# Christina-hshi/SH-assembly

Hardware: AMD Instinct MI355X
Metric: k-mers counted/sec (whole node), CQF build, C.elegans-like k=47 (higher is better)
Workload: dtype u64

## Files before the change

sh-assembly_amd/csrc/partition_kernels.hip:

```cpp
#include "shk_device.h"
#include <type_traits>

#define SHK_RP_TILE 4096
#define SHK_RP_MAXP 1024
#define SHK_SCAN_TILE 2048

struct ShkRpLevel {
  uint32_t shift;
  uint32_t bits;
  uint32_t nbuckets;
  uint32_t hb;
  uint64_t q_lo;
  uint64_t nslots;
  uint32_t cb;
  uint32_t out32;
  uint32_t ablate;
  uint32_t slot_cap;
  uint32_t ng_log2;
};

__device__ __forceinline__ uint32_t shk_word_region(uint64_t w, uint32_t hb, uint64_t q_lo) {
  uint64_t key = hb >= 64 ? w : (w & ((1ULL << hb) - 1));
  return (uint32_t)(((key >> 8) - q_lo) >> SHK_REGION_LOG2);
}

enum { RP_WORDS = 0, RP_NARROW_OUT = 1, RP_NARROW_IN = 2 };
__device__ __forceinline__ uint32_t shk_narrow_rec(uint64_t w, uint32_t hb, uint64_t q_lo, uint32_t cb) {
  const uint64_t key = hb >= 64 ? w : (w & ((1ULL << hb) - 1));
  const uint32_t up = (uint32_t)(key - (q_lo << 8)) & ((1u << (32 - cb)) - 1);
  return (up << cb) | ((uint32_t)(w >> hb) & ((1u << cb) - 1));
}

template <typename T>
__global__ void k_scan_reduce(const T *in, uint64_t n_host, const uint64_t *n_dev, uint64_t *block_sums) {
  __shared__ uint64_t scratch[SHK_MAX_WAVES + 1];
  const uint64_t n = n_dev ? *n_dev : n_host;
  const uint64_t base = (uint64_t)blockIdx.x * SHK_SCAN_TILE;
  uint64_t s = 0;
  for (uint64_t i = base + threadIdx.x; i < base + SHK_SCAN_TILE && i < n; i += blockDim.x) s += in[i];
  uint64_t tot = shk_block_sum64(s, scratch);
  if (threadIdx.x == 0) block_sums[blockIdx.x] = tot;
}
__global__ void k_scan_top(uint64_t *block_sums, uint64_t nblocks, uint64_t *total) {
  __shared__ uint64_t scratch[SHK_MAX_WAVES + 1];
  __shared__ uint64_t carry_s;
  if (threadIdx.x == 0) carry_s = 0;
  __syncthreads();
  for (uint64_t b = 0; b < nblocks; b += blockDim.x) {
    uint64_t i = b + threadIdx.x;
    uint64_t v = i < nblocks ? block_sums[i] : 0, tot;
    uint64_t ex = shk_block_exscan64(v, &tot, scratch);
    uint64_t carry = carry_s;
    if (i < nblocks) block_sums[i] = carry + ex;
    __syncthreads();
    if (threadIdx.x == 0) carry_s = carry + tot;
    __syncthreads();
  }
  if (threadIdx.x == 0) *total = carry_s;
}
template <typename T>
__global__ void k_scan_apply(const T *in, uint64_t n_host, const uint64_t *n_dev, const uint64_t *block_sums,
                             const uint64_t *total, uint64_t *out) {
  __shared__ uint64_t scratch[SHK_MAX_WAVES + 1];
  const uint64_t n = n_dev ? *n_dev : n_host;
  const uint64_t base = (uint64_t)blockIdx.x * SHK_SCAN_TILE;
  if (base > n) return;
  const unsigned per = SHK_SCAN_TILE / blockDim.x;
  const uint64_t my = base + (uint64_t)threadIdx.x * per;
  uint64_t s = 0;
  for (unsigned j = 0; j < per; j++)
    if (my + j < n) s += in[my + j];
  uint64_t tot;
  uint64_t ex = shk_block_exscan64(s, &tot, scratch) + block_sums[blockIdx.x];
  for (unsigned j = 0; j < per; j++) {
    if (my + j < n) { out[my + j] = ex; ex += in[my + j]; }
  }
  if (threadIdx.x == 0 && n >= base && n < base + SHK_SCAN_TILE) out[n] = *total;
}

__global__ void k_rp_base1(const uint64_t *n_p, uint64_t *bucket_base) {
  if (threadIdx.x == 0 && blockIdx.x == 0) { bucket_base[0] = 0; bucket_base[1] = *n_p; }
}

__global__ void k_rp_tile_first(const uint64_t *bucket_base, uint32_t nbuckets, const uint64_t *n_p, uint32_t *tfb) {
  const uint64_t n = *n_p;
  const uint64_t w = (uint64_t)blockIdx.x * blockDim.x + threadIdx.x;
  const uint64_t pos = w * SHK_RP_TILE;
  if (pos >= n) return;
  uint32_t lo = 0, hi = nbuckets;
  while (hi - lo > 1) {
    uint32_t mid = (lo + hi) / 2;
    if (bucket_base[mid] <= pos) lo = mid; else hi = mid;
  }
  tfb[w] = lo;
}

template <bool NARROW>
__global__ void k_rp_hist(const uint64_t *words_, const uint64_t *n_p, const uint64_t *bucket_base,
                          const uint32_t *tfb, ShkRpLevel lv, uint64_t *hist, uint32_t wtiles) {
  __shared__ uint32_t lh[SHK_RP_MAXP];
  using W = typename std::conditional<NARROW, uint32_t, uint64_t>::type;
  const W *words = reinterpret_cast<const W *>(words_);
  const uint64_t n = *n_p;
  const uint64_t wstart = (uint64_t)blockIdx.x * wtiles * SHK_RP_TILE;
  if (wstart >= n) return;
  const uint64_t wend = wstart + (uint64_t)wtiles * SHK_RP_TILE < n ? wstart + (uint64_t)wtiles * SHK_RP_TILE : n;
  const uint32_t P = 1u << lv.bits;
  for (uint32_t b = tfb[(uint64_t)blockIdx.x * wtiles]; b < lv.nbuckets && bucket_base[b] < wend; b++) {
    const uint64_t lo = bucket_base[b] > wstart ? bucket_base[b] : wstart;
    const uint64_t hi = bucket_base[b + 1] < wend ? bucket_base[b + 1] : wend;
    if (hi <= lo) continue;
    for (uint32_t d = threadIdx.x; d < (P << lv.ng_log2); d += blockDim.x) lh[d] = 0;
    __syncthreads();
    for (uint64_t i0 = lo; i0 < hi; i0 += 4ull * blockDim.x) {
      W w[4];
#pragma unroll
      for (int u = 0; u < 4; u++) {
        const uint64_t i = i0 + (uint64_t)u * blockDim.x + threadIdx.x;
        w[u] = i < hi ? words[i] : 0;
      }
#pragma unroll
      for (int u = 0; u < 4; u++) {
        const uint64_t i = i0 + (uint64_t)u * blockDim.x + threadIdx.x;
        if (i < hi) {
          const uint32_t dg = NARROW ? (uint32_t)(w[u] >> (16 + lv.cb)) : (shk_word_region(w[u], lv.hb, lv.q_lo) >> lv.shift) & (P - 1);
          const uint32_t grp = (uint32_t)(i >> SHK_RP_TILE0_LOG2) & ((1u << lv.ng_log2) - 1);
          atomicAdd(&lh[(dg << lv.ng_log2) | grp], 1u);
        }
      }
    }
    __syncthreads();
    for (uint32_t d = threadIdx.x; d < (P << lv.ng_log2); d += blockDim.x)
      if (lh[d]) atomicAdd((unsigned long long *)&hist[(((uint64_t)b * P) << lv.ng_log2) + d], (unsigned long long)lh[d]);
    __syncthreads();
  }
}

__global__ void k_rp_group_bases(const uint64_t *sub, uint32_t nd, uint32_t ng_log2, uint64_t *base) {
  const uint32_t d = blockIdx.x * blockDim.x + threadIdx.x;
  if (d <= nd) base[d] = sub[(uint64_t)d << ng_log2];
}

#define SHK_RP_THREADS 512
#define SHK_RP_KPT (SHK_RP_TILE / SHK_RP_THREADS)
template <int LB2>
__global__ void k_rp_hist2(const uint64_t *words, const uint64_t *n_p, ShkRpLevel lv0, ShkRpLevel lv1, uint64_t *hist0, uint64_t *hist1,
                           uint32_t wtiles) {
  __shared__ uint32_t lh0[SHK_RP_MAXP];
  __shared__ uint32_t lh1[1u << LB2];
  const uint64_t n = *n_p;
  const uint64_t wstart = (uint64_t)blockIdx.x * wtiles * SHK_RP_TILE;
  if (wstart >= n) return;
  const uint64_t wend = wstart + (uint64_t)wtiles * SHK_RP_TILE < n ? wstart + (uint64_t)wtiles * SHK_RP_TILE : n;
  const uint32_t P0 = 1u << lv0.bits, C = 1u << (lv0.bits + lv1.bits);
  for (uint32_t d = threadIdx.x; d < (P0 << lv0.ng_log2); d += blockDim.x) lh0[d] = 0;
  for (uint32_t d = threadIdx.x; d < C; d += blockDim.x) lh1[d] = 0;
  __syncthreads();
  for (uint64_t i0 = wstart; i0 < wend; i0 += 4ull * blockDim.x) {
    uint64_t w[4];
#pragma unroll
    for (int u = 0; u < 4; u++) {
      const uint64_t i = i0 + (uint64_t)u * blockDim.x + threadIdx.x;
      w[u] = i < wend ? words[i] : 0;
    }
#pragma unroll
    for (int u = 0; u < 4; u++) {
      const uint64_t i = i0 + (uint64_t)u * blockDim.x + threadIdx.x;
      if (i < wend) {
        const uint32_t region = shk_word_region(w[u], lv0.hb, lv0.q_lo);
        const uint32_t d0 = (region >> lv0.shift) & (P0 - 1);
        const uint32_t grp = (uint32_t)(i >> SHK_RP_TILE0_LOG2) & ((1u << lv0.ng_log2) - 1);
        atomicAdd(&lh0[(d0 << lv0.ng_log2) | grp], 1u);
        atomicAdd(&lh1[(region >> lv1.shift) & (C - 1)], 1u);
      }
    }
  }
  __syncthreads();
  for (uint32_t d = threadIdx.x; d < (P0 << lv0.ng_log2); d += blockDim.x)
    if (lh0[d]) atomicAdd((unsigned long long *)&hist0[d], (unsigned long long)lh0[d]);
  for (uint32_t d = threadIdx.x; d < C; d += blockDim.x)
    if (lh1[d]) atomicAdd((unsigned long long *)&hist1[d], (unsigned long long)lh1[d]);
}

__global__ void k_rp_slot_cursors(uint64_t *cursor, uint64_t n, uint32_t cap) {
  const uint64_t stride = (uint64_t)gridDim.x * blockDim.x;
  for (uint64_t i = (uint64_t)blockIdx.x * blockDim.x + threadIdx.x; i < n; i += stride) cursor[i] = i * cap;
}

template <int TILE_LOG2, int THREADS, int PMAX = SHK_RP_MAXP, int FORM = RP_WORDS>
__global__ void __launch_bounds__(THREADS) k_rp_scatter(const uint64_t *in_, uint64_t *out, const uint64_t *n_p,
                                                        const uint64_t *bucket_base, const uint32_t *tfb, ShkRpLevel lv,
                                                        uint64_t *cursor, uint32_t *err) {
  constexpr uint32_t SHK_RP_TILE_ = 1u << TILE_LOG2;
  constexpr int KPT_ = (int)(SHK_RP_TILE_ / THREADS);
  static_assert(SHK_RP_TILE_ <= 65536, "a rank inside a digit takes 16 bits");
  using WIN = typename std::conditional<FORM == RP_NARROW_IN, uint32_t, uint64_t>::type;
  using WST = typename std::conditional<FORM == RP_WORDS, uint64_t, uint32_t>::type;
  const WIN *in = reinterpret_cast<const WIN *>(in_);
  __shared__ uint32_t lh[PMAX];
  __shared__ uint32_t lbase[PMAX];
  __shared__ uint64_t gbase[PMAX];
  __shared__ WST stage[SHK_RP_TILE_];
  __shared__ uint32_t scratch[SHK_MAX_WAVES + 1];
  const uint64_t n = *n_p;
  const uint64_t wstart = (uint64_t)blockIdx.x * SHK_RP_TILE_;
  if (wstart >= n) return;
  const uint64_t wend = wstart + SHK_RP_TILE_ < n ? wstart + SHK_RP_TILE_ : n;
  const uint32_t P = 1u << lv.bits;
  for (uint32_t b = (lv.nbuckets > 1 ? tfb[(uint64_t)blockIdx.x << (TILE_LOG2 - 12)] : 0u); b < lv.nbuckets && bucket_base[b] < wend; b++) {
    const uint64_t lo = bucket_base[b] > wstart ? bucket_base[b] : wstart;
    const uint64_t hi = bucket_base[b + 1] < wend ? bucket_base[b + 1] : wend;
    if (hi <= lo) continue;
    const uint32_t cnt = (uint32_t)(hi - lo);
    for (uint32_t d = threadIdx.x; d < P; d += THREADS) lh[d] = 0;
    WIN w[KPT_];
#pragma unroll
    for (int u = 0; u < KPT_; u++) {
      const uint32_t i = threadIdx.x + (uint32_t)u * THREADS;
      w[u] = i < cnt ? in[lo + i] : 0;
    }
    __syncthreads();
    uint32_t dr[KPT_];
    WST x[KPT_];
#pragma unroll
    for (int u = 0; u < KPT_; u++) {
      const uint32_t i = threadIdx.x + (uint32_t)u * THREADS;
      dr[u] = 0;
      x[u] = (WST)w[u];
      if (i < cnt) {
        uint32_t d;
        if (FORM == RP_NARROW_IN) d = (uint32_t)(w[u] >> (16 + lv.cb));
        else d = (shk_word_region(w[u], lv.hb, lv.q_lo) >> lv.shift) & (P - 1);
        if (FORM == RP_NARROW_OUT) {
          const uint64_t key = lv.hb >= 64 ? w[u] : (w[u] & ((1ULL << lv.hb) - 1));
          if ((key >> 8) - lv.q_lo >= lv.nslots) atomicOr(err, SHK_E_CORRUPT);
          x[u] = (WST)shk_narrow_rec(w[u], lv.hb, lv.q_lo, lv.cb);
        }
        dr[u] = (d << 16) | atomicAdd(&lh[d], 1u);
      }
    }
    __syncthreads();
    uint32_t carry = 0;
    for (uint32_t d0 = 0; d0 < P; d0 += THREADS) {
      uint32_t d = d0 + threadIdx.x;
      uint32_t v = d < P ? lh[d] : 0, tot;
      uint32_t ex = shk_block_exscan(v, &tot, scratch);
      if (d < P) {
        lbase[d] = carry + ex;
        if (lv.ablate & 1) gbase[d] = cursor[((uint64_t)b * P + d) << lv.ng_log2] + (uint64_t)(blockIdx.x % 1024) * 24;
        else gbase[d] = v ? atomicAdd((unsigned long long *)&cursor[((((uint64_t)b * P) + d) << lv.ng_log2) | (blockIdx.x & ((1u << lv.ng_log2) - 1))], (unsigned long long)v) : 0;
        if (lv.slot_cap && v && gbase[d] + v > ((uint64_t)b * P + d + 1) * lv.slot_cap) {
          atomicOr(err, SHK_E_SLOT_FULL);
          gbase[d] = ~0ULL;
        }
      }
      carry += tot;
    }
    __syncthreads();
#pragma unroll
    for (int u = 0; u < KPT_; u++) {
      const uint32_t i = threadIdx.x + (uint32_t)u * THREADS;
      if (i < cnt) stage[lbase[dr[u] >> 16] + (dr[u] & 0xFFFFu)] = x[u];
    }
    __syncthreads();
    if (FORM == RP_NARROW_OUT) {
      uint32_t *out32 = reinterpret_cast<uint32_t *>(out);
      for (uint32_t d = threadIdx.x / SHK_WAVE; d < P; d += THREADS / SHK_WAVE) {
        const uint32_t l0 = lbase[d], len = lh[d];
        const uint64_t g0 = gbase[d];
        for (uint32_t j = threadIdx.x % SHK_WAVE; j < len; j += SHK_WAVE) out32[g0 + j] = stage[l0 + j];
      }
    } else {
      for (uint32_t i = threadIdx.x; i < cnt; i += THREADS) {
        const WST xs = stage[i];
        if (FORM == RP_NARROW_IN) {
          const uint32_t d = xs >> (16 + lv.cb);
          const uint32_t rec = (((uint32_t)(xs >> lv.cb) & 0xFFFFu) << SHK_CHUNK_BITS) | ((uint32_t)xs & ((1u << lv.cb) - 1));
          if (gbase[d] != ~0ULL) reinterpret_cast<uint32_t *>(out)[gbase[d] + (i - lbase[d])] = rec;
          continue;
        }
        const uint64_t x64 = xs;
        uint32_t d = (shk_word_region(x64, lv.hb, lv.q_lo) >> lv.shift) & (P - 1);
        if (lv.out32) {
          const uint64_t key = lv.hb >= 64 ? x64 : (x64 & ((1ULL << lv.hb) - 1));
          const uint64_t q = (key >> 8) - lv.q_lo;
          if (q >= lv.nslots) atomicOr(err, SHK_E_CORRUPT);
          const uint32_t rec = ((((uint32_t)q & (SHK_REGION - 1)) << 8 | (uint32_t)(key & 0xff)) << SHK_CHUNK_BITS) |
                               ((uint32_t)(x64 >> lv.hb) & (SHK_MAX_CHUNKS - 1));
          if (gbase[d] != ~0ULL) reinterpret_cast<uint32_t *>(out)[gbase[d] + (i - lbase[d])] = rec;
        } else {
          out[gbase[d] + (i - lbase[d])] = x64;
        }
      }
    }
    shk_lds_barrier();
  }
}
```

sh-assembly_amd/csrc/roll_kernels.hip:

```cpp
#include "shk_device.h"

#define SHK_ROLL_STEPS 16

struct ShkRollArgs {
  const uint8_t *text;
  uint64_t safe_end;
  const uint64_t *rd_start, *rd_end, *nreads_p;
  const uint16_t *rd_chunk;
  uint32_t chunk_first, chunk_mul, k, hb;
  uint64_t q_lo;
  uint32_t dig_shift, dig_bits;
  uint32_t hist_shift, hist_bits;
  uint64_t *hist;
  uint64_t *cursor;
  uint64_t *out;
  uint64_t cap;
  uint32_t *err;
  const struct ShkQuad *pk;
  const uint64_t *pk_base;
  const uint32_t *pk_flag;
};

struct ShkRollRow { uint64_t f, r; };
struct ShkRollTabs {
// ... 9 lines not shown
    const uint64_t f = b >= 0 ? sf[b] : 0, c = bc >= 0 ? sf[bc] : 0;
    t->in[i].f = f; t->in[i].r = shk_rol64(c, k - 1);
    t->out[i].f = shk_rol64(f, k); t->out[i].r = shk_ror64(c, 1);
    if (i < 4) {
      t->in4[i].f = sf[i]; t->in4[i].r = shk_rol64(sf[3 - i], k - 1);
      t->out4[i].f = shk_rol64(sf[i], k); t->out4[i].r = shk_ror64(sf[3 - i], 1);
    }
  }
}
__device__ __forceinline__ uint64_t shk_rol1(uint64_t x) {
  const uint32_t lo = (uint32_t)x, hi = (uint32_t)(x >> 32);
  return ((uint64_t)((hi << 1) | (lo >> 31)) << 32) | ((lo << 1) | (hi >> 31));
}
__device__ __forceinline__ uint64_t shk_ror1(uint64_t x) {
  const uint32_t lo = (uint32_t)x, hi = (uint32_t)(x >> 32);
  return ((uint64_t)((hi >> 1) | (lo << 31)) << 32) | ((lo >> 1) | (hi << 31));
}

struct ShkQuad { uint32_t x, y, z, w; };
__device__ __forceinline__ ShkQuad shk_quad(uint32_t x, uint32_t y, uint32_t z, uint32_t w) { ShkQuad q = {x, y, z, w}; return q; }
__device__ __forceinline__ ShkQuad shk_load16(const uint8_t *text, uint64_t at, uint64_t safe_end) {
  ShkQuad v;
  if (at + 16 <= safe_end) { __builtin_memcpy(&v, text + at, 16); return v; }
  uint32_t w[4] = {0, 0, 0, 0};
#pragma unroll
  for (int j = 0; j < 16; j++)
    if (at + j < safe_end) w[j >> 2] |= (uint32_t)text[at + j] << (8 * (j & 3));
  return shk_quad(w[0], w[1], w[2], w[3]);
}

#define SHK_ROLL_QUADS 4
struct ShkRollState {
  uint64_t st;
  uint32_t len;
  uint32_t i;
  uint32_t fill;
  uint64_t fh, rh;
  ShkQuad i0_, i1_, i2_, i3_, o0_, o1_, o2_, o3_;
};
__device__ __forceinline__ ShkQuad shk_pick_quad(const ShkQuad &a, const ShkQuad &b, const ShkQuad &c, const ShkQuad &d, uint32_t p) {
  const uint32_t m0 = 0u - (uint32_t)(p == 0), m1 = 0u - (uint32_t)(p == 1), m2 = 0u - (uint32_t)(p == 2), m3 = 0u - (uint32_t)(p == 3);
  ShkQuad v;
  v.x = (a.x & m0) | (b.x & m1) | (c.x & m2) | (d.x & m3);
  v.y = (a.y & m0) | (b.y & m1) | (c.y & m2) | (d.y & m3);
  v.z = (a.z & m0) | (b.z & m1) | (c.z & m2) | (d.z & m3);
  v.w = (a.w & m0) | (b.w & m1) | (c.w & m2) | (d.w & m3);
  return v;
}

template <int NQ, typename Emit>
__device__ __forceinline__ bool shk_roll_round(const ShkRollTabs *T, const uint8_t *text, uint64_t safe_end, ShkRollState &s,
                                               uint32_t k, uint64_t mask, Emit emit) {
  if (s.i >= s.len) return false;
  const uint32_t ph = (s.i / SHK_ROLL_STEPS) % NQ;
  if (ph == 0) {
#define SHK_ROLL_LOAD(Q, IN, OUT) { const uint32_t at = s.i + SHK_ROLL_STEPS * Q; \
      IN = at < s.len ? shk_load16(text, s.st + at, safe_end) : shk_quad(0, 0, 0, 0); \
      OUT = (at >= k && at < s.len) ? shk_load16(text, s.st + at - k, safe_end) : shk_quad(0, 0, 0, 0); }
    SHK_ROLL_LOAD(0, s.i0_, s.o0_)
    if (NQ > 1) SHK_ROLL_LOAD(1, s.i1_, s.o1_)
    if (NQ > 2) { SHK_ROLL_LOAD(2, s.i2_, s.o2_) SHK_ROLL_LOAD(3, s.i3_, s.o3_) }
#undef SHK_ROLL_LOAD
  }
  ShkQuad vin, vout;
  if (NQ == 1) { vin = s.i0_; vout = s.o0_; }
  else if (NQ == 2) { vin = shk_pick_quad(s.i0_, s.i1_, s.i0_, s.i1_, ph); vout = shk_pick_quad(s.o0_, s.o1_, s.o0_, s.o1_, ph); }
  else { vin = shk_pick_quad(s.i0_, s.i1_, s.i2_, s.i3_, ph); vout = shk_pick_quad(s.o0_, s.o1_, s.o2_, s.o3_, ph); }
  const uint32_t win[4] = {vin.x, vin.y, vin.z, vin.w}, wout[4] = {vout.x, vout.y, vout.z, vout.w};
  const uint32_t i0 = s.i;
  uint32_t anyN = 0;
#pragma unroll
  for (int q = 0; q < 4; q++) {
    const uint32_t x = win[q] ^ 0x4E4E4E4Eu;
    anyN |= (x - 0x01010101u) & ~x & 0x80808080u;
  }
  if (s.fill >= k && i0 >= k && !anyN) {
    uint64_t fh = s.fh, rh = s.rh;
    const auto step = [&](int j, bool whole) {
      const int sh = 8 * (j & 3) - 4;
      const uint32_t oi = (sh < 0 ? win[j >> 2] << 4 : win[j >> 2] >> sh) & 0xFF0u;
      const uint32_t oo = (sh < 0 ? wout[j >> 2] << 4 : wout[j >> 2] >> sh) & 0xFF0u;
      const ShkRollRow ri = *reinterpret_cast<const ShkRollRow *>(reinterpret_cast<const uint8_t *>(T->in) + oi);
      const ShkRollRow ro = *reinterpret_cast<const ShkRollRow *>(reinterpret_cast<const uint8_t *>(T->out) + oo);
      fh = shk_rol1(fh) ^ ri.f ^ ro.f;
      rh = shk_ror1(rh) ^ ri.r ^ ro.r;
      if (whole || i0 + j < s.len) emit(j, (fh < rh ? fh : rh) & mask);
    };
    if (i0 + SHK_ROLL_STEPS <= s.len) {
#pragma unroll
      for (int j = 0; j < SHK_ROLL_STEPS; j++) step(j, true);
    } else {
#pragma unroll
      for (int j = 0; j < SHK_ROLL_STEPS; j++) step(j, false);
    }
    s.fh = fh; s.rh = rh;
  } else if (s.fill + SHK_ROLL_STEPS < k && i0 + SHK_ROLL_STEPS <= s.len) {
    uint64_t fh = s.fh, rh = s.rh;
#pragma unroll
    for (int j = 0; j < SHK_ROLL_STEPS; j++) {
      const int sh = 8 * (j & 3) - 4;
      const uint32_t oi = (sh < 0 ? win[j >> 2] << 4 : win[j >> 2] >> sh) & 0xFF0u;
      const ShkRollRow ri = *reinterpret_cast<const ShkRollRow *>(reinterpret_cast<const uint8_t *>(T->in) + oi);
      fh = shk_rol1(fh) ^ ri.f;
      rh = shk_ror1(rh) ^ ri.r;
    }
    s.fh = fh; s.rh = rh; s.fill += SHK_ROLL_STEPS;
  } else {
#pragma unroll
    for (int j = 0; j < SHK_ROLL_STEPS; j++) {
      if (i0 + j < s.len) {
        const uint32_t cin = (win[j >> 2] >> (8 * (j & 3))) & 0xFFu;
        if (s.fill >= k && cin == 'N') {
          s.fill = 0; s.fh = 0; s.rh = 0;
        } else {
          uint64_t f = shk_rol1(s.fh) ^ T->in[cin].f, r = shk_ror1(s.rh) ^ T->in[cin].r;
          if (s.fill >= k) {
            const uint32_t cout = i0 >= k ? (wout[j >> 2] >> (8 * (j & 3))) & 0xFFu : text[s.st + i0 + j - k];
            f ^= T->out[cout].f; r ^= T->out[cout].r;
          } else s.fill++;
          s.fh = f; s.rh = r;
          if (s.fill >= k) emit(j, (f < r ? f : r) & mask);
        }
      }
    }
  }
  s.i = i0 + SHK_ROLL_STEPS < s.len ? i0 + SHK_ROLL_STEPS : s.len;
  return true;
}

__global__ void k_pack_count(const uint64_t *rd_start, const uint64_t *rd_end, const uint64_t *nreads_p, uint32_t k, uint32_t *units) {
  const uint64_t nreads = *nreads_p;
  const uint64_t stride = (uint64_t)gridDim.x * blockDim.x;
  for (uint64_t r = (uint64_t)blockIdx.x * blockDim.x + threadIdx.x; r < nreads; r += stride) {
    const uint64_t len = rd_end[r] - rd_start[r];
    units[r] = (len >= k && len <= 65535) ? (uint32_t)((len + 63) >> 6) : 0;
  }
}
__device__ __forceinline__ uint32_t shk_zero_bytes(uint32_t v) { return ~(((v & 0x7F7F7F7Fu) + 0x7F7F7F7Fu) | v | 0x7F7F7F7Fu); }
__global__ void k_pack_reads(const uint8_t *text, uint64_t safe_end, const uint64_t *rd_start, const uint64_t *rd_end, const uint64_t *nreads_p,
                             const uint64_t *pk_base, uint32_t *flag, ShkQuad *pk, uint64_t cap_units) {
  const uint64_t nreads = *nreads_p;
  const uint64_t stride = ((uint64_t)gridDim.x * blockDim.x) >> 2;
  for (uint64_t r = ((uint64_t)blockIdx.x * blockDim.x + threadIdx.x) >> 2; r < nreads; r += stride) {
    const uint32_t units = flag[r] & 0x7FFFFFFFu;
    if (!units) continue;
    const uint64_t base = pk_base[r];
    if (base + units > cap_units) { if ((threadIdx.x & 3) == 0) atomicOr(&flag[r], 0x80000000u); continue; }
    const uint64_t st = rd_start[r];
    const uint32_t len = (uint32_t)(rd_end[r] - st);
    uint32_t bad = 0;
    for (uint32_t u = threadIdx.x & 3; u < units; u += 4) {
      uint32_t o[4] = {0, 0, 0, 0};
#pragma unroll
      for (int q = 0; q < 4; q++) {
        const uint32_t pos = 64 * u + 16 * q;
        if (pos < len) {
          const ShkQuad v = shk_load16(text, st + pos, safe_end);
          const uint32_t w[4] = {v.x, v.y, v.z, v.w};
#pragma unroll
          for (int b = 0; b < 4; b++) {
            const uint32_t y = w[b] & 0xDFDFDFDFu;
            const uint32_t ok = shk_zero_bytes(y ^ 0x41414141u) | shk_zero_bytes(y ^ 0x43434343u) | shk_zero_bytes(y ^ 0x47474747u) |
                                shk_zero_bytes(y ^ 0x54545454u);
            const uint32_t left = len - pos > 4u * b ? len - pos - 4u * b : 0;
            const uint32_t need = left >= 4 ? 0x80808080u : (0x80808080u & ((1u << (8 * left)) - 1));
            bad |= need & ~ok;
            const uint32_t x = ((w[b] >> 1) ^ (w[b] >> 2)) & 0x03030303u;
            o[q] |= ((x * 0x01041040u) >> 24) << (8 * b);
          }
        }
      }
      pk[base + u] = shk_quad(o[0], o[1], o[2], o[3]);
    }
    if (bad) atomicOr(&flag[r], 0x80000000u);
  }
}

__device__ __forceinline__ uint32_t shk_pick_word(uint32_t a, uint32_t b, uint32_t c, uint32_t d, uint32_t p) {
  return (a & (0u - (uint32_t)(p == 0))) | (b & (0u - (uint32_t)(p == 1))) | (c & (0u - (uint32_t)(p == 2))) | (d & (0u - (uint32_t)(p == 3)));
}
template <typename Emit>
__device__ __forceinline__ bool shk_roll_round_pk(const ShkRollTabs *T, const ShkQuad *pk, ShkRollState &s, uint32_t k, uint64_t mask, Emit emit) {
  if (s.i >= s.len) return false;
  const uint32_t i0 = s.i, ph = (i0 >> 4) & 3;
  if (ph == 0) s.i0_ = pk[i0 >> 6];
  const uint32_t zin = shk_pick_word(s.i0_.x, s.i0_.y, s.i0_.z, s.i0_.w, ph);
  uint64_t fh = s.fh, rh = s.rh;
  if (i0 >= k) {
    const uint32_t n = (i0 >> 4) - ((k + 15) >> 4);
    const uint32_t n3 = n - 3 * ((n * 0xAAABu) >> 17);
    const uint32_t ob = 2 * (i0 - k);
    if (n3 == 0) __builtin_memcpy(&s.o0_, reinterpret_cast<const uint8_t *>(pk) + 4 * (uint64_t)(ob >> 5), 16);
    const uint32_t a = shk_pick_word(s.o0_.x, s.o0_.y, s.o0_.z, 0, n3), b = shk_pick_word(s.o0_.y, s.o0_.z, s.o0_.w, 0, n3);
    const uint32_t zout = (uint32_t)((((uint64_t)b << 32) | a) >> (ob & 31));
    const auto step = [&](int j, bool whole) {
      const uint32_t oi = (j < 2 ? zin << (4 - 2 * j) : zin >> (2 * j - 4)) & 0x30u;
      const uint32_t oo = (j < 2 ? zout << (4 - 2 * j) : zout >> (2 * j - 4)) & 0x30u;
      const ShkRollRow ri = *reinterpret_cast<const ShkRollRow *>(reinterpret_cast<const uint8_t *>(T->in4) + oi);
      const ShkRollRow ro = *reinterpret_cast<const ShkRollRow *>(reinterpret_cast<const uint8_t *>(T->out4) + oo);
      fh = shk_rol1(fh) ^ ri.f ^ ro.f;
      rh = shk_ror1(rh) ^ ri.r ^ ro.r;
      if (whole || i0 + j < s.len) emit(j, (fh < rh ? fh : rh) & mask);
    };
    if (i0 + SHK_ROLL_STEPS <= s.len) {
#pragma unroll
      for (int j = 0; j < SHK_ROLL_STEPS; j++) step(j, true);
    } else {
#pragma unroll
      for (int j = 0; j < SHK_ROLL_STEPS; j++) step(j, false);
    }
  } else if (i0 + SHK_ROLL_STEPS < k) {
#pragma unroll
    for (int j = 0; j < SHK_ROLL_STEPS; j++) {
      const uint32_t oi = (j < 2 ? zin << (4 - 2 * j) : zin >> (2 * j - 4)) & 0x30u;
      const ShkRollRow ri = *reinterpret_cast<const ShkRollRow *>(reinterpret_cast<const uint8_t *>(T->in4) + oi);
      fh = shk_rol1(fh) ^ ri.f;
      rh = shk_ror1(rh) ^ ri.r;
    }
  } else {
    const uint32_t z0 = (i0 >> 6) == 0 ? s.i0_.x : pk[0].x;
#pragma unroll
    for (int j = 0; j < SHK_ROLL_STEPS; j++) {
      const uint32_t idx = i0 + j;
      const ShkRollRow ri = T->in4[(zin >> (2 * j)) & 3u];
      uint64_t f = shk_rol1(fh) ^ ri.f, r = shk_ror1(rh) ^ ri.r;
      if (idx >= k) {
        const ShkRollRow ro = T->out4[(z0 >> (2 * (idx - k))) & 3u];
        f ^= ro.f; r ^= ro.r;
      }
      fh = f; rh = r;
      if (idx + 1 >= k && idx < s.len) emit(j, (f < r ? f : r) & mask);
    }
  }
  s.fh = fh; s.rh = rh;
  s.i = i0 + SHK_ROLL_STEPS < s.len ? i0 + SHK_ROLL_STEPS : s.len;
  return true;
}

__device__ __forceinline__ uint32_t shk_roll_digit(uint64_t key, const ShkRollArgs &A) {
  const uint32_t region = (uint32_t)(key >> 16) - (uint32_t)(A.q_lo >> 8);
  return (region >> A.dig_shift) & ((1u << A.dig_bits) - 1);
}

template <int LB, int THREADS>
__global__ void __launch_bounds__(THREADS) k_roll_hist(ShkRollArgs A) {
  __shared__ ShkRollTabs T;
  __shared__ uint32_t lh[1u << LB];
  shk_roll_tabs_init(&T, A.k);
  const uint32_t P = 1u << A.hist_bits;
  for (uint32_t d = threadIdx.x; d < P; d += blockDim.x) lh[d] = 0;
  __syncthreads();
  const uint64_t nreads = *A.nreads_p;
  const uint64_t mask = A.hb >= 64 ? ~0ULL : ((1ULL << A.hb) - 1);
  const uint64_t stride = (uint64_t)gridDim.x * blockDim.x;
  const uint32_t qlo16 = (uint32_t)(A.q_lo >> 8);
  for (uint64_t r = (uint64_t)blockIdx.x * blockDim.x + threadIdx.x; r < nreads; r += stride) {
    const uint64_t st = A.rd_start[r], en = A.rd_end[r];
    if (en - st > 65535) { atomicOr(A.err, SHK_E_BAD_FASTQ); continue; }
    if (en - st < A.k) continue;
    ShkRollState s;
    s.st = st; s.len = (uint32_t)(en - st); s.i = 0; s.fill = 0; s.fh = 0; s.rh = 0;
    const auto count = [&](int, uint64_t key) { atomicAdd(&lh[(((uint32_t)(key >> 16) - qlo16) >> A.hist_shift) & (P - 1)], 1u); };
    if (A.pk && !(A.pk_flag[r] >> 31)) {
      const ShkQuad *up = A.pk + A.pk_base[r];
      while (shk_roll_round_pk(&T, up, s, A.k, mask, count)) {}
    } else {
      while (shk_roll_round<4>(&T, A.text, A.safe_end, s, A.k, mask, count)) {}
    }
  }
  __syncthreads();
  for (uint32_t d = threadIdx.x; d < P; d += blockDim.x)
    if (lh[d]) atomicAdd((unsigned long long *)&A.hist[d], (unsigned long long)lh[d]);
}
__global__ void k_roll_fold(const uint64_t *hist2, uint32_t p0, uint32_t p1, uint64_t *hist0) {
  const uint32_t d = blockIdx.x * blockDim.x + threadIdx.x;
  if (d >= p0) return;
  uint64_t t = 0;
  for (uint32_t j = 0; j < p1; j++) t += hist2[(uint64_t)d * p1 + j];
  hist0[d] = t;
}

template <int THREADS, int NQ>
__global__ void __launch_bounds__(THREADS) k_roll_scatter(ShkRollArgs A) {
  constexpr uint32_t TILE = THREADS * SHK_ROLL_STEPS;
  __shared__ ShkRollTabs T;
  __shared__ uint32_t lh[1024], lbase[1024];
  __shared__ uint64_t gbase[1024];
  __shared__ uint64_t stage[TILE];
  __shared__ uint32_t scratch[SHK_MAX_WAVES + 1];
  __shared__ uint32_t any_left;
  shk_roll_tabs_init(&T, A.k);
  const uint32_t P = 1u << A.dig_bits;
  const uint64_t nreads = *A.nreads_p;
  const uint64_t mask = A.hb >= 64 ? ~0ULL : ((1ULL << A.hb) - 1);
  const uint64_t stride = (uint64_t)gridDim.x * THREADS;
  uint64_t r = (uint64_t)blockIdx.x * THREADS + threadIdx.x;
  ShkRollState s;
  s.st = 0; s.len = 0; s.i = 0; s.fill = 0; s.fh = 0; s.rh = 0;
  uint64_t tag = 0;
  bool have = false;
  for (;;) {
    while (!have && r < nreads) {
      const uint64_t st = A.rd_start[r], en = A.rd_end[r];
      if (en - st <= 65535 && en - st >= A.k) {
        s.st = st; s.len = (uint32_t)(en - st); s.i = 0; s.fill = 0; s.fh = 0; s.rh = 0;
        tag = (uint64_t)(A.chunk_first + A.rd_chunk[r] * A.chunk_mul) << A.hb;
        if (A.pk && !(A.pk_flag[r] >> 31)) s.st = A.pk_base[r] | (1ULL << 63);
        have = true;
      }
      r += stride;
    }
    for (uint32_t d = threadIdx.x; d < P; d += THREADS) lh[d] = 0;
    if (threadIdx.x == 0) any_left = 0;
    shk_lds_barrier();
    uint64_t w[SHK_ROLL_STEPS];
    uint32_t vm = 0;
    if (have) {
      const auto keep = [&](int j, uint64_t key) {
        w[j] = key | tag;
        atomicAdd(&lh[shk_roll_digit(key, A)], 1u);
        vm |= 1u << j;
      };
      have = (s.st >> 63) ? shk_roll_round_pk(&T, A.pk + (s.st & ~(1ULL << 63)), s, A.k, mask, keep)
                          : shk_roll_round<NQ>(&T, A.text, A.safe_end, s, A.k, mask, keep);
      if (have && s.i >= s.len) have = false;
    }
    if (have || r < nreads) any_left = 1;
    __syncthreads();
    const bool more = any_left != 0;
    uint32_t carry = 0;
    for (uint32_t d0 = 0; d0 < P; d0 += THREADS) {
      const uint32_t d = d0 + threadIdx.x;
      uint32_t v = d < P ? lh[d] : 0, tot;
      const uint32_t ex = shk_block_exscan(v, &tot, scratch);
      if (d < P) {
        lbase[d] = carry + ex;
        gbase[d] = (v ? atomicAdd((unsigned long long *)&A.cursor[d], (unsigned long long)v) : 0) - (carry + ex);
      }
      carry += tot;
    }
    __syncthreads();
    const uint32_t cnt = carry;
#pragma unroll
    for (int u = 0; u < SHK_ROLL_STEPS; u++)
      if ((vm >> u) & 1u) stage[atomicAdd(&lbase[shk_roll_digit(A.hb >= 64 ? w[u] : (w[u] & mask), A)], 1u)] = w[u];
    __syncthreads();
    for (uint32_t i = threadIdx.x; i < cnt; i += THREADS) {
      const uint64_t x = stage[i];
      const uint32_t d = shk_roll_digit(A.hb >= 64 ? x : (x & mask), A);
      const uint64_t at = gbase[d] + i;
      if (at < A.cap) A.out[at] = x; else atomicOr(A.err, SHK_E_KEYS_FULL);
    }
    shk_lds_barrier();
    if (!more) break;
  }
}
```

sh-assembly_amd/csrc/shk_api.hip:

```cpp
#include "../../include/shk.h"
#include <thread>

#include <hip/hip_runtime.h>
#include <math.h>
#include <stdio.h>
#include <stdlib.h>
#include <string.h>
#include <vector>
#include <string>
#include <algorithm>
#include <unordered_set>
#include <unordered_map>

#include "kmer_kernels.hip"
#include "roll_kernels.hip"
#include "partition_kernels.hip"
#include "cqf_kernels.hip"
#include "merge2_kernels.hip"
#include "walk_kernels.hip"
#include "unitig_kernels.hip"

#define SHK_SLACK 256

enum {
  KP_COUNT_LINES, KP_SCAN_CHUNKS, KP_EMIT_READS, KP_COUNT_KEYS, KP_HASH, KP_SCAN, KP_RP_PREP, KP_RP_HIST,
  KP_RP_SCATTER, KP_MERGE_SUM, KP_REGION_SCAN, KP_MERGE_WRITE, KP_MERGE_SPILL, KP_PLACE, KP_MARKS, KP_LOOKUP, KP_WALK, KP_UG_WALK, KP_UG_FINISH, KP_MERGE_FUSED, KP_MERGE_SAMPLE, KP_MISC, KP_ROLL_HIST, KP_ROLL_SCATTER, KP_PACK, KP_RP_SLOTS, KP_RP_SCATTER_NARROW, KP_SPECTRUM, KP_JOIN, KP_N
};
static const char *kp_names[KP_N] = {
  "k_count_lines", "k_scan_chunks", "k_emit_reads", "k_count_keys", "k_hash_reads", "k_scan_*", "k_rp_prep",
  "k_rp_hist", "k_rp_scatter", "k_region_merge<summary>", "k_region_scan", "k_region_merge<write>",
  "k_region_merge<spill>", "k_region_place", "k_denoise_marks", "k_lookup", "k_extend_forward+k_select_seeds", "k_ug_walk", "k_ug_check/emit/median/links", "k_region_merge<fused>", "k_region_merge<sample>", "misc", "k_roll_hist", "k_roll_scatter", "k_pack_reads", "k_rp_slot_cursors", "k_rp_scatter<narrow>", "k_region_spectrum", "k_region_join"};

struct PendingEvent { int id; hipEvent_t a, b; };

#define SHK_SCALAR_WORDS 64
enum ShkDevSlot {
  DS_NREADS = 0,
  DS_NWORDS = 1,
  DS_SCAN_TOTAL = 2,
  DS_MARKS = 3,
  DS_MAX_COUNT = 4,
  DS_DUMP_STOP = 5,
  DS_JOIN_STOP = 6,
  DS_JOIN_ACC = 7,
  DS_WALK_IN = 8,
  DS_WALK_OUT = 10,
  DS_SPECTRUM = 12,
  DS_STAMPS = 16,
  DS_PAIR_LEN = 40,
  DS_PAIR_BASE = 42,
  DS_END = 46
};
enum ShkHostSlot {
  HP_COUNTERS = 0,
  HP_SPECTRUM = 8,
  HP_ERR = 40,
  HP_NREADS = 41,
  HP_NWORDS = 42,
  HP_NWORDS_IN = 43,
  HP_FREE_PTR = 44,
  HP_TOTAL = 45,
  HP_AUX = 46,
  HP_MARKS = 47,
  HP_IFIN = 48,
  HP_IFIRST = 49,
  HP_WALK_IN = 50,
  HP_WALK_OUT = 52,
  HP_PAIR = 56,
  HP_END = 62
};
enum { CNT_NEWD, CNT_ADDED, CNT_REMOVED, CNT_ADDED_BEFORE };
static_assert(HP_COUNTERS + SHK_NCOUNTERS <= HP_ERR, "the counters mirror ends before the error word");
static_assert(HP_COUNTERS + SHK_NCOUNTERS <= HP_SPECTRUM && DS_SPECTRUM + (int)SHK_SPEC_WORDS <= DS_STAMPS, "the spectrum's totals have four words of their own");
static_assert(DS_END <= SHK_SCALAR_WORDS && HP_END <= SHK_SCALAR_WORDS, "both blocks fit their 64 words");
static_assert(DS_PAIR_BASE + 4 == DS_END && HP_PAIR + (DS_END - DS_PAIR_LEN) == HP_END, "the pair block is uploaded in one copy");

enum { RP_SCATTER_GROUPED, RP_SCATTER_WIDE, RP_SCATTER_TILE };
struct ShkPartLevel {
  uint8_t scatter;
  bool pair_hist;
  bool may_slot;
  bool may_narrow;
};

struct ShkStageBufs {
  hipStream_t stream = hipStream_t();
  bool lent = false;
  uint8_t *d_text = nullptr;
  uint64_t *d_chunk_off = nullptr, *d_chunk_len = nullptr, *d_nlines = nullptr, *d_reads_base = nullptr;
  uint64_t *d_rd_start = nullptr, *d_rd_end = nullptr;
  uint16_t *d_rd_chunk = nullptr;
  uint32_t *d_nkeys = nullptr;
  uint64_t *d_key_base = nullptr;
  uint64_t *d_words[2] = {};
  uint64_t *d_scalars = nullptr;
  uint64_t *d_block_sums = nullptr;
  uint64_t *d_hist[4] = {};
  uint64_t *d_base_sub = nullptr;
  uint64_t *d_base[5] = {};
  uint64_t *d_cursor = nullptr;
  uint32_t *d_tfb = nullptr;
  uint32_t *d_err = nullptr;
  uint64_t *h_pinned = nullptr;
  uint32_t last_err_bits = 0;
  uint32_t region_cap = 0;
  uint32_t slot_overflows = 0;
  int slots_off = 0;
  double prof_ms[KP_N] = {};
  uint64_t prof_n[KP_N] = {};
  std::vector<PendingEvent> pending;
  std::vector<hipEvent_t> evpool;
};

struct shk_ctx : ShkStageBufs {
  shk_config cfg;
  int dev;
  uint64_t g_nslots;
  uint64_t q_lo, nslots, xnslots, nblocks, table_bytes;
  uint32_t nregions, rbits;
  uint32_t nlevels;
  ShkRpLevel lv[4];
  ShkPartLevel part[4];
  bool roll_two;
  uint32_t threads, hash_groups;
  uint64_t nelts, ndistinct;
  uint32_t rounds_left, rounds_done;
  uint8_t *tab[2];
  uint64_t *fin[2];
  int cur;
  uint8_t *d_up[2];
  hipStream_t copy_stream;
  hipEvent_t up_done[2];
  int up_next, up_pending[2];
  uint32_t *d_summary;
  long long *d_tile_a, *d_tile_b, *d_tile_f;
  uint64_t *d_dump_offs;
  int big_image;
  uint8_t *spill[2];
  int live;
  int rec_live;
  int table_stale;
  int lazy_ok;
  uint32_t *d_over_list;
  int spill_valid; const uint64_t *spill_words; uint32_t spill_lo, spill_hi; int spill_denoise, spill_big;
  uint64_t spill_nover;
  uint16_t *d_newchunks;
  unsigned long long *d_chist;
  uint64_t *h_chist;
  uint32_t chist_n;
  uint32_t sample_stride;
  uint32_t pt_lo, pt_split, pt_hi; int pt_valid; uint64_t pt_nprot;
  const uint64_t *pt_words;
  unsigned long long *d_counters;
  uint64_t max_reads;
  int prof_on;
  double new_frac;
  int staged;
  uint32_t *d_isum; uint8_t *d_ilens; uint64_t *d_fin_i; uint64_t *d_prot;
  int counted;
  uint64_t *d_send[2];
  int send_next;
  struct ShkFront *front;
};

#define HIPCHK(x) do { hipError_t e_ = (x); if (e_ != hipSuccess) { fprintf(stderr, "libshk: %s failed: %s (%s:%d)\n", #x, hipGetErrorString(e_), __FILE__, __LINE__); return SHK_ERR_HIP; } } while (0)

static hipEvent_t ev_get(ShkStageBufs *c) {
  if (!c->evpool.empty()) { hipEvent_t e = c->evpool.back(); c->evpool.pop_back(); return e; }
  hipEvent_t e; hipEventCreate(&e); return e;
}
struct ProfScope {
  ShkStageBufs *c; int id; bool on; hipEvent_t a, b;
  ProfScope(const shk_ctx *ctx, ShkStageBufs *c_, int id_) : c(c_), id(id_), on(ctx->prof_on != 0) {
    if (on) { a = ev_get(c); b = ev_get(c); hipEventRecord(a, c->stream); }
  }
  ProfScope(shk_ctx *ctx, int id_) : ProfScope(ctx, ctx, id_) {}
  ~ProfScope() {
    if (on) { hipEventRecord(b, c->stream); PendingEvent p = {id, a, b}; c->pending.push_back(p); }
  }
};
static void prof_collect(ShkStageBufs *c) {
  for (size_t i = 0; i < c->pending.size(); i++) {
    float ms = 0;
    hipEventSynchronize(c->pending[i].b);
    hipEventElapsedTime(&ms, c->pending[i].a, c->pending[i].b);
    c->prof_ms[c->pending[i].id] += ms;
    c->prof_n[c->pending[i].id]++;
    c->evpool.push_back(c->pending[i].a);
    c->evpool.push_back(c->pending[i].b);
  }
  c->pending.clear();
}

static int map_err_bits(uint32_t bits) {
  if (!bits) return SHK_OK;
  if (bits & SHK_E_TABLE_FULL) return SHK_ERR_TABLE_FULL;
  if (bits & (SHK_E_OLD_EXTENT | SHK_E_NEW_EXTENT | SHK_E_HASH_FULL | SHK_E_RUN_TOO_LONG)) return SHK_ERR_REGION;
  if (bits & SHK_E_CORRUPT) return SHK_ERR_CORRUPT;
  if (bits & SHK_E_BAD_FASTQ) return SHK_ERR_FASTQ;
  if (bits & SHK_E_KEYS_FULL) return SHK_ERR_BATCH;
  return SHK_ERR_CORRUPT;
}

extern "C" const char *shk_strerror(int code) {
  switch (code) {
    case SHK_OK: return "ok";
    case SHK_ERR_ARG: return "bad argument or unsupported geometry";
    case SHK_ERR_HIP: return "HIP runtime error (is a GPU present?)";
    case SHK_ERR_TABLE_FULL: return "counting quotient filter is full";
    case SHK_ERR_REGION: return "a 256-quotient region exceeds the kernel's on-chip image or hash";
    case SHK_ERR_CORRUPT: return "table metadata inconsistent or key outside this context's range";
    case SHK_ERR_FASTQ: return "malformed FASTQ input";
    case SHK_ERR_BATCH: return "batch exceeds the capacities given to shk_create";
    case SHK_ERR_IO: return "file I/O error";
  }
  return "unknown error";
}
extern "C" uint32_t shk_last_error_bits(shk_ctx *c) { return c ? c->last_err_bits : 0; }

template <typename T> static int dmalloc(T **p, uint64_t n) {
  void *v = nullptr;
  HIPCHK(hipMalloc(&v, n * sizeof(T) + SHK_SLACK));
  *p = (T *)v;
  return 0;
}

static int ensure_chist(shk_ctx *c);
static int point_alloc(shk_ctx *c);
static uint64_t level_out(const shk_ctx *c, uint32_t l) { return (uint64_t)c->lv[l].nbuckets << c->lv[l].bits; }

static int bufs_alloc(const shk_ctx *c, ShkStageBufs *b, bool lent) {
  const uint64_t capk = c->cfg.max_batch_keys;
  const uint32_t maxch = SHK_MAX_CHUNKS;
  b->lent = lent;
  if (lent) HIPCHK(hipStreamCreateWithFlags(&b->stream, hipStreamNonBlocking));
  else HIPCHK(hipStreamCreate(&b->stream));
  if (dmalloc(&b->d_text, c->cfg.max_batch_bytes + 64)) return SHK_ERR_HIP;
  if (dmalloc(&b->d_chunk_off, maxch) || dmalloc(&b->d_chunk_len, maxch) || dmalloc(&b->d_nlines, (uint64_t)maxch * SHK_PARSE_SEGS) ||
      dmalloc(&b->d_reads_base, maxch + 1)) return SHK_ERR_HIP;
  if (dmalloc(&b->d_rd_start, c->max_reads + 1) || dmalloc(&b->d_rd_end, c->max_reads + 1) ||
      dmalloc(&b->d_nkeys, c->max_reads + 1) || dmalloc(&b->d_rd_chunk, c->max_reads + 1) || dmalloc(&b->d_key_base, c->max_reads + 2)) return SHK_ERR_HIP;
  if (!lent && (dmalloc(&b->d_words[0], capk + 1) || dmalloc(&b->d_words[1], capk + 1))) return SHK_ERR_HIP;
  if (dmalloc(&b->d_scalars, SHK_SCALAR_WORDS)) return SHK_ERR_HIP;
  HIPCHK(hipMemsetAsync(b->d_scalars, 0, SHK_SCALAR_WORDS * 8, b->stream));
  {
    uint64_t mx = capk > c->max_reads ? capk : c->max_reads;
    uint64_t pw = 1ULL << c->rbits;
    if (pw > mx) mx = pw;
    if (dmalloc(&b->d_block_sums, mx / SHK_SCAN_TILE + 4 + 8192)) return SHK_ERR_HIP;
  }
  if (dmalloc(&b->d_base[0], 2)) return SHK_ERR_HIP;
  for (uint32_t l = 0; l < c->nlevels; l++) {
    const uint64_t n = level_out(c, l);
    if (dmalloc(&b->d_hist[l], (n << c->lv[l].ng_log2) + 1)) return SHK_ERR_HIP;
    if (!(lent && l + 1 == c->nlevels) && dmalloc(&b->d_base[l + 1], n + 2)) return SHK_ERR_HIP;
    if (l == 0 && dmalloc(&b->d_base_sub, (n << c->lv[0].ng_log2) + 2)) return SHK_ERR_HIP;
  }
  { const uint64_t nb = level_out(c, c->nlevels - 1), first = 1ULL << (c->lv[0].bits + c->lv[0].ng_log2);
    if (dmalloc(&b->d_cursor, (nb > first ? nb : first) + 2)) return SHK_ERR_HIP; }
  if (dmalloc(&b->d_tfb, capk / SHK_RP_TILE + 2)) return SHK_ERR_HIP;
  if (dmalloc(&b->d_err, 4)) return SHK_ERR_HIP;
  HIPCHK(hipMemsetAsync(b->d_err, 0, 16, b->stream));
  HIPCHK(hipHostMalloc((void **)&b->h_pinned, SHK_SCALAR_WORDS * sizeof(uint64_t), hipHostMallocDefault));
  HIPCHK(hipStreamSynchronize(b->stream));
  return SHK_OK;
}

static void bufs_free(const shk_ctx *c, ShkStageBufs *b) {
  if (b->stream) hipStreamSynchronize(b->stream);
  prof_collect(b);
  for (size_t i = 0; i < b->evpool.size(); i++) hipEventDestroy(b->evpool[i]);
  b->evpool.clear();
  hipFree(b->d_text); hipFree(b->d_chunk_off); hipFree(b->d_chunk_len); hipFree(b->d_nlines); hipFree(b->d_reads_base);
  hipFree(b->d_rd_start); hipFree(b->d_rd_end); hipFree(b->d_rd_chunk); hipFree(b->d_nkeys); hipFree(b->d_key_base); hipFree(b->d_scalars);
  hipFree(b->d_block_sums); hipFree(b->d_base_sub); hipFree(b->d_cursor); hipFree(b->d_tfb); hipFree(b->d_err);
  if (!b->lent) { hipFree(b->d_words[0]); hipFree(b->d_words[1]); }
  for (uint32_t l = 0; l < 4; l++) hipFree(b->d_hist[l]);
  for (uint32_t l = 0; l < 5; l++) if (!(b->lent && l == c->nlevels)) hipFree(b->d_base[l]);
  hipHostFree(b->h_pinned);
  if (b->stream) hipStreamDestroy(b->stream);
  *b = ShkStageBufs();
}

static int create_init(shk_ctx *c, const shk_config *cfg) {
  const uint32_t ns = cfg->num_shards ? cfg->num_shards : 1;
  c->cfg = *cfg;
  c->dev = cfg->device;
  HIPCHK(hipSetDevice(c->dev));
  c->g_nslots = 1ULL << cfg->qb;
  if (c->g_nslots / ns < 64) return SHK_ERR_ARG;
  c->nslots = c->g_nslots / ns;
  c->q_lo = c->nslots * cfg->shard_index;
  c->xnslots = c->nslots + (uint64_t)(10 * sqrt((double)c->g_nslots));
  c->nblocks = (c->xnslots + 63) / 64;
  c->table_bytes = c->nblocks * SHK_BLOCK_BYTES;
  c->nregions = (uint32_t)((c->nslots + SHK_REGION - 1) / SHK_REGION);
  c->rbits = 0;
  while ((1u << c->rbits) < c->nregions) c->rbits++;
  const uint32_t mlb = cfg->max_level_bits ? cfg->max_level_bits : 10;
  if (mlb > 10) return SHK_ERR_ARG;
  const uint32_t nlevels = (c->rbits + mlb - 1) / mlb;
  if (nlevels > 4) return SHK_ERR_ARG;
  c->nlevels = nlevels ? nlevels : 1;
  {
    uint32_t left = c->rbits, nb = 1;
    for (uint32_t l = 0; l < c->nlevels; l++) {
      uint32_t bits = (left + (c->nlevels - l) - 1) / (c->nlevels - l);
      left -= bits;
      c->lv[l].shift = left; c->lv[l].bits = bits; c->lv[l].nbuckets = nb; c->lv[l].hb = cfg->hb; c->lv[l].q_lo = c->q_lo;
      c->lv[l].nslots = c->nslots; c->lv[l].cb = 0; c->lv[l].out32 = 0; c->lv[l].ablate = 0; c->lv[l].ng_log2 = 0; c->lv[l].slot_cap = 0;
      nb <<= bits;
    }
    c->lv[c->nlevels - 1].out32 = 1;
    if (c->lv[0].bits >= 2 && c->lv[0].bits <= 7 && !getenv("SHK_RP_NO_GROUPS")) c->lv[0].ng_log2 = 3;
  }
  c->threads = cfg->threads_per_group ? cfg->threads_per_group : 512;
  if (c->threads < 64 || c->threads > 1024 || (c->threads & (c->threads - 1))) return SHK_ERR_ARG;
  c->hash_groups = cfg->hash_groups ? cfg->hash_groups : 2048;
  const bool words8 = getenv("SHK_RP_WORDS8") && atoi(getenv("SHK_RP_WORDS8")) != 0;
  c->roll_two = c->nlevels >= 2 && c->lv[0].bits + c->lv[1].bits <= 14;
  for (uint32_t l = 0; l < c->nlevels; l++) {
    const bool last = l + 1 == c->nlevels;
    c->part[l].scatter = l == 0 && c->lv[0].ng_log2 ? RP_SCATTER_GROUPED : c->threads >= 512 && !last && c->lv[l].bits <= 8 ? RP_SCATTER_WIDE : RP_SCATTER_TILE;
    c->part[l].pair_hist = l == 0 && c->roll_two && c->lv[1].ng_log2 == 0;
    c->part[l].may_slot = last && l >= 1 && c->lv[l].out32;
    c->part[l].may_narrow = l >= 1 && l + 2 == c->nlevels && !words8;
    c->lv[l].cb = 32 - 16 - c->lv[c->nlevels - 1].bits;
  }
  c->rounds_left = cfg->num_denoise;
  c->max_reads = cfg->max_batch_reads ? cfg->max_batch_reads : cfg->max_batch_bytes / 16 + 1024;
  { int rc = bufs_alloc(c, c, false); if (rc) return rc; }
  for (int i = 0; i < 2; i++) {
    if (dmalloc(&c->tab[i], c->table_bytes)) return SHK_ERR_HIP;
    if (dmalloc(&c->fin[i], (uint64_t)c->nregions + 2)) return SHK_ERR_HIP;
  }
  if (dmalloc(&c->d_summary, SHK_SUM_STRIDE * (uint64_t)c->nregions + 8)) return SHK_ERR_HIP;
  if (dmalloc(&c->d_dump_offs, (uint64_t)c->nregions + 2)) return SHK_ERR_HIP;
  c->sample_stride = c->nregions >= (1u << 20) ? 16 : 8;
  if (const char *e = getenv("SHK_SAMPLE_STRIDE")) c->sample_stride = (uint32_t)atoi(e);
  else if (c->nregions < (1u << 14)) c->sample_stride = 0;
  c->lazy_ok = 1;
  if (const char *e = getenv("SHK_LAZY_PLACE")) c->lazy_ok = atoi(e) != 0;
  if (dmalloc(&c->spill[0], (uint64_t)c->nregions * SHK_SPILL_STRIDE) || dmalloc(&c->d_over_list, (uint64_t)c->nregions + 1)) return SHK_ERR_HIP;
  { uint64_t nt = c->nregions / SHK_RSCAN_TILE + 2;
    if (dmalloc(&c->d_tile_a, nt) || dmalloc(&c->d_tile_b, nt) || dmalloc(&c->d_tile_f, nt)) return SHK_ERR_HIP; }
  if (dmalloc(&c->d_counters, SHK_NCOUNTERS)) return SHK_ERR_HIP;
  HIPCHK(hipMemsetAsync(c->tab[0], 0, c->table_bytes + SHK_SLACK, c->stream));
  HIPCHK(hipMemsetAsync(c->tab[1], 0, c->table_bytes + SHK_SLACK, c->stream));
  HIPCHK(hipMemsetAsync(c->fin[0], 0, ((uint64_t)c->nregions + 2) * 8, c->stream));
  HIPCHK(hipMemsetAsync(c->fin[1], 0, ((uint64_t)c->nregions + 2) * 8, c->stream));
  HIPCHK(hipStreamSynchronize(c->stream));
  if (cfg->num_denoise > 0 || cfg->num_shards > 1) {
    if (ensure_chist(c) || point_alloc(c)) return SHK_ERR_HIP;
  }
  if (cfg->num_shards > 1) {
    for (int b = 0; b < 2; b++)
      if (dmalloc(&c->d_send[b], c->cfg.max_batch_keys + 1)) return SHK_ERR_HIP;
  }
  return SHK_OK;
}

extern "C" int shk_create(const shk_config *cfg, shk_ctx **out) {
  if (!cfg || !out) return SHK_ERR_ARG;
  if (cfg->qb < 6 || cfg->qb > 40 || cfg->hb != cfg->qb + 8 || cfg->k < 1 || cfg->k > SHK_MAX_K) return SHK_ERR_ARG;
  uint32_t ns = cfg->num_shards ? cfg->num_shards : 1;
  if (ns & (ns - 1)) return SHK_ERR_ARG;
  if (cfg->shard_index >= ns) return SHK_ERR_ARG;
  if (cfg->hb + SHK_CHUNK_BITS > 64) return SHK_ERR_ARG;
  shk_ctx *c = new shk_ctx();
  const int rc = create_init(c, cfg);
  if (rc) { shk_destroy(c); return rc; }
  *out = c;
  return SHK_OK;
}

static void front_destroy(shk_ctx *c);
extern "C" void shk_destroy(shk_ctx *c) {
  if (!c) return;
  hipSetDevice(c->dev);
  front_destroy(c);
  if (c->stream) hipStreamSynchronize(c->stream);
  if (c->copy_stream) {
    hipStreamSynchronize(c->copy_stream);
    for (int b = 0; b < 2; b++) { if (c->d_up[b]) hipFree(c->d_up[b]); if (c->up_done[b]) hipEventDestroy(c->up_done[b]); }
    hipStreamDestroy(c->copy_stream);
  }
  if (getenv("SHK_STAMPS") && c->d_scalars) {
    unsigned long long st[16];
    hipMemcpy(st, c->d_scalars + DS_STAMPS, sizeof(st), hipMemcpyDeviceToHost);
    static const char *nm[9] = {"stage+init", "fold keys", "old rank/select", "count sort", "merge pass", "scan+stats", "(unused)", "placement", "stores"};
    unsigned long long tot = 0; for (int i = 0; i < 9; i++) tot += st[i];
    for (int i = 0; i < 9; i++) fprintf(stderr, "SHK_STAMPS %-16s %6.2f %%\n", nm[i], tot ? 100.0 * st[i] / tot : 0.0);
  }
  for (int i = 0; i < 2; i++) { hipFree(c->tab[i]); hipFree(c->fin[i]); hipFree(c->d_send[i]); }
  hipFree(c->d_isum); hipFree(c->d_ilens); hipFree(c->d_fin_i); hipFree(c->d_prot);
  hipFree(c->d_newchunks); hipFree(c->d_chist); hipHostFree(c->h_chist);
  hipFree(c->spill[0]); hipFree(c->spill[1]); hipFree(c->d_over_list); hipFree(c->d_summary); hipFree(c->d_dump_offs); hipFree(c->d_tile_a); hipFree(c->d_tile_b); hipFree(c->d_tile_f); hipFree(c->d_counters);
  bufs_free(c, c);
  delete c;
}

template <typename T>
static int run_scan(const shk_ctx *c, ShkStageBufs *b, const T *in, uint64_t n_max, const uint64_t *n_dev, uint64_t *out, uint64_t *sums = nullptr) {
  ProfScope ps(c, b, KP_SCAN);
  if (!sums) sums = b->d_block_sums;
  const uint32_t nb = (uint32_t)(n_max / SHK_SCAN_TILE + 1);
  hipLaunchKernelGGL((k_scan_reduce<T>), dim3(nb), dim3(c->threads), 0, b->stream, in, n_max, n_dev, sums);
  hipLaunchKernelGGL(k_scan_top, dim3(1), dim3(c->threads), 0, b->stream, sums, (uint64_t)nb, b->d_scalars + DS_SCAN_TOTAL);
  hipLaunchKernelGGL((k_scan_apply<T>), dim3(nb), dim3(c->threads), 0, b->stream, in, n_max, n_dev, sums,
                     b->d_scalars + DS_SCAN_TOTAL, out);
  HIPCHK(hipGetLastError());
  return 0;
}

static int err_enqueue(ShkStageBufs *b) { HIPCHK(hipMemcpyAsync(b->h_pinned + HP_ERR, b->d_err, 4, hipMemcpyDeviceToHost, b->stream)); return 0; }
static int err_take(ShkStageBufs *b, bool record, uint32_t *bits) {
  *bits = *(uint32_t *)(b->h_pinned + HP_ERR);
  if (*bits && record) b->last_err_bits = *bits;
  if (*bits) HIPCHK(hipMemsetAsync(b->d_err, 0, 16, b->stream));
  return 0;
}
static int fetch_err(ShkStageBufs *b, uint32_t *bits) {
  if (err_enqueue(b)) return SHK_ERR_HIP;
  HIPCHK(hipStreamSynchronize(b->stream));
  return err_take(b, true, bits);
}
static int set_nwords(ShkStageBufs *b, uint64_t n) {
  b->h_pinned[HP_NWORDS_IN] = n;
  HIPCHK(hipMemcpyAsync(b->d_scalars + DS_NWORDS, b->h_pinned + HP_NWORDS_IN, 8, hipMemcpyHostToDevice, b->stream));
  return 0;
}

static int upload_wait(shk_ctx *c, const void *text, int on_device, hipStream_t stream) {
  for (int u = 0; on_device && u < 2; u++)
    if (c->d_up[u] && text == (const void *)c->d_up[u] && c->up_pending[u]) { HIPCHK(hipStreamWaitEvent(stream, c->up_done[u], 0)); c->up_pending[u] = 0; }
  return SHK_OK;
}

static bool chunk_labels_ok(uint32_t nchunks, uint32_t chunk_first, uint32_t chunk_mul) {
  return nchunks != 0 && nchunks <= SHK_MAX_CHUNKS && chunk_first + (uint64_t)(nchunks - 1) * chunk_mul < SHK_MAX_CHUNKS;
}

static bool text_aligned(const void *text, int on_device) { return !on_device || ((uintptr_t)text & 15) == 0; }
static int parse_stage(const shk_ctx *c, ShkStageBufs *b, const void *text, int on_device, uint64_t text_bytes, const uint64_t *chunk_off,
                       const uint64_t *chunk_len, uint32_t nchunks, const uint8_t **dtext_out, uint64_t *nreads_out) {
  if (!text_aligned(text, on_device)) return SHK_ERR_ARG;
  for (uint32_t i = 0; i < nchunks; i++)
    if (chunk_off[i] + chunk_len[i] > text_bytes) return SHK_ERR_ARG;
  const uint8_t *dtext;
  if (on_device) {
    dtext = (const uint8_t *)text;
  } else {
    if (text_bytes > c->cfg.max_batch_bytes) return SHK_ERR_BATCH;
    HIPCHK(hipMemcpyAsync(b->d_text, text, text_bytes, hipMemcpyHostToDevice, b->stream));
    dtext = b->d_text;
  }
  HIPCHK(hipMemcpyAsync(b->d_chunk_off, chunk_off, nchunks * 8, hipMemcpyHostToDevice, b->stream));
  HIPCHK(hipMemcpyAsync(b->d_chunk_len, chunk_len, nchunks * 8, hipMemcpyHostToDevice, b->stream));
  { ProfScope ps(c, b, KP_COUNT_LINES);
    hipLaunchKernelGGL(k_count_lines, dim3(nchunks * SHK_PARSE_SEGS), dim3(c->threads), 0, b->stream, dtext, b->d_chunk_off, b->d_chunk_len, b->d_nlines); }
  { ProfScope ps(c, b, KP_SCAN_CHUNKS);
    hipLaunchKernelGGL(k_scan_chunks, dim3(1), dim3(c->threads), 0, b->stream, b->d_nlines, nchunks, b->d_reads_base, b->d_scalars + DS_NREADS); }
  HIPCHK(hipMemcpyAsync(b->h_pinned + HP_NREADS, b->d_scalars + DS_NREADS, 8, hipMemcpyDeviceToHost, b->stream));
  HIPCHK(hipStreamSynchronize(b->stream));
  const uint64_t nreads = b->h_pinned[HP_NREADS];
  if (nreads > c->max_reads) return SHK_ERR_BATCH;
  { ProfScope ps(c, b, KP_EMIT_READS);
    hipLaunchKernelGGL(k_emit_reads, dim3(nchunks * SHK_PARSE_SEGS), dim3(c->threads), 0, b->stream, dtext, b->d_chunk_off, b->d_chunk_len,
                       b->d_reads_base, b->d_nlines, b->d_rd_start, b->d_rd_end, b->d_rd_chunk); }
  *dtext_out = dtext;
  *nreads_out = nreads;
  return SHK_OK;
}

static int hash_stage(const shk_ctx *c, ShkStageBufs *b, const void *text, int on_device, uint64_t text_bytes, const uint64_t *chunk_off,
                      const uint64_t *chunk_len, uint32_t nchunks, uint32_t chunk_first, uint32_t chunk_mul, bool hist0 = false) {
  if (!chunk_labels_ok(nchunks, chunk_first, chunk_mul)) return SHK_ERR_BATCH;
  if (!text_aligned(text, on_device)) return SHK_ERR_ARG;
  if (hist0) HIPCHK(hipMemsetAsync(b->d_hist[0], 0, (1ULL << (c->lv[0].bits + c->lv[0].ng_log2)) * 8, b->stream));
  const uint8_t *dtext;
  uint64_t nreads;
  { int rc = parse_stage(c, b, text, on_device, text_bytes, chunk_off, chunk_len, nchunks, &dtext, &nreads); if (rc) return rc; }
  uint32_t groups = c->hash_groups;
  { uint64_t need = nreads / (c->threads / SHK_WAVE) + 1; if (need < groups) groups = (uint32_t)need; }
  { ProfScope ps(c, b, KP_COUNT_KEYS);
    const uint64_t blocks = nreads / 256 + 1;
    hipLaunchKernelGGL(k_count_keys, dim3((uint32_t)(blocks < (1u << 20) ? blocks : (1u << 20))), dim3(256), 0, b->stream, dtext, b->d_rd_start, b->d_rd_end,
                       b->d_scalars + DS_NREADS, c->cfg.k, b->d_nkeys, b->d_err); }
  if (run_scan<uint32_t>(c, b, b->d_nkeys, nreads, nullptr, b->d_key_base)) return SHK_ERR_HIP;
  HIPCHK(hipMemcpyAsync(b->d_scalars + DS_NWORDS, b->d_key_base + nreads, 8, hipMemcpyDeviceToDevice, b->stream));
  { ProfScope ps(c, b, KP_HASH);
    const uint32_t ht = c->threads < SHK_HASH_WAVES * SHK_WAVE ? c->threads : SHK_HASH_WAVES * SHK_WAVE;
    hipLaunchKernelGGL(k_hash_reads, dim3(groups * (c->threads / ht)), dim3(ht), 0, b->stream, dtext, b->d_rd_start, b->d_rd_end,
                       b->d_scalars + DS_NREADS, b->d_rd_chunk, chunk_first, chunk_mul, b->d_key_base, c->cfg.k, c->cfg.hb,
                       b->d_words[0], c->cfg.max_batch_keys, b->d_err, hist0 ? b->d_hist[0] : nullptr, c->lv[0].shift, c->lv[0].bits, c->q_lo, c->lv[0].ng_log2); }
  HIPCHK(hipGetLastError());
  return SHK_OK;
}

static int pack_stage(const shk_ctx *c, ShkStageBufs *b, ShkRollArgs &A, uint64_t nreads, uint64_t text_bytes, uint64_t *buf) {
  A.pk = nullptr; A.pk_base = nullptr; A.pk_flag = nullptr;
  const uint64_t cap_units = c->cfg.max_batch_keys / 2 > 1 ? c->cfg.max_batch_keys / 2 - 1 : 0;
  if (getenv("SHK_NO_PACK") || text_bytes / 64 + nreads + 1 > cap_units) return SHK_OK;
  ProfScope ps(c, b, KP_PACK);
  const uint32_t t = c->threads < 256 ? c->threads : 256;
  { const uint64_t blocks = nreads / t + 1;
    hipLaunchKernelGGL(k_pack_count, dim3((uint32_t)(blocks < 4096 ? blocks : 4096)), dim3(t), 0, b->stream, (const uint64_t *)b->d_rd_start,
                       (const uint64_t *)b->d_rd_end, (const uint64_t *)(b->d_scalars + DS_NREADS), c->cfg.k, b->d_nkeys); }
  if (run_scan<uint32_t>(c, b, b->d_nkeys, nreads, nullptr, b->d_key_base)) return SHK_ERR_HIP;
  { const uint64_t blocks = nreads * 4 / t + 1;
    hipLaunchKernelGGL(k_pack_reads, dim3((uint32_t)(blocks < 16384 ? blocks : 16384)), dim3(t), 0, b->stream, A.text, A.safe_end,
                       (const uint64_t *)b->d_rd_start, (const uint64_t *)b->d_rd_end, (const uint64_t *)(b->d_scalars + DS_NREADS),
                       (const uint64_t *)b->d_key_base, b->d_nkeys, (ShkQuad *)buf, cap_units); }
  A.pk = (const ShkQuad *)buf; A.pk_base = b->d_key_base; A.pk_flag = b->d_nkeys;
  return SHK_OK;
}

static void roll_args(const shk_ctx *c, ShkStageBufs *b, ShkRollArgs &A, const uint8_t *dtext, uint64_t text_bytes,
                      uint32_t chunk_first, uint32_t chunk_mul) {
  A.text = dtext; A.safe_end = (text_bytes + 15) & ~15ULL;
  A.rd_start = b->d_rd_start; A.rd_end = b->d_rd_end; A.nreads_p = b->d_scalars + DS_NREADS; A.rd_chunk = b->d_rd_chunk;
  A.chunk_first = chunk_first; A.chunk_mul = chunk_mul; A.k = c->cfg.k; A.hb = c->cfg.hb;
  A.cap = c->cfg.max_batch_keys; A.err = b->d_err;
}
static void launch_roll_hist(const shk_ctx *c, ShkStageBufs *b, const ShkRollArgs &A, uint64_t nreads, bool wide) {
  const bool small = c->threads < 512;
  const uint32_t t = small ? 64 : wide ? 512 : 256, max_blocks = small ? 64 : wide ? 1024 : 4096;
  const uint64_t blocks = nreads / t + 1;
  const dim3 grid((uint32_t)(blocks < max_blocks ? blocks : max_blocks));
  if (small && wide) hipLaunchKernelGGL((k_roll_hist<14, 64>), grid, dim3(64), 0, b->stream, A);
  else if (small) hipLaunchKernelGGL((k_roll_hist<10, 64>), grid, dim3(64), 0, b->stream, A);
  else if (wide) hipLaunchKernelGGL((k_roll_hist<14, 512>), grid, dim3(512), 0, b->stream, A);
  else hipLaunchKernelGGL((k_roll_hist<10, 256>), grid, dim3(256), 0, b->stream, A);
}
static void launch_roll_scatter(const shk_ctx *c, ShkStageBufs *b, const ShkRollArgs &A, uint64_t nreads) {
  ProfScope ps(c, b, KP_ROLL_SCATTER);
  if (c->threads >= 512) {
    const uint64_t blocks = nreads / 1024 + 1;
    hipLaunchKernelGGL((k_roll_scatter<1024, 1>), dim3((uint32_t)(blocks < 512 ? blocks : 512)), dim3(1024), 0, b->stream, A);
  } else {
    const uint64_t blocks = nreads / 64 + 1;
    hipLaunchKernelGGL((k_roll_scatter<64, 4>), dim3((uint32_t)(blocks < 64 ? blocks : 64)), dim3(64), 0, b->stream, A);
  }
}

static bool roll_path(const shk_ctx *c) { return c->nlevels >= 2; }
static int roll_stage(const shk_ctx *c, ShkStageBufs *b, const void *text, int on_device, uint64_t text_bytes, const uint64_t *chunk_off,
                      const uint64_t *chunk_len, uint32_t nchunks, uint32_t chunk_first, uint32_t chunk_mul) {
  if (!chunk_labels_ok(nchunks, chunk_first, chunk_mul)) return SHK_ERR_BATCH;
  const uint8_t *dtext;
  uint64_t nreads;
  { int rc = parse_stage(c, b, text, on_device, text_bytes, chunk_off, chunk_len, nchunks, &dtext, &nreads); if (rc) return rc; }
  const uint64_t P = 1ULL << c->lv[0].bits;
  const uint32_t cb = c->lv[0].bits + c->lv[1].bits;
  const bool two = c->roll_two;
  if (two) HIPCHK(hipMemsetAsync(b->d_hist[1], 0, (1ULL << cb) * 8, b->stream));
  else HIPCHK(hipMemsetAsync(b->d_hist[0], 0, P * 8, b->stream));
  ShkRollArgs A;
  roll_args(c, b, A, dtext, text_bytes, chunk_first, chunk_mul);
  A.q_lo = c->q_lo;
  A.dig_shift = c->lv[0].shift; A.dig_bits = c->lv[0].bits;
  A.hist = two ? b->d_hist[1] : b->d_hist[0]; A.hist_shift = two ? c->lv[1].shift : c->lv[0].shift; A.hist_bits = two ? cb : c->lv[0].bits;
  A.cursor = b->d_cursor; A.out = b->d_words[0];
  { int rc = pack_stage(c, b, A, nreads, text_bytes, b->d_words[1]); if (rc) return rc; }
  { ProfScope ps(c, b, KP_ROLL_HIST);
    launch_roll_hist(c, b, A, nreads, two);
    if (two) hipLaunchKernelGGL(k_roll_fold, dim3((uint32_t)(P / 256 + 1)), dim3(256), 0, b->stream, (const uint64_t *)b->d_hist[1], (uint32_t)P,
                                1u << c->lv[1].bits, b->d_hist[0]); }
  if (run_scan<uint64_t>(c, b, b->d_hist[0], P, nullptr, b->d_base[1])) return SHK_ERR_HIP;
  HIPCHK(hipMemcpyAsync(b->d_scalars + DS_NWORDS, b->d_base[1] + P, 8, hipMemcpyDeviceToDevice, b->stream));
  HIPCHK(hipMemcpyAsync(b->d_cursor, b->d_base[1], P * 8, hipMemcpyDeviceToDevice, b->stream));
  launch_roll_scatter(c, b, A, nreads);
  HIPCHK(hipGetLastError());
  return SHK_OK;
}

struct ShkPartInput {
  const uint64_t *src[2]; uint64_t n[2]; int nsrc;
  int in_buf;
  uint32_t first_level;
  bool counted[2];
  uint32_t nchunks;
};
static ShkPartInput part_from_roll(const shk_ctx *c, const ShkStageBufs *b, uint64_t n, uint32_t nchunks) { return {{b->d_words[0], nullptr}, {n, 0}, 1, 0, 1, {false, c->roll_two}, nchunks}; }
static ShkPartInput part_from_hash(const ShkStageBufs *b, uint64_t n, uint32_t nchunks) { return {{b->d_words[0], nullptr}, {n, 0}, 1, 0, 0, {true, false}, nchunks}; }
static ShkPartInput part_from_words(const ShkStageBufs *b, const uint64_t *w, uint64_t n, const uint64_t *w2 = nullptr, uint64_t n2 = 0) {
  return {{w, w2}, {n, n2}, w2 ? 2 : 1, w == b->d_words[0] ? 0 : w == b->d_words[1] ? 1 : -1, 0, {false, false}, 0};
}

static uint32_t slot_capacity(const shk_ctx *c, uint64_t nregions, uint64_t nwords) {
  uint64_t cp = 2 * c->cfg.max_batch_keys / nregions;
  if (cp > (1u << 20)) cp = 1u << 20;
  const double mean = (double)nwords / (double)nregions;
  return cp >= 64 && (double)cp >= mean + 6.0 * sqrt(8.0 * mean + 1.0) + 16.0 ? (uint32_t)cp : 0;
}

static int partition_stage(const shk_ctx *c, ShkStageBufs *b, const ShkPartInput &in, int *dst) {
  const uint64_t *n_p = b->d_scalars + DS_NWORDS;
  const uint64_t nmax = in.n[0] + in.n[1];
  { ProfScope ps(c, b, KP_RP_PREP);
    hipLaunchKernelGGL(k_rp_base1, dim3(1), dim3(64), 0, b->stream, n_p, b->d_base[0]); }
  const uint32_t nwin = (uint32_t)(nmax / SHK_RP_TILE + 1);
  int cur = in.in_buf < 0 ? 1 : in.in_buf;
  bool counted[4] = {in.counted[0], in.counted[1], false, false};
  bool narrow = false;
  b->region_cap = 0;
  for (uint32_t l = in.first_level; l < c->nlevels; l++) {
    const ShkPartLevel &pl = c->part[l];
    const uint64_t nb = c->lv[l].nbuckets, P = 1ULL << c->lv[l].bits;
    const bool narrow_in = narrow;
    narrow = pl.may_narrow && in.nchunks && in.nchunks <= (1u << c->lv[l].cb);
    struct Src { const uint64_t *w, *n_p, *base; uint64_t n; } srcs[2] = {{l == in.first_level ? in.src[0] : b->d_words[cur], n_p, b->d_base[l], nmax}, {}};
    int nsrc = 1;
    if (l == 0 && in.nsrc == 2) {
      srcs[0] = {in.src[0], b->d_scalars + DS_PAIR_LEN, b->d_scalars + DS_PAIR_BASE, in.n[0]};
      srcs[1] = {in.src[1], b->d_scalars + DS_PAIR_LEN + 1, b->d_scalars + DS_PAIR_BASE + 2, in.n[1]};
      nsrc = 2;
    }
    uint32_t cap = pl.may_slot && !b->slots_off && !counted[l] ? slot_capacity(c, nb * P, nmax) : 0;
    { ProfScope ps(c, b, KP_RP_PREP);
      hipLaunchKernelGGL(k_rp_tile_first, dim3(nwin / 256 + 1), dim3(256), 0, b->stream, b->d_base[l], (uint32_t)nb, n_p, b->d_tfb); }
    for (;;) {
      ShkRpLevel lvl = c->lv[l];
#ifdef SHK_DIAGNOSTICS
      if (const char *e = getenv("SHK_RP_ABLATE")) lvl.ablate = (uint32_t)atoi(e);
#endif
      uint64_t *cursor = b->d_cursor;
      if (cap) {
        ProfScope ps(c, b, KP_RP_SLOTS);
        cursor = b->d_base[l + 1];
        lvl.slot_cap = cap;
        hipLaunchKernelGGL(k_rp_slot_cursors, dim3((uint32_t)((nb * P) / 256 + 1 < 4096 ? (nb * P) / 256 + 1 : 4096)), dim3(256), 0, b->stream, cursor, nb * P, cap);
      } else {
        if (!counted[l] && pl.pair_hist) {
          HIPCHK(hipMemsetAsync(b->d_hist[0], 0, (P << c->lv[0].ng_log2) * 8, b->stream));
          HIPCHK(hipMemsetAsync(b->d_hist[1], 0, (P << c->lv[1].bits) * 8, b->stream));
          ProfScope ps(c, b, KP_RP_HIST);
          const uint32_t wt = nwin / 1024 + 1;
          for (int si = 0; si < nsrc; si++)
            hipLaunchKernelGGL((k_rp_hist2<14>), dim3(nwin / wt + 1), dim3(c->threads < 512 ? c->threads : 512), 0, b->stream, srcs[si].w, srcs[si].n_p,
                               c->lv[0], c->lv[1], b->d_hist[0], b->d_hist[1], wt);
          counted[1] = true;
        } else if (!counted[l]) {
          HIPCHK(hipMemsetAsync(b->d_hist[l], 0, ((nb * P) << c->lv[l].ng_log2) * 8, b->stream));
          ProfScope ps(c, b, KP_RP_HIST);
          const uint32_t wt = nwin / 4096 + 1;
          for (int si = 0; si < nsrc; si++)
            if (narrow_in)
              hipLaunchKernelGGL(k_rp_hist<true>, dim3(nwin / wt + 1), dim3(c->threads), 0, b->stream, srcs[si].w, srcs[si].n_p, srcs[si].base, b->d_tfb,
                                 c->lv[l], b->d_hist[l], wt);
            else
              hipLaunchKernelGGL(k_rp_hist<false>, dim3(nwin / wt + 1), dim3(c->threads), 0, b->stream, srcs[si].w, srcs[si].n_p, srcs[si].base, b->d_tfb,
                                 c->lv[l], b->d_hist[l], wt);
        }
        if (c->lv[l].ng_log2) {
          const uint32_t ng = c->lv[l].ng_log2;
          if (run_scan<uint64_t>(c, b, b->d_hist[l], P << ng, nullptr, b->d_base_sub)) return SHK_ERR_HIP;
          HIPCHK(hipMemcpyAsync(b->d_cursor, b->d_base_sub, (P << ng) * 8, hipMemcpyDeviceToDevice, b->stream));
          ProfScope ps(c, b, KP_RP_PREP);
          hipLaunchKernelGGL(k_rp_group_bases, dim3((uint32_t)(P / 256 + 1)), dim3(256), 0, b->stream, b->d_base_sub, (uint32_t)P, ng, b->d_base[l + 1]);
        } else {
          if (run_scan<uint64_t>(c, b, b->d_hist[l], nb * P, nullptr, b->d_base[l + 1])) return SHK_ERR_HIP;
          HIPCHK(hipMemcpyAsync(b->d_cursor, b->d_base[l + 1], nb * P * 8, hipMemcpyDeviceToDevice, b->stream));
        }
      }
      { ProfScope ps(c, b, narrow || narrow_in ? KP_RP_SCATTER_NARROW : KP_RP_SCATTER);
        for (int si = 0; si < nsrc; si++) {
          const Src &S = srcs[si];
          const dim3 wide((uint32_t)(S.n >> SHK_RP_TILE0_LOG2) + 1);
          if (narrow && pl.scatter == RP_SCATTER_WIDE)
            hipLaunchKernelGGL((k_rp_scatter<SHK_RP_TILE0_LOG2, 1024, 256, RP_NARROW_OUT>), wide, dim3(1024), 0, b->stream, S.w, b->d_words[cur ^ 1], S.n_p,
                               S.base, b->d_tfb, lvl, cursor, b->d_err);
          else if (narrow)
            hipLaunchKernelGGL((k_rp_scatter<12, SHK_RP_THREADS, SHK_RP_MAXP, RP_NARROW_OUT>), dim3((uint32_t)(S.n / SHK_RP_TILE + 1)), dim3(SHK_RP_THREADS), 0,
                               b->stream, S.w, b->d_words[cur ^ 1], S.n_p, S.base, b->d_tfb, lvl, cursor, b->d_err);
          else if (narrow_in)
            hipLaunchKernelGGL((k_rp_scatter<12, SHK_RP_THREADS, SHK_RP_MAXP, RP_NARROW_IN>), dim3((uint32_t)(S.n / SHK_RP_TILE + 1)), dim3(SHK_RP_THREADS), 0,
                               b->stream, S.w, b->d_words[cur ^ 1], S.n_p, S.base, b->d_tfb, lvl, cursor, b->d_err);
          else if (pl.scatter == RP_SCATTER_GROUPED)
            hipLaunchKernelGGL((k_rp_scatter<SHK_RP_TILE0_LOG2, 1024>), wide, dim3(1024), 0, b->stream, S.w, b->d_words[cur ^ 1], S.n_p, S.base,
                               b->d_tfb, lvl, cursor, b->d_err);
          else if (pl.scatter == RP_SCATTER_WIDE)
            hipLaunchKernelGGL((k_rp_scatter<SHK_RP_TILE0_LOG2, 1024, 256>), wide, dim3(1024), 0, b->stream, S.w, b->d_words[cur ^ 1], S.n_p, S.base,
                               b->d_tfb, lvl, cursor, b->d_err);
          else
            hipLaunchKernelGGL((k_rp_scatter<12, SHK_RP_THREADS>), dim3((uint32_t)(S.n / SHK_RP_TILE + 1)), dim3(SHK_RP_THREADS), 0, b->stream, S.w,
                               b->d_words[cur ^ 1], S.n_p, S.base, b->d_tfb, lvl, cursor, b->d_err);
        } }
      if (!cap) break;
      uint32_t bits = 0;
      if (fetch_err(b, &bits)) return SHK_ERR_HIP;
      if (bits & ~SHK_E_SLOT_FULL) return map_err_bits(bits & ~SHK_E_SLOT_FULL);
      if (!bits) { b->region_cap = cap; b->slot_overflows = 0; break; }
      if (++b->slot_overflows >= 2) b->slots_off = 1;
      cap = 0;
    }
    cur ^= 1;
  }
  HIPCHK(hipGetLastError());
  *dst = cur;
  return SHK_OK;
}

#define SHK_REGION_SLICE (1u << 24)
#define SHK_FOR_REGION_SLICES(c, A, nblk) \
  for (uint32_t r0_ = 0, nblk = 0; r0_ < (c)->nregions && ((A).r0 = r0_, nblk = (c)->nregions - r0_ < SHK_REGION_SLICE ? (c)->nregions - r0_ : SHK_REGION_SLICE, true); r0_ += SHK_REGION_SLICE)

template <int MODE>
static void launch_merge(shk_ctx *c, const ShkMergeArgs &A0, bool rec = false) {
  ShkMergeArgs A = A0;
  SHK_FOR_REGION_SLICES(c, A, nblk) {
    if (MODE != 1 && rec)
      hipLaunchKernelGGL((k_region_merge<MODE == 1 ? 0 : MODE, SHK_IMG_BLOCKS, false, true>), dim3(nblk), dim3(SHK_MERGE_GROUP), 0, c->stream, A);
    else if (c->big_image)
      hipLaunchKernelGGL((k_region_merge<MODE, SHK_IMG_BLOCKS_BIG>), dim3(nblk), dim3(SHK_MERGE_GROUP), 0, c->stream, A);
    else
      hipLaunchKernelGGL((k_region_merge<MODE, SHK_IMG_BLOCKS>), dim3(nblk), dim3(SHK_MERGE_GROUP), 0, c->stream, A);
  }
}

struct MergeOut {
  uint64_t newd, added, removed;
  uint32_t err;
};

static uint8_t *spill_out(const shk_ctx *c) { return c->spill[c->rec_live ? c->live ^ 1 : c->live]; }

static bool lazy_reserve(shk_ctx *c) {
  if (!c->lazy_ok || c->spill[1]) return c->lazy_ok != 0;
  void *v = nullptr;
  if (hipMalloc(&v, (uint64_t)c->nregions * SHK_SPILL_STRIDE + SHK_SLACK) != hipSuccess) {
    (void)hipGetLastError();
    c->lazy_ok = 0;
    return false;
  }
  c->spill[1] = (uint8_t *)v;
  return true;
}

static void fill_args(shk_ctx *c, ShkMergeArgs *A, const uint64_t *words, uint32_t lo, uint32_t hi, int denoise);
static int table_sync(shk_ctx *c) {
  if (!c->table_stale) return SHK_OK;
  ShkMergeArgs A;
  fill_args(c, &A, nullptr, 0, 0, 0);
  A.tabB = c->tab[c->cur]; A.finB = c->fin[c->cur]; A.spill = c->spill[c->live]; A.summary = nullptr;
  HIPCHK(hipMemsetAsync(c->tab[c->cur], 0, c->table_bytes, c->stream));
  { ProfScope ps(c, KP_PLACE);
    SHK_FOR_REGION_SLICES(c, A, nblk)
      hipLaunchKernelGGL((k_region_place<SHK_IMG_BLOCKS>), dim3(nblk), dim3(SHK_WAVE), 0, c->stream, A); }
  HIPCHK(hipGetLastError());
  uint32_t bits = 0;
  if (fetch_err(c, &bits)) return SHK_ERR_HIP;
  if (bits) return map_err_bits(bits);
  c->table_stale = 0;
  return SHK_OK;
}

static void fill_args(shk_ctx *c, ShkMergeArgs *A, const uint64_t *words, uint32_t lo, uint32_t hi, int denoise) {
  A->want_hist = 0;
  A->tabA = c->tab[c->cur]; A->tabB = c->tab[c->cur ^ 1];
  A->finA = c->fin[c->cur]; A->finB = c->fin[c->cur ^ 1];
  A->words = reinterpret_cast<const uint32_t *>(words); A->region_base = c->d_base[c->nlevels]; A->region_cap = c->region_cap;
  A->nslots = c->nslots; A->xnslots = c->xnslots; A->nblocks = c->nblocks; A->q_lo = c->q_lo; A->hb = c->cfg.hb;
  A->chunk_lo = lo; A->chunk_hi = hi; A->denoise = denoise;
  A->ablate = 0;
#ifdef SHK_DIAGNOSTICS
  { const char *ab = getenv("SHK_ABLATE"); A->ablate = ab ? (uint32_t)atoi(ab) : 0; }
#endif
  { const char *sp = getenv("SHK_STAMPS");
    A->dbg = (sp && strcmp(sp, "fused") != 0) ? (unsigned long long *)(c->d_scalars + DS_STAMPS) : nullptr; }
  A->spill = spill_out(c); A->orec = c->spill[c->live]; A->over_list = c->d_over_list; A->n_over = c->d_counters + SHK_CNT_NOVER; A->list = nullptr;
  A->newchunks = nullptr; A->chist = nullptr;
  A->counted = c->counted;
  A->r0 = 0; A->rstride = 1;
  A->split = ~0u; A->isum = nullptr; A->ilens = nullptr; A->prot_list = nullptr; A->nprot = 0;
  A->summary = c->d_summary; A->counters = c->d_counters; A->err = c->d_err;
}

static int ensure_chist(shk_ctx *c) {
  if (c->d_newchunks) return SHK_OK;
  if (dmalloc(&c->d_newchunks, (uint64_t)c->nregions * SHK_NC_CAP) || dmalloc(&c->d_chist, (uint64_t)SHK_MAX_CHUNKS)) return SHK_ERR_HIP;
  HIPCHK(hipHostMalloc((void **)&c->h_chist, SHK_MAX_CHUNKS * sizeof(uint64_t), hipHostMallocDefault));
  return SHK_OK;
}

static int merge_summary(shk_ctx *c, const uint64_t *words, uint32_t lo, uint32_t hi, int denoise, MergeOut *o,
                         bool with_chist, bool spill) {
  const bool rec = c->rec_live && !denoise;
  if (!rec) { int rc = table_sync(c); if (rc) return rc; }
  ShkMergeArgs A;
  fill_args(c, &A, words, lo, hi, denoise);
  HIPCHK(hipMemsetAsync(c->d_counters, 0, (SHK_CNT_NOVER + 1) * 8, c->stream));
  c->spill_valid = 0;
  if (with_chist) {
    int rc = ensure_chist(c);
    if (rc) return rc;
    A.want_hist = 1; A.newchunks = c->d_newchunks; A.chist = c->d_chist;
    HIPCHK(hipMemsetAsync(c->d_chist, 0, SHK_MAX_CHUNKS * 8, c->stream));
  }
  if (spill) { ProfScope ps(c, KP_MERGE_SPILL);
    launch_merge<3>(c, A, rec); }
  else { ProfScope ps(c, KP_MERGE_SUM);
    launch_merge<0>(c, A, rec); }
  { ProfScope ps(c, KP_REGION_SCAN);
    const uint32_t ntiles = (c->nregions + SHK_RSCAN_TILE - 1) / SHK_RSCAN_TILE;
    hipLaunchKernelGGL(k_region_scan_a, dim3(ntiles), dim3(c->threads), 0, c->stream, c->d_summary, c->nregions, c->d_tile_a, c->d_tile_b);
    hipLaunchKernelGGL(k_region_scan_b, dim3(1), dim3(c->threads), 0, c->stream, c->d_tile_a, c->d_tile_b, ntiles, c->d_tile_f);
    hipLaunchKernelGGL(k_region_scan_c, dim3(ntiles), dim3(c->threads), 0, c->stream, c->d_summary, c->nregions, c->d_tile_f,
                       c->xnslots, (uint32_t)(c->big_image ? SHK_IMG_BLOCKS_BIG * 64 : SHK_IMG_SLOTS), c->fin[c->cur ^ 1], c->d_counters, c->d_err); }
  if (with_chist) {
    ProfScope ps(c, KP_MISC);
    hipLaunchKernelGGL(k_chunk_hist, dim3((c->nregions + SHK_CHIST_REGIONS - 1) / SHK_CHIST_REGIONS), dim3(256), 0, c->stream,
                       c->d_newchunks, c->d_summary, c->nregions, c->d_chist);
    HIPCHK(hipMemcpyAsync(c->h_chist, c->d_chist, ((uint64_t)hi + 1) * 8, hipMemcpyDeviceToHost, c->stream));
  }
  HIPCHK(hipGetLastError());
  const uint64_t *cnt = c->h_pinned + HP_COUNTERS;
  HIPCHK(hipMemcpyAsync(c->h_pinned + HP_COUNTERS, c->d_counters, (SHK_CNT_NOVER + 1) * 8, hipMemcpyDeviceToHost, c->stream));
  if (err_enqueue(c)) return SHK_ERR_HIP;
  HIPCHK(hipStreamSynchronize(c->stream));
  o->newd = cnt[CNT_NEWD]; o->added = cnt[CNT_ADDED]; o->removed = cnt[CNT_REMOVED];
  if (err_take(c, true, &o->err)) return SHK_ERR_HIP;
  c->chist_n = with_chist ? hi + 1 : 0;
  if (spill && !o->err) {
    c->spill_valid = 1; c->spill_words = words; c->spill_lo = lo; c->spill_hi = hi; c->spill_denoise = denoise;
    c->spill_big = c->big_image; c->spill_nover = cnt[SHK_CNT_NOVER];
  }
  return SHK_OK;
}

static int merge_write(shk_ctx *c, const uint64_t *words, uint32_t lo, uint32_t hi, int denoise) {
  const bool match = c->spill_valid && c->spill_words == words && c->spill_lo == lo && c->spill_hi == hi && c->spill_denoise == denoise &&
                     c->spill_big == c->big_image;
  if (match && c->spill_nover == 0 && !c->big_image && !c->counted && lazy_reserve(c)) {
    if (c->rec_live) c->live ^= 1;
    c->rec_live = 1; c->table_stale = 1;
    c->spill_valid = 0;
    c->cur ^= 1;
    return SHK_OK;
  }
  if (!match || c->spill_nover) { int rc = table_sync(c); if (rc) return rc; }
  ShkMergeArgs A;
  fill_args(c, &A, words, lo, hi, denoise);
  HIPCHK(hipMemsetAsync(c->tab[c->cur ^ 1], 0, c->table_bytes, c->stream));
  if (match) {
    { ProfScope ps(c, KP_PLACE);
      SHK_FOR_REGION_SLICES(c, A, nblk) {
        if (c->big_image) hipLaunchKernelGGL((k_region_place<SHK_IMG_BLOCKS_BIG>), dim3(nblk), dim3(SHK_WAVE), 0, c->stream, A);
        else hipLaunchKernelGGL((k_region_place<SHK_IMG_BLOCKS>), dim3(nblk), dim3(SHK_WAVE), 0, c->stream, A);
      }
      A.r0 = 0; }
    if (c->spill_nover) {
      A.list = c->d_over_list;
      ProfScope ps(c, KP_MERGE_WRITE);
      if (c->big_image)
        hipLaunchKernelGGL((k_region_merge<1, SHK_IMG_BLOCKS_BIG>), dim3((uint32_t)c->spill_nover), dim3(SHK_MERGE_GROUP), 0, c->stream, A);
      else
        hipLaunchKernelGGL((k_region_merge<1, SHK_IMG_BLOCKS>), dim3((uint32_t)c->spill_nover), dim3(SHK_MERGE_GROUP), 0, c->stream, A);
    }
  } else {
    ProfScope ps(c, KP_MERGE_WRITE);
    launch_merge<1>(c, A);
  }
  c->spill_valid = 0;
  HIPCHK(hipGetLastError());
  c->rec_live = 0; c->table_stale = 0;
  c->cur ^= 1;
  return SHK_OK;
}

static int denoise_round_once(shk_ctx *c, uint64_t *removed) {
  uint64_t ml = c->cfg.min_denoise_len ? c->cfg.min_denoise_len : (1ULL << 20);
  { int rc = table_sync(c); if (rc) return rc; }
  { ProfScope ps(c, KP_MARKS);
    hipLaunchKernelGGL(k_denoise_marks, dim3(1), dim3(64), 0, c->stream, c->tab[c->cur], c->nslots, c->xnslots, c->nblocks,
                       ml, (unsigned long long *)(c->d_scalars + DS_MARKS)); }
  MergeOut o;
  int rc = merge_summary(c, nullptr, 0, 0, 1, &o, false, true);
  if (rc) return rc;
  if (o.err) return map_err_bits(o.err);
  rc = merge_write(c, nullptr, 0, 0, 1);
  if (rc) return rc;
  c->nelts -= o.removed;
  c->ndistinct -= o.removed;
  *removed = o.removed;
  return SHK_OK;
}

static int denoise_with_rest(shk_ctx *c, const uint64_t *words, uint32_t lo, uint32_t hi, shk_batch_stats *st, bool *done) {
  *done = false;
  uint64_t ml = c->cfg.min_denoise_len ? c->cfg.min_denoise_len : (1ULL << 20);
  { int rc = table_sync(c); if (rc) return rc; }
  { ProfScope ps(c, KP_MARKS);
    hipLaunchKernelGGL(k_denoise_marks, dim3(1), dim3(64), 0, c->stream, c->tab[c->cur], c->nslots, c->xnslots, c->nblocks,
                       ml, (unsigned long long *)(c->d_scalars + DS_MARKS)); }
  MergeOut o;
  int rc = merge_summary(c, words, lo, hi, 1, &o, false, true);
  if (rc) return rc;
  if (o.err) return SHK_OK;
  if (c->rounds_left > 0 && c->ndistinct - o.removed + o.newd >= c->cfg.ndistinct_for_denoise) return SHK_OK;
  rc = merge_write(c, words, lo, hi, 1);
  if (rc) return rc;
  c->nelts = c->nelts - o.removed + o.added;
  c->ndistinct = c->ndistinct - o.removed + o.newd;
  st->removed += o.removed; st->denoise_rounds++;
  st->kmers += o.added; st->new_distinct += o.newd; st->chunks += hi - lo + 1;
  c->big_image = 0;
  *done = true;
  return SHK_OK;
}

#define SHK_PROT_CAP 65536u
struct PointOut {
  uint64_t newd_after, added_after, removed, added_before;
  uint32_t err;
  uint64_t islots, ifin;
  int first_used;
};

static int point_alloc(shk_ctx *c) {
  if (c->d_isum) return SHK_OK;
  if (dmalloc(&c->d_isum, 2 * (uint64_t)c->nregions + 2) || dmalloc(&c->d_ilens, (uint64_t)c->nregions * SHK_REGION) ||
      dmalloc(&c->d_fin_i, (uint64_t)c->nregions + 2) || dmalloc(&c->d_prot, (uint64_t)SHK_PROT_CAP)) return SHK_ERR_HIP;
  return SHK_OK;
}

static void point_scans(shk_ctx *c, bool final_table, bool inter_table, long long carry) {
  const uint32_t ntiles = (c->nregions + SHK_RSCAN_TILE - 1) / SHK_RSCAN_TILE;
  const uint32_t img_slots = (uint32_t)SHK_IMG_SLOTS;
  ProfScope ps(c, KP_REGION_SCAN);
  if (final_table) {
    hipLaunchKernelGGL(k_region_scan_a, dim3(ntiles), dim3(c->threads), 0, c->stream, c->d_summary, c->nregions, c->d_tile_a, c->d_tile_b, (uint32_t)SHK_SUM_STRIDE);
    hipLaunchKernelGGL(k_region_scan_b, dim3(1), dim3(c->threads), 0, c->stream, c->d_tile_a, c->d_tile_b, ntiles, c->d_tile_f, 0LL);
    hipLaunchKernelGGL(k_region_scan_c, dim3(ntiles), dim3(c->threads), 0, c->stream, c->d_summary, c->nregions, c->d_tile_f,
                       c->xnslots, img_slots, c->fin[c->cur ^ 1], c->d_counters, c->d_err, (uint32_t)SHK_SUM_STRIDE);
  }
  if (inter_table) {
    hipLaunchKernelGGL(k_region_scan_a, dim3(ntiles), dim3(c->threads), 0, c->stream, c->d_isum, c->nregions, c->d_tile_a, c->d_tile_b, 2u);
    hipLaunchKernelGGL(k_region_scan_b, dim3(1), dim3(c->threads), 0, c->stream, c->d_tile_a, c->d_tile_b, ntiles, c->d_tile_f, carry);
    hipLaunchKernelGGL(k_region_scan_c, dim3(ntiles), dim3(c->threads), 0, c->stream, c->d_isum, c->nregions, c->d_tile_f,
                       c->xnslots, img_slots, c->d_fin_i, c->d_counters, c->d_err, 2u);
  }
}

static int point_read(shk_ctx *c, PointOut *po) {
  HIPCHK(hipGetLastError());
  const uint64_t *cnt = c->h_pinned + HP_COUNTERS;
  HIPCHK(hipMemcpyAsync(c->h_pinned + HP_COUNTERS, c->d_counters, SHK_NCOUNTERS * 8, hipMemcpyDeviceToHost, c->stream));
  if (err_enqueue(c)) return SHK_ERR_HIP;
  HIPCHK(hipStreamSynchronize(c->stream));
  po->newd_after = cnt[CNT_NEWD]; po->added_after = cnt[CNT_ADDED]; po->removed = cnt[CNT_REMOVED]; po->added_before = cnt[CNT_ADDED_BEFORE];
  return err_take(c, false, &po->err);
}

static int point_try(shk_ctx *c, const uint64_t *words, uint32_t lo, uint32_t split, uint32_t hi, bool with_chist, PointOut *po) {
  int rc = point_alloc(c);
  if (rc) return rc;
  if (with_chist) { rc = ensure_chist(c); if (rc) return rc; }
  ShkMergeArgs A;
  fill_args(c, &A, words, lo, hi, 1);
  A.split = split; A.isum = c->d_isum; A.ilens = c->d_ilens;
  if (with_chist) {
    A.want_hist = 1; A.newchunks = c->d_newchunks; A.chist = c->d_chist;
    HIPCHK(hipMemsetAsync(c->d_chist, 0, SHK_MAX_CHUNKS * 8, c->stream));
  }
  { const char *sp = getenv("SHK_STAMPS");
    A.dbg = (sp && strcmp(sp, "plain") != 0) ? (unsigned long long *)(c->d_scalars + DS_STAMPS) : nullptr; }
  c->spill_valid = 0;
  c->chist_n = 0;
  HIPCHK(hipMemsetAsync(c->d_counters, 0, SHK_NCOUNTERS * 8, c->stream));
  { ProfScope ps(c, KP_MERGE_FUSED);
    SHK_FOR_REGION_SLICES(c, A, nblk) {
      if (c->rec_live) hipLaunchKernelGGL((k_region_merge<3, SHK_IMG_BLOCKS, true, true>), dim3(nblk), dim3(SHK_MERGE_GROUP), 0, c->stream, A);
      else hipLaunchKernelGGL((k_region_merge<3, SHK_IMG_BLOCKS, true>), dim3(nblk), dim3(SHK_MERGE_GROUP), 0, c->stream, A);
    } }
  point_scans(c, true, true, 0);
  if (with_chist) {
    ProfScope ps(c, KP_MISC);
    hipLaunchKernelGGL(k_chunk_hist, dim3((c->nregions + SHK_CHIST_REGIONS - 1) / SHK_CHIST_REGIONS), dim3(256), 0, c->stream,
                       c->d_newchunks, c->d_summary, c->nregions, c->d_chist, 1u);
    HIPCHK(hipMemcpyAsync(c->h_chist, c->d_chist, ((uint64_t)hi + 1) * 8, hipMemcpyDeviceToHost, c->stream));
  }
  HIPCHK(hipMemcpyAsync(c->h_pinned + HP_IFIN, c->d_fin_i + c->nregions, 8, hipMemcpyDeviceToHost, c->stream));
  HIPCHK(hipMemcpyAsync(c->h_pinned + HP_IFIRST, c->d_ilens, 1, hipMemcpyDeviceToHost, c->stream));
  rc = point_read(c, po);
  if (rc) return rc;
  po->islots = c->h_pinned[HP_COUNTERS + SHK_CNT_ISLOTS];
  po->ifin = c->h_pinned[HP_IFIN];
  po->first_used = (c->h_pinned[HP_IFIRST] & 0xff) != 0;
  if (with_chist && !po->err) c->chist_n = hi + 1;
  return SHK_OK;
}

static int point_walk(shk_ctx *c, long long carry, const ShkWalkShard &W, const uint64_t state_in[2], uint64_t state_out[2],
                      uint64_t *nprot, uint32_t *err) {
  const uint64_t ml = c->cfg.min_denoise_len ? c->cfg.min_denoise_len : (1ULL << 20);
  if (carry > 0) point_scans(c, false, true, carry);
  c->h_pinned[HP_WALK_IN] = state_in[0]; c->h_pinned[HP_WALK_IN + 1] = state_in[1];
  HIPCHK(hipMemcpyAsync(c->d_scalars + DS_WALK_IN, c->h_pinned + HP_WALK_IN, 16, hipMemcpyHostToDevice, c->stream));
  { ProfScope ps(c, KP_MARKS);
    hipLaunchKernelGGL(k_denoise_marks_virtual, dim3(1), dim3(64), 0, c->stream, (const uint64_t *)c->d_fin_i, (const uint8_t *)c->d_ilens,
                       (const uint32_t *)c->d_isum, c->nslots, c->xnslots, ml, c->d_prot, SHK_PROT_CAP, (unsigned long long *)(c->d_scalars + DS_MARKS),
                       W, (const uint64_t *)(c->d_scalars + DS_WALK_IN), c->d_scalars + DS_WALK_OUT); }
  HIPCHK(hipGetLastError());
  HIPCHK(hipMemcpyAsync(c->h_pinned + HP_MARKS, c->d_scalars + DS_MARKS, 8, hipMemcpyDeviceToHost, c->stream));
  HIPCHK(hipMemcpyAsync(c->h_pinned + HP_WALK_OUT, c->d_scalars + DS_WALK_OUT, 16, hipMemcpyDeviceToHost, c->stream));
  if (err_enqueue(c)) return SHK_ERR_HIP;
  HIPCHK(hipStreamSynchronize(c->stream));
  *nprot = c->h_pinned[HP_MARKS];
  state_out[0] = c->h_pinned[HP_WALK_OUT]; state_out[1] = c->h_pinned[HP_WALK_OUT + 1];
  return err_take(c, false, err);
}

static int point_finish(shk_ctx *c, const uint64_t *words, uint32_t lo, uint32_t split, uint32_t hi, uint64_t nprot, PointOut *po) {
  if (nprot > SHK_PROT_CAP) { po->err |= SHK_E_FUSED; return SHK_OK; }
  if (nprot) {
    std::vector<uint64_t> prot(nprot);
    HIPCHK(hipMemcpyAsync(prot.data(), c->d_prot, nprot * 8, hipMemcpyDeviceToHost, c->stream));
    HIPCHK(hipStreamSynchronize(c->stream));
    std::vector<uint32_t> regs;
    for (uint64_t q : prot) { const uint32_t r = (uint32_t)(q >> SHK_REGION_LOG2); if (regs.empty() || regs.back() != r) regs.push_back(r); }
    ShkMergeArgs A;
    fill_args(c, &A, words, lo, hi, 1);
    A.split = split; A.isum = c->d_isum; A.ilens = c->d_ilens;
    HIPCHK(hipMemsetAsync(c->d_counters, 0, SHK_NCOUNTERS * 8, c->stream));
    HIPCHK(hipMemcpyAsync(c->d_over_list, regs.data(), regs.size() * 4, hipMemcpyHostToDevice, c->stream));
    A.list = c->d_over_list; A.prot_list = c->d_prot; A.nprot = (uint32_t)nprot;
    { ProfScope ps(c, KP_MISC);
      if (c->rec_live) hipLaunchKernelGGL((k_region_merge<3, SHK_IMG_BLOCKS, true, true>), dim3((uint32_t)regs.size()), dim3(SHK_MERGE_GROUP), 0, c->stream, A);
      else hipLaunchKernelGGL((k_region_merge<3, SHK_IMG_BLOCKS, true>), dim3((uint32_t)regs.size()), dim3(SHK_MERGE_GROUP), 0, c->stream, A); }
    HIPCHK(hipStreamSynchronize(c->stream));
    point_scans(c, true, false, 0);
    int rc = point_read(c, po);
    if (rc) return rc;
  }
  if (!po->err) {
    c->spill_valid = 1; c->spill_words = words; c->spill_lo = lo; c->spill_hi = hi; c->spill_denoise = 1; c->spill_big = c->big_image;
    c->spill_nover = 0;
  }
  return SHK_OK;
}

static int denoise_fused(shk_ctx *c, const uint64_t *words, uint32_t lo, uint32_t cstar, uint32_t hi, uint64_t newd_before,
                         shk_batch_stats *st, bool *done, bool verify = false, uint32_t *exact_ch = nullptr, int *crossing = nullptr) {
  *done = false;
  if (crossing) *crossing = -1;
  if (c->big_image || getenv("SHK_NO_FUSED_POINT")) return SHK_OK;
  PointOut po;
  int rc = point_try(c, words, lo, cstar, hi, verify, &po);
  if (rc) return rc;
  if (po.err) {
    if (getenv("SHK_DEBUG_FUSED")) fprintf(stderr, "SHK_DEBUG_FUSED fallback: flags 0x%x\n", po.err);
    return SHK_OK;
  }
  if (verify) {
    uint64_t run = c->ndistinct;
    uint32_t ch = lo;
    for (; ch < hi; ch++) {
      run += c->h_chist[ch];
      if (run >= c->cfg.ndistinct_for_denoise) break;
    }
    if (ch == hi) run += c->h_chist[ch];
    const bool crosses = run >= c->cfg.ndistinct_for_denoise;
    if (exact_ch) *exact_ch = ch;
    if (crossing) *crossing = crosses ? 1 : 0;
    if (getenv("SHK_DEBUG_FUSED")) fprintf(stderr, "SHK_DEBUG_FUSED guess %u exact %u crossing %d\n", cstar, ch, (int)crosses);
    if (!crosses || ch != cstar) return SHK_OK;
    newd_before = run - c->ndistinct;
  }
  ShkWalkShard W;
  W.prev_fp = -1; W.cap_local = c->nslots; W.last = 1; W.next_first_used = 0;
  const uint64_t s_in[2] = {0, 0};
  uint64_t s_out[2], nprot = 0;
  uint32_t werr = 0;
  rc = point_walk(c, 0, W, s_in, s_out, &nprot, &werr);
  if (rc) return rc;
  if (werr) return SHK_OK;
  rc = point_finish(c, words, lo, cstar, hi, nprot, &po);
  if (rc) return rc;
  if (po.err) {
    c->spill_valid = 0;
    if (getenv("SHK_DEBUG_FUSED")) fprintf(stderr, "SHK_DEBUG_FUSED fallback: flags 0x%x (second go)\n", po.err);
    return SHK_OK;
  }
  if (c->rounds_left > 1 && c->ndistinct + newd_before - po.removed + po.newd_after >= c->cfg.ndistinct_for_denoise) { c->spill_valid = 0; return SHK_OK; }
  rc = merge_write(c, words, lo, hi, 1);
  if (rc) return rc;
  c->nelts = c->nelts + po.added_before - po.removed + po.added_after;
  c->ndistinct = c->ndistinct + newd_before - po.removed + po.newd_after;
  c->rounds_left--; c->rounds_done++;
  st->removed += po.removed; st->denoise_rounds++;
  st->kmers += po.added_before + po.added_after; st->new_distinct += newd_before + po.newd_after; st->chunks += hi - lo + 1;
  *done = true;
  if (getenv("SHK_DEBUG_FUSED")) fprintf(stderr, "SHK_DEBUG_FUSED one-pass point at chunk %u of [%u, %u]: removed %llu protected %llu\n", cstar, lo, hi,
                                         (unsigned long long)po.removed, (unsigned long long)nprot);
  return SHK_OK;
}

static int denoise_round(shk_ctx *c, uint64_t *removed) {
  int rc = denoise_round_once(c, removed);
  if (rc == SHK_ERR_REGION && !c->big_image && (c->last_err_bits & (SHK_E_OLD_EXTENT | SHK_E_NEW_EXTENT))) {
    c->big_image = 1;
    c->last_err_bits = 0;
    rc = denoise_round_once(c, removed);
  }
  if (!rc) c->big_image = 0;
  return rc;
}

static int sample_pass(shk_ctx *c, const uint64_t *words, uint32_t lo, uint32_t hi, uint32_t *ns_out, uint32_t *err_out) {
  int rc = ensure_chist(c);
  if (rc) return rc;
  const uint32_t stride = c->sample_stride > 1 ? c->sample_stride : 1;
  const uint32_t ns = (c->nregions + stride - 1) / stride;
  ShkMergeArgs A;
  fill_args(c, &A, words, lo, hi, 0);
  A.want_hist = 1; A.newchunks = c->d_newchunks; A.chist = c->d_chist; A.rstride = stride;
  c->spill_valid = 0;
  c->chist_n = 0;
  HIPCHK(hipMemsetAsync(c->d_chist, 0, SHK_MAX_CHUNKS * 8, c->stream));
  { ProfScope ps(c, KP_MERGE_SAMPLE);
    for (uint32_t r0 = 0; r0 < ns; r0 += SHK_REGION_SLICE) {
      A.r0 = r0;
      const uint32_t nblk = ns - r0 < SHK_REGION_SLICE ? ns - r0 : SHK_REGION_SLICE;
      if (c->rec_live) hipLaunchKernelGGL((k_region_merge<0, SHK_IMG_BLOCKS, false, true>), dim3(nblk), dim3(SHK_MERGE_GROUP), 0, c->stream, A);
      else hipLaunchKernelGGL((k_region_merge<0, SHK_IMG_BLOCKS>), dim3(nblk), dim3(SHK_MERGE_GROUP), 0, c->stream, A);
    }
    hipLaunchKernelGGL(k_chunk_hist, dim3((ns + SHK_CHIST_REGIONS - 1) / SHK_CHIST_REGIONS), dim3(256), 0, c->stream,
                       c->d_newchunks, c->d_summary, c->nregions, c->d_chist, stride); }
  HIPCHK(hipGetLastError());
  HIPCHK(hipMemcpyAsync(c->h_chist, c->d_chist, ((uint64_t)hi + 1) * 8, hipMemcpyDeviceToHost, c->stream));
  if (err_enqueue(c)) return SHK_ERR_HIP;
  HIPCHK(hipStreamSynchronize(c->stream));
  *ns_out = ns;
  return err_take(c, false, err_out);
}

static int sample_locate(shk_ctx *c, const uint64_t *words, uint32_t lo, uint32_t hi, int *verdict, uint32_t *guess) {
  *verdict = 2;
  if (c->ndistinct >= c->cfg.ndistinct_for_denoise) return SHK_OK;
  uint32_t ns = 0, err = 0;
  int rc = sample_pass(c, words, lo, hi, &ns, &err);
  if (rc) return rc;
  if (err) return SHK_OK;
  const double F = (double)c->nregions / (double)ns;
  const double need = (double)(c->cfg.ndistinct_for_denoise - c->ndistinct);
  double cum = 0;
  uint32_t at = hi + 1;
  for (uint32_t ch = lo; ch <= hi; ch++) {
    cum += F * (double)c->h_chist[ch];
    if (at > hi && cum >= need) at = ch;
  }
  const double margin = 6.0 * sqrt(F * cum + 1.0);
  if (cum + margin < need) *verdict = 0;
  else if (cum - margin >= need && at <= hi) { *verdict = 1; *guess = at; }
  if (getenv("SHK_DEBUG_FUSED")) fprintf(stderr, "SHK_DEBUG_FUSED sample: need %.0f predicted %.0f +- %.0f -> verdict %d at %u of [%u, %u]\n", need, cum, margin / 6.0, *verdict, at, lo, hi);
  return SHK_OK;
}

static int merge_stage_from(shk_ctx *c, const uint64_t *words, uint32_t nchunks, uint64_t nwords, shk_batch_stats *st,
                            uint32_t *lo_io) {
  const uint32_t soft = SHK_E_TABLE_FULL | SHK_E_NEW_EXTENT;
  uint32_t &lo = *lo_io;
  while (lo < nchunks) {
    uint32_t hi = nchunks - 1;
    const bool watch = c->rounds_left > 0;
    MergeOut o;
    int rc;
    const double reach = c->new_frac > 0 ? 2.0 * c->new_frac * (double)nwords * (double)(hi - lo + 1) / (double)nchunks : (double)nwords;
    const bool possible = watch && (double)c->ndistinct + reach >= (double)c->cfg.ndistinct_for_denoise;
    int sv = 2;
    if (possible && c->sample_stride > 1 && !c->big_image && !c->counted) {
      uint32_t guess = 0;
      rc = sample_locate(c, words, lo, hi, &sv, &guess);
      if (rc) return rc;
      if (sv == 1 && guess + 1 < nchunks) {
        bool fused = false;
        uint32_t ech = 0;
        int crossing = -1;
        rc = denoise_fused(c, words, lo, guess, nchunks - 1, 0, st, &fused, true, &ech, &crossing);
        if (rc) return rc;
        if (fused) { lo = nchunks; continue; }
        if (crossing == 1 && ech != guess && ech + 1 < nchunks) {
          uint64_t run = 0;
          for (uint32_t ch = lo; ch <= ech; ch++) run += c->h_chist[ch];
          rc = denoise_fused(c, words, lo, ech, nchunks - 1, run, st, &fused);
          if (rc) return rc;
          if (fused) { lo = nchunks; continue; }
        }
      }
    }
    const bool with_chist = possible && sv != 0;
    bool have_chist = false;
    for (;;) {
      rc = merge_summary(c, words, lo, hi, 0, &o, with_chist, true);
      if (rc) return rc;
      if (with_chist && !(o.err & ~soft)) have_chist = true;
      if (o.err & ~(soft | SHK_E_HASH_FULL)) return map_err_bits(o.err & ~(soft | SHK_E_HASH_FULL));
      if (o.err & SHK_E_HASH_FULL) {
        if (hi == lo) return SHK_ERR_REGION;
        hi = lo + (hi - lo) / 2;
        continue;
      }
      break;
    }
    bool fire = false;
    if (watch && c->ndistinct + o.newd >= c->cfg.ndistinct_for_denoise) {
      if (!have_chist) {
        rc = merge_summary(c, words, lo, hi, 0, &o, true, false);
        if (rc) return rc;
        if (o.err & ~soft) return map_err_bits(o.err & ~soft);
      }
      uint64_t run = c->ndistinct;
      uint32_t ch = lo;
      for (; ch < hi; ch++) {
        run += c->h_chist[ch];
        if (run >= c->cfg.ndistinct_for_denoise) break;
      }
      if (ch == hi) run += c->h_chist[ch];
      if (ch + 1 < nchunks) {
        bool fused = false;
        rc = denoise_fused(c, words, lo, ch, nchunks - 1, run - c->ndistinct, st, &fused);
        if (rc) return rc;
        if (fused) { lo = nchunks; continue; }
      }
      hi = ch;
      fire = true;
      rc = merge_summary(c, words, lo, hi, 0, &o, false, true);
      if (rc) return rc;
      if (o.err) return map_err_bits(o.err);
      rc = merge_write(c, words, lo, hi, 0);
      if (rc) return rc;
    } else {
      if (o.err) return map_err_bits(o.err);
      rc = merge_write(c, words, lo, hi, 0);
      if (rc) return rc;
    }
    if (o.added && !fire) c->new_frac = (double)o.newd / (double)o.added;
    c->ndistinct += o.newd;
    c->nelts += o.added;
    st->kmers += o.added;
    st->new_distinct += o.newd;
    st->chunks += hi - lo + 1;
    if (fire) {
      uint64_t removed = 0;
      c->rounds_left--;
      c->rounds_done++;
      if (hi + 1 < nchunks) {
        bool done = false;
        rc = denoise_with_rest(c, words, hi + 1, nchunks - 1, st, &done);
        if (rc) return rc;
        if (done) { lo = nchunks; continue; }
      }
      rc = denoise_round(c, &removed);
      if (rc) return rc;
      st->removed += removed;
      st->denoise_rounds++;
    }
    lo = hi + 1;
  }
  return SHK_OK;
}

static int merge_stage(shk_ctx *c, const uint64_t *words, uint32_t nchunks, uint64_t nwords, shk_batch_stats *st) {
  uint32_t lo = 0;
  int rc = merge_stage_from(c, words, nchunks, nwords, st, &lo);
  if (rc == SHK_ERR_REGION && !c->big_image && (c->last_err_bits & (SHK_E_OLD_EXTENT | SHK_E_NEW_EXTENT))) {
    c->big_image = 1;
    c->last_err_bits = 0;
    rc = merge_stage_from(c, words, nchunks, nwords, st, &lo);
  }
  return rc;
}

static int finish(shk_ctx *c, int rc) {
  uint32_t bits = 0;
  int rc2 = fetch_err(c, &bits);
  prof_collect(c);
  if (rc) return rc;
  if (rc2) return rc2;
  return map_err_bits(bits);
}

static int front_end(const shk_ctx *c, ShkStageBufs *b, const void *text, int on_device, uint64_t text_bytes, const uint64_t *chunk_off,
                     const uint64_t *chunk_len, uint32_t nchunks, uint64_t *nwords, int *dst, uint32_t *region_cap) {
  const bool roll = roll_path(c);
  int rc = roll ? roll_stage(c, b, text, on_device, text_bytes, chunk_off, chunk_len, nchunks, 0, 1)
                : hash_stage(c, b, text, on_device, text_bytes, chunk_off, chunk_len, nchunks, 0, 1, true);
  if (rc) return rc;
  uint32_t bits = 0;
  HIPCHK(hipMemcpyAsync(b->h_pinned + HP_NWORDS, b->d_scalars + DS_NWORDS, 8, hipMemcpyDeviceToHost, b->stream));
  if (fetch_err(b, &bits)) return SHK_ERR_HIP;
  if (bits) return map_err_bits(bits);
  *nwords = b->h_pinned[HP_NWORDS];
  if (*nwords > c->cfg.max_batch_keys) return SHK_ERR_BATCH;
  rc = partition_stage(c, b, roll ? part_from_roll(c, b, *nwords, nchunks) : part_from_hash(b, *nwords, nchunks), dst);
  *region_cap = b->region_cap;
  return rc;
}

extern "C" int shk_count_chunks(shk_ctx *c, const void *text, int text_on_device, uint64_t text_bytes,
                                const uint64_t *chunk_off, const uint64_t *chunk_len, uint32_t nchunks,
                                shk_batch_stats *stats) {
  if (!c || !text || !chunk_off || !chunk_len) return SHK_ERR_ARG;
  shk_batch_stats st;
  memset(&st, 0, sizeof(st));
  HIPCHK(hipSetDevice(c->dev));
  if (upload_wait(c, text, text_on_device, c->stream)) return SHK_ERR_HIP;
  uint64_t nwords = 0;
  int dst = 0;
  uint32_t cap = 0;
  int rc = front_end(c, c, text, text_on_device, text_bytes, chunk_off, chunk_len, nchunks, &nwords, &dst, &cap);
  if (rc) return finish(c, rc);
  rc = merge_stage(c, c->d_words[dst], nchunks, nwords, &st);
  if (stats) *stats = st;
  return finish(c, rc);
}

struct ShkFrontSlot {
  uint64_t *words = nullptr;
  uint64_t *base = nullptr;
  uint32_t cap = 0;
  std::thread th;
  bool busy = false;
  int rc = 0;
  uint64_t nwords = 0;
  uint32_t nchunks = 0;
};
struct ShkFront {
  ShkStageBufs b;
  ShkFrontSlot slot[2];
  int head = 0, count = 0;
  int par = 0;
  uint64_t *scratch = nullptr;
};

static int front_init(shk_ctx *c) {
  ShkFront *F = new ShkFront();
  c->front = F;
  { int rc = bufs_alloc(c, &F->b, true); if (rc) return rc; }
  F->par = roll_path(c) ? (int)((c->nlevels - 1) & 1) : (int)(c->nlevels & 1);
  const uint64_t capk = c->cfg.max_batch_keys;
  if (dmalloc(&F->scratch, capk + 1)) return SHK_ERR_HIP;
  for (int k2 = 0; k2 < 2; k2++)
    if (dmalloc(&F->slot[k2].words, capk + 1) || dmalloc(&F->slot[k2].base, level_out(c, c->nlevels - 1) + 2)) return SHK_ERR_HIP;
  return SHK_OK;
}
static void front_destroy(shk_ctx *c) {
  ShkFront *F = c->front;
  if (!F) return;
  for (int k2 = 0; k2 < 2; k2++) if (F->slot[k2].th.joinable()) F->slot[k2].th.join();
  bufs_free(c, &F->b);
  hipFree(F->scratch);
  for (int k2 = 0; k2 < 2; k2++) { hipFree(F->slot[k2].words); hipFree(F->slot[k2].base); }
  delete F;
  c->front = nullptr;
}

static void front_run(const shk_ctx *c, ShkFrontSlot *S, const void *text, int on_device, uint64_t text_bytes, std::vector<uint64_t> off,
                      std::vector<uint64_t> len) {
  ShkFront *F = c->front;
  ShkStageBufs *b = &F->b;
  hipSetDevice(c->dev);
  b->d_words[F->par] = S->words; b->d_words[F->par ^ 1] = F->scratch;
  b->d_base[c->nlevels] = S->base;
  S->nwords = 0; S->nchunks = (uint32_t)off.size();
  int dst = 0;
  int rc = front_end(c, b, text, on_device, text_bytes, off.data(), len.data(), S->nchunks, &S->nwords, &dst, &S->cap);
  if (!rc) {
    uint32_t bits = 0;
    if (fetch_err(b, &bits)) rc = SHK_ERR_HIP;
    else if (bits) rc = map_err_bits(bits);
    else if (dst != F->par) rc = SHK_ERR_CORRUPT;
  }
  if (rc) hipStreamSynchronize(b->stream);
  S->rc = rc;
}

extern "C" int shk_prepare_chunks(shk_ctx *c, const void *text, int text_on_device, uint64_t text_bytes, const uint64_t *chunk_off,
                                  const uint64_t *chunk_len, uint32_t nchunks) {
  if (!c || !text || !chunk_off || !chunk_len || !text_aligned(text, text_on_device)) return SHK_ERR_ARG;
  if (!chunk_labels_ok(nchunks, 0, 1)) return SHK_ERR_BATCH;
  if (c->cfg.num_shards > 1) return SHK_ERR_ARG;
  HIPCHK(hipSetDevice(c->dev));
  if (!c->front) { int rc = front_init(c); if (rc) { front_destroy(c); return rc; } }
  ShkFront *F = c->front;
  if (F->count == 2) return SHK_ERR_BATCH;
  ShkFrontSlot *S = &F->slot[(F->head + F->count) & 1];
  ShkFrontSlot *O = &F->slot[(F->head + F->count + 1) & 1];
  if (O->th.joinable()) O->th.join();
  if (upload_wait(c, text, text_on_device, F->b.stream)) return SHK_ERR_HIP;
  std::vector<uint64_t> off(chunk_off, chunk_off + nchunks), len(chunk_len, chunk_len + nchunks);
  S->busy = true;
  F->count++;
#if defined(__HIPCC__)
  S->th = std::thread(front_run, c, S, text, text_on_device, text_bytes, std::move(off), std::move(len));
#else
  front_run(c, S, text, text_on_device, text_bytes, std::move(off), std::move(len));
#endif
  return SHK_OK;
}

extern "C" int shk_prepare_reserve(shk_ctx *c) {
  if (!c || c->cfg.num_shards > 1) return SHK_ERR_ARG;
  HIPCHK(hipSetDevice(c->dev));
  if (!c->front) { int rc = front_init(c); if (rc) { front_destroy(c); return rc; } }
  lazy_reserve(c);
  if (c->cfg.num_denoise) {
    int rc = ensure_chist(c);
    if (!rc) rc = point_alloc(c);
    if (rc) return rc;
  }
  return SHK_OK;
}

extern "C" int shk_count_prepared(shk_ctx *c, shk_batch_stats *stats) {
  if (!c || !c->front || c->front->count == 0) return SHK_ERR_ARG;
  HIPCHK(hipSetDevice(c->dev));
  ShkFront *F = c->front;
  ShkFrontSlot *S = &F->slot[F->head];
  if (S->th.joinable()) S->th.join();
  F->head ^= 1; F->count--;
  S->busy = false;
  ShkStageBufs *f = &F->b;
  shk_batch_stats st;
  memset(&st, 0, sizeof(st));
  if (stats) *stats = st;
  {
    ShkFrontSlot *O = &F->slot[F->head];
    if (!(O->busy && O->th.joinable())) {
      prof_collect(f);
      for (int i = 0; i < KP_N; i++) { c->prof_ms[i] += f->prof_ms[i]; c->prof_n[i] += f->prof_n[i]; f->prof_ms[i] = 0; f->prof_n[i] = 0; }
    } }
  if (S->rc) return S->rc;
  uint64_t *saved = c->d_base[c->nlevels];
  const uint32_t saved_cap = c->region_cap;
  c->d_base[c->nlevels] = S->base; c->region_cap = S->cap;
  int rc = merge_stage(c, S->words, S->nchunks, S->nwords, &st);
  c->d_base[c->nlevels] = saved; c->region_cap = saved_cap;
  if (stats) *stats = st;
  return finish(c, rc);
}

extern "C" int shk_upload_text(shk_ctx *c, const void *host_text, uint64_t nbytes, void **d_text) {
  if (!c || !host_text || !d_text || nbytes > c->cfg.max_batch_bytes) return c && host_text && d_text ? SHK_ERR_BATCH : SHK_ERR_ARG;
  HIPCHK(hipSetDevice(c->dev));
  if (!c->copy_stream) {
    HIPCHK(hipStreamCreateWithFlags(&c->copy_stream, hipStreamNonBlocking));
    for (int b = 0; b < 2; b++) HIPCHK(hipEventCreateWithFlags(&c->up_done[b], hipEventDisableTiming));
  }
  const int b = c->up_next;
  if (!c->d_up[b] && dmalloc(&c->d_up[b], c->cfg.max_batch_bytes + 64)) return SHK_ERR_HIP;
  HIPCHK(hipMemcpyAsync(c->d_up[b], host_text, nbytes, hipMemcpyHostToDevice, c->copy_stream));
  HIPCHK(hipEventRecord(c->up_done[b], c->copy_stream));
  c->up_pending[b] = 1;
  c->up_next ^= 1;
  *d_text = c->d_up[b];
  return SHK_OK;
}

extern "C" int shk_host_alloc(uint64_t nbytes, void **p) {
  if (!p) return SHK_ERR_ARG;
  HIPCHK(hipHostMalloc(p, nbytes, hipHostMallocDefault));
  return SHK_OK;
}
extern "C" void shk_host_free(void *p) { if (p) hipHostFree(p); }

extern "C" int shk_hash_chunks(shk_ctx *c, const void *text, int text_on_device, uint64_t text_bytes,
                               const uint64_t *chunk_off, const uint64_t *chunk_len, uint32_t nchunks,
                               uint64_t **d_words, uint64_t *nwords) {
  if (!c || !text || !d_words || !nwords) return SHK_ERR_ARG;
  HIPCHK(hipSetDevice(c->dev));
  if (upload_wait(c, text, text_on_device, c->stream)) return SHK_ERR_HIP;
  int rc = hash_stage(c, c, text, text_on_device, text_bytes, chunk_off, chunk_len, nchunks, c->cfg.shard_index, c->cfg.num_shards ? c->cfg.num_shards : 1);
  if (rc) return finish(c, rc);
  HIPCHK(hipMemcpyAsync(c->h_pinned + HP_NWORDS, c->d_scalars + DS_NWORDS, 8, hipMemcpyDeviceToHost, c->stream));
  rc = finish(c, 0);
  *d_words = c->d_words[0];
  *nwords = c->h_pinned[HP_NWORDS];
  return rc;
}

static int partition_words(shk_ctx *c, const uint64_t *d_words, uint64_t nwords, int *dst) {
  if (set_nwords(c, nwords)) return SHK_ERR_HIP;
  return partition_stage(c, c, part_from_words(c, d_words, nwords), dst);
}

extern "C" int shk_count_words(shk_ctx *c, const uint64_t *d_words, uint64_t nwords, uint32_t nchunks,
                               shk_batch_stats *stats) {
  if (!c || (!d_words && nwords) || nchunks == 0 || nchunks > SHK_MAX_CHUNKS) return SHK_ERR_ARG;
  if (nwords > c->cfg.max_batch_keys) return SHK_ERR_BATCH;
  shk_batch_stats st;
  memset(&st, 0, sizeof(st));
  HIPCHK(hipSetDevice(c->dev));
  int dst = 0;
  int rc = partition_words(c, d_words, nwords, &dst);
  if (rc) return finish(c, rc);
  rc = merge_stage(c, c->d_words[dst], nchunks, nwords, &st);
  if (stats) *stats = st;
  return finish(c, rc);
}

static int send_buffer(shk_ctx *c, uint64_t **send) {
  const int b = c->send_next;
  if (!c->d_send[b] && dmalloc(&c->d_send[b], c->cfg.max_batch_keys + 1)) return SHK_ERR_HIP;
  *send = c->d_send[b];
  c->send_next ^= 1;
  return SHK_OK;
}

enum { ROUTE_HIST = 0, ROUTE_CURSOR = 4096 };
template <typename F>
static int owner_bins(shk_ctx *c, uint32_t nbins, uint32_t per_owner, F count, uint64_t *counts, std::vector<uint64_t> &base) {
  uint64_t *hist = c->d_block_sums + ROUTE_HIST;
  HIPCHK(hipMemsetAsync(hist, 0, nbins * 8, c->stream));
  count();
  std::vector<uint64_t> hh(nbins);
  HIPCHK(hipMemcpyAsync(hh.data(), hist, nbins * 8, hipMemcpyDeviceToHost, c->stream));
  uint32_t bits = 0;
  if (fetch_err(c, &bits)) return SHK_ERR_HIP;
  if (bits) return map_err_bits(bits);
  base.assign(nbins + 1, 0);
  std::fill(counts, counts + nbins / per_owner, 0);
  for (uint32_t i = 0; i < nbins; i++) { counts[i / per_owner] += hh[i]; base[i + 1] = base[i] + hh[i]; }
  HIPCHK(hipMemcpyAsync(c->d_block_sums + ROUTE_CURSOR, base.data(), nbins * 8, hipMemcpyHostToDevice, c->stream));
  return SHK_OK;
}

extern "C" int shk_route_words(shk_ctx *c, uint64_t nwords, uint32_t nshards, uint64_t **d_out, uint64_t *counts) {
  if (!c || !d_out || !counts || nshards == 0 || (nshards & (nshards - 1)) || nshards > SHK_RP_MAXP) return SHK_ERR_ARG;
  if (nwords > c->cfg.max_batch_keys) return SHK_ERR_BATCH;
  HIPCHK(hipSetDevice(c->dev));
  uint32_t lg = 0;
  while ((1u << lg) < nshards) lg++;
  uint64_t *send;
  if (send_buffer(c, &send)) return SHK_ERR_HIP;
  if (lg == 0) {
    HIPCHK(hipMemcpyAsync(send, c->d_words[0], nwords * 8, hipMemcpyDeviceToDevice, c->stream));
    *d_out = send; counts[0] = nwords;
    return finish(c, 0);
  }
  if (c->cfg.qb < SHK_REGION_LOG2 + lg) return SHK_ERR_ARG;
  ShkRpLevel lv;
  lv.shift = (c->cfg.qb - SHK_REGION_LOG2) - lg; lv.bits = lg; lv.nbuckets = 1; lv.hb = c->cfg.hb; lv.q_lo = 0;
  lv.nslots = ~0ULL; lv.cb = 0; lv.out32 = 0; lv.ablate = 0; lv.ng_log2 = 0; lv.slot_cap = 0;
  if (set_nwords(c, nwords)) return SHK_ERR_HIP;
  const uint64_t *n_p = c->d_scalars + DS_NWORDS;
  const uint32_t nwin = (uint32_t)(nwords / SHK_RP_TILE + 1);
  { ProfScope ps(c, KP_RP_PREP);
    hipLaunchKernelGGL(k_rp_base1, dim3(1), dim3(64), 0, c->stream, n_p, c->d_base[0]);
    hipLaunchKernelGGL(k_rp_tile_first, dim3(nwin / 256 + 1), dim3(256), 0, c->stream, c->d_base[0], 1u, n_p, c->d_tfb); }
  std::vector<uint64_t> base;
  int rc = owner_bins(c, nshards, 1, [&] {
    ProfScope ps(c, KP_RP_HIST);
    const uint32_t wt = nwin / 4096 + 1;
    hipLaunchKernelGGL(k_rp_hist<false>, dim3(nwin / wt + 1), dim3(c->threads), 0, c->stream, c->d_words[0], n_p, c->d_base[0], c->d_tfb, lv, c->d_block_sums + ROUTE_HIST, wt);
  }, counts, base);
  if (rc) return finish(c, rc);
  { ProfScope ps(c, KP_RP_SCATTER);
    hipLaunchKernelGGL((k_rp_scatter<12, SHK_RP_THREADS>), dim3(nwin), dim3(SHK_RP_THREADS), 0, c->stream, c->d_words[0], send, n_p,
                       c->d_base[0], c->d_tfb, lv, c->d_block_sums + ROUTE_CURSOR, c->d_err); }
  HIPCHK(hipGetLastError());
  *d_out = send;
  return finish(c, 0);
}

extern "C" int shk_hash_route_chunks(shk_ctx *c, const void *text, int text_on_device, uint64_t text_bytes, const uint64_t *chunk_off,
                                     const uint64_t *chunk_len, uint32_t nchunks, uint32_t nshards, uint64_t **d_out, uint64_t *counts,
                                     uint64_t *nwords) {
  if (!c || !text || !chunk_off || !chunk_len || !d_out || !counts || !nwords) return SHK_ERR_ARG;
  if (nshards == 0 || (nshards & (nshards - 1)) || nshards > SHK_RP_MAXP) return SHK_ERR_ARG;
  HIPCHK(hipSetDevice(c->dev));
  uint32_t lg = 0;
  while ((1u << lg) < nshards) lg++;
  if (c->cfg.qb < SHK_REGION_LOG2 + lg) return SHK_ERR_ARG;
  const uint32_t chunk_first = c->cfg.shard_index, chunk_mul = c->cfg.num_shards ? c->cfg.num_shards : 1;
  if (!chunk_labels_ok(nchunks, chunk_first, chunk_mul)) return SHK_ERR_BATCH;
  uint64_t *send;
  if (send_buffer(c, &send)) return SHK_ERR_HIP;
  const uint8_t *dtext;
  uint64_t nreads;
  if (upload_wait(c, text, text_on_device, c->stream)) return SHK_ERR_HIP;
  int rc = parse_stage(c, c, text, text_on_device, text_bytes, chunk_off, chunk_len, nchunks, &dtext, &nreads);
  if (rc) return finish(c, rc);
  const uint32_t rb = c->cfg.qb - SHK_REGION_LOG2;
  const uint32_t db = lg > 7 ? lg : (rb < 7 ? (rb > lg ? rb : lg) : 7);
  const uint32_t nbins = 1u << db, per_owner = nbins / nshards;
  ShkRollArgs A;
  roll_args(c, c, A, dtext, text_bytes, chunk_first, chunk_mul);
  A.q_lo = 0;
  A.dig_shift = rb - db; A.dig_bits = db;
  A.hist_shift = A.dig_shift; A.hist_bits = db;
  A.hist = c->d_block_sums + ROUTE_HIST; A.cursor = c->d_block_sums + ROUTE_CURSOR; A.out = send;
  rc = pack_stage(c, c, A, nreads, text_bytes, c->d_words[0]);
  if (rc) return finish(c, rc);
  std::vector<uint64_t> base;
  rc = owner_bins(c, nbins, per_owner, [&] {
    ProfScope ps(c, KP_ROLL_HIST);
    launch_roll_hist(c, c, A, nreads, false);
  }, counts, base);
  if (rc) return finish(c, rc);
  *nwords = base[nbins];
  if (base[nbins] > c->cfg.max_batch_keys) return finish(c, SHK_ERR_BATCH);
  launch_roll_scatter(c, c, A, nreads);
  HIPCHK(hipGetLastError());
  *d_out = send;
  return finish(c, 0);
}

extern "C" int shk_route_reserve(shk_ctx *c) {
  if (!c) return SHK_ERR_ARG;
  HIPCHK(hipSetDevice(c->dev));
  for (int b = 0; b < 2; b++)
    if (!c->d_send[b] && dmalloc(&c->d_send[b], c->cfg.max_batch_keys + 1)) return SHK_ERR_HIP;
  { int rc = ensure_chist(c); if (!rc) rc = point_alloc(c); if (rc) return rc; }
  lazy_reserve(c);
  return SHK_OK;
}

extern "C" int shk_stage_words_pair(shk_ctx *c, const uint64_t *d_a, uint64_t na, const uint64_t *d_b, uint64_t nb) {
  if (!c || (!d_a && na) || (!d_b && nb)) return SHK_ERR_ARG;
  if (na == 0) return shk_stage_words(c, d_b, nb);
  if (nb == 0) return shk_stage_words(c, d_a, na);
  if (na + nb > c->cfg.max_batch_keys) return SHK_ERR_BATCH;
  { const uint64_t *o0 = c->d_words[0], *o1 = c->d_words[0] + c->cfg.max_batch_keys + 1;
    if ((d_a + na > o0 && d_a < o1) || (d_b + nb > o0 && d_b < o1)) return SHK_ERR_ARG; }
  if (c->nlevels == 0) return SHK_ERR_ARG;
  HIPCHK(hipSetDevice(c->dev));
  if (set_nwords(c, na + nb)) return SHK_ERR_HIP;
  const uint64_t pair[DS_END - DS_PAIR_LEN] = {na, nb, 0, na, 0, nb};
  memcpy(c->h_pinned + HP_PAIR, pair, sizeof(pair));
  HIPCHK(hipMemcpyAsync(c->d_scalars + DS_PAIR_LEN, c->h_pinned + HP_PAIR, sizeof(pair), hipMemcpyHostToDevice, c->stream));
  int dst = 0;
  int rc = partition_stage(c, c, part_from_words(c, d_a, na, d_b, nb), &dst);
  c->staged = dst;
  return finish(c, rc);
}

extern "C" int shk_stage_words(shk_ctx *c, const uint64_t *d_words, uint64_t nwords) {
  if (!c || (!d_words && nwords)) return SHK_ERR_ARG;
  if (nwords > c->cfg.max_batch_keys) return SHK_ERR_BATCH;
  HIPCHK(hipSetDevice(c->dev));
  int dst = 0;
  int rc = partition_words(c, d_words, nwords, &dst);
  c->staged = dst;
  return finish(c, rc);
}

static void summary_out(const MergeOut &o, shk_summary *out) {
  out->new_distinct = o.newd; out->added = o.added; out->removed = o.removed;
  out->err_bits = o.err; out->reserved = 0;
}

extern "C" int shk_stage_summary(shk_ctx *c, uint32_t lo, uint32_t hi, int want_chunks, shk_summary *out) {
  if (!c || !out || hi < lo || hi >= SHK_MAX_CHUNKS) return SHK_ERR_ARG;
  HIPCHK(hipSetDevice(c->dev));
  MergeOut o;
  int rc = merge_summary(c, c->d_words[c->staged], lo, hi, 0, &o, want_chunks != 0, true);
  if (!rc && !c->big_image && (o.err & (SHK_E_OLD_EXTENT | SHK_E_NEW_EXTENT)) && !(o.err & SHK_E_TABLE_FULL)) {
    c->big_image = 1;
    rc = merge_summary(c, c->d_words[c->staged], lo, hi, 0, &o, want_chunks != 0, true);
  }
  prof_collect(c);
  if (rc) return rc;
  summary_out(o, out);
  return SHK_OK;
}

extern "C" int shk_stage_commit(shk_ctx *c, uint32_t lo, uint32_t hi, const shk_summary *s) {
  if (!c || !s || hi < lo) return SHK_ERR_ARG;
  if (s->err_bits) return map_err_bits(s->err_bits);
  HIPCHK(hipSetDevice(c->dev));
  int rc = merge_write(c, c->d_words[c->staged], lo, hi, 0);
  if (!rc) { c->ndistinct += s->new_distinct; c->nelts += s->added; }
  return finish(c, rc);
}

extern "C" int shk_stage_try(shk_ctx *c, uint32_t lo, uint32_t hi, int want_chunks, shk_summary *out) {
  if (!c || !out || hi < lo || hi >= SHK_MAX_CHUNKS) return SHK_ERR_ARG;
  HIPCHK(hipSetDevice(c->dev));
  MergeOut o;
  int rc;
  for (int attempt = 0; attempt < 2; attempt++) {
    rc = merge_summary(c, c->d_words[c->staged], lo, hi, 0, &o, want_chunks != 0, true);
    if (rc || c->big_image || !(o.err & (SHK_E_OLD_EXTENT | SHK_E_NEW_EXTENT)) || (o.err & SHK_E_TABLE_FULL)) break;
    c->big_image = 1;
  }
  prof_collect(c);
  if (rc) return rc;
  summary_out(o, out);
  return SHK_OK;
}

extern "C" int shk_stage_accept(shk_ctx *c, const shk_summary *s) {
  if (!c || !s) return SHK_ERR_ARG;
  if (s->err_bits) return map_err_bits(s->err_bits);
  HIPCHK(hipSetDevice(c->dev));
  if (!c->spill_valid) return SHK_ERR_ARG;
  const int dn = c->spill_denoise;
  int rc = merge_write(c, c->spill_words, c->spill_lo, c->spill_hi, dn);
  if (rc) return finish(c, rc);
  if (dn) { c->big_image = 0; c->rounds_done++; }
  c->ndistinct += s->new_distinct; c->nelts += s->added;
  c->ndistinct -= s->removed; c->nelts -= s->removed;
  return finish(c, SHK_OK);
}

extern "C" int shk_stage_try_denoise(shk_ctx *c, uint32_t lo, uint32_t hi, shk_summary *out) {
  if (!c || !out || hi < lo || hi >= SHK_MAX_CHUNKS) return SHK_ERR_ARG;
  HIPCHK(hipSetDevice(c->dev));
  uint64_t ml = c->cfg.min_denoise_len ? c->cfg.min_denoise_len : (1ULL << 20);
  { int rc = table_sync(c); if (rc) return rc; }
  { ProfScope ps(c, KP_MARKS);
    hipLaunchKernelGGL(k_denoise_marks, dim3(1), dim3(64), 0, c->stream, c->tab[c->cur], c->nslots, c->xnslots, c->nblocks,
                       ml, (unsigned long long *)(c->d_scalars + DS_MARKS)); }
  MergeOut o;
  int rc = merge_summary(c, c->d_words[c->staged], lo, hi, 1, &o, false, true);
  prof_collect(c);
  if (rc) return rc;
  summary_out(o, out);
  return SHK_OK;
}

extern "C" int shk_stage_chunk_hist(shk_ctx *c, uint64_t *out, uint32_t n) {
  if (!c || !out || !c->chist_n || n > c->chist_n) return SHK_ERR_ARG;
  memcpy(out, c->h_chist, (size_t)n * sizeof(uint64_t));
  return SHK_OK;
}

extern "C" int shk_stage_sample(shk_ctx *c, uint32_t lo, uint32_t hi, uint64_t *hist, uint32_t *regions, uint32_t *sampled,
                                uint32_t *err_bits) {
  if (!c || !hist || !regions || !sampled || !err_bits || hi < lo || hi >= SHK_MAX_CHUNKS) return SHK_ERR_ARG;
  HIPCHK(hipSetDevice(c->dev));
  uint32_t ns = 0, err = 0;
  int rc = sample_pass(c, c->d_words[c->staged], lo, hi, &ns, &err);
  prof_collect(c);
  if (rc) return rc;
  memcpy(hist, c->h_chist, ((size_t)hi + 1) * sizeof(uint64_t));
  *regions = c->nregions; *sampled = ns; *err_bits = err;
  return SHK_OK;
}

extern "C" int shk_stage_point_try(shk_ctx *c, uint32_t lo, uint32_t split, uint32_t hi, shk_point *out) {
  if (!c || !out || hi < lo || split + 1 < lo || split > hi || hi >= SHK_MAX_CHUNKS) return SHK_ERR_ARG;
  HIPCHK(hipSetDevice(c->dev));
  c->pt_valid = 0;
  memset(out, 0, sizeof(*out));
  if (c->big_image) { out->err_bits = SHK_E_FUSED; return SHK_OK; }
  PointOut po;
  int rc = point_try(c, c->d_words[c->staged], lo, split, hi, true, &po);
  prof_collect(c);
  if (rc) return rc;
  out->new_after = po.newd_after; out->added_after = po.added_after; out->removed = po.removed; out->added_before = po.added_before;
  out->err_bits = po.err; out->first_used = (uint32_t)po.first_used; out->islots = po.islots; out->ifin = po.ifin;
  if (!po.err) { c->pt_lo = lo; c->pt_split = split; c->pt_hi = hi; c->pt_valid = 1; c->pt_nprot = 0; c->pt_words = c->d_words[c->staged]; }
  return SHK_OK;
}

extern "C" int shk_stage_round_try(shk_ctx *c, shk_point *out) {
  if (!c || !out) return SHK_ERR_ARG;
  HIPCHK(hipSetDevice(c->dev));
  c->pt_valid = 0;
  memset(out, 0, sizeof(*out));
  if (c->big_image) { out->err_bits = SHK_E_FUSED; return SHK_OK; }
  PointOut po;
  int rc = point_try(c, nullptr, 0, 0, 0, false, &po);
  prof_collect(c);
  if (rc) return rc;
  out->new_after = po.newd_after; out->added_after = po.added_after; out->removed = po.removed; out->added_before = po.added_before;
  out->err_bits = po.err; out->first_used = (uint32_t)po.first_used; out->islots = po.islots; out->ifin = po.ifin;
  if (!po.err) { c->pt_lo = 1; c->pt_split = 0; c->pt_hi = 0; c->pt_valid = 1; c->pt_nprot = 0; c->pt_words = nullptr; }
  return SHK_OK;
}

extern "C" int shk_stage_point_walk(shk_ctx *c, int64_t carry, int64_t prev_fp, int last, int next_first_used,
                                    const uint64_t state_in[2], uint64_t state_out[2], uint64_t *nprot, uint32_t *err_bits) {
  if (!c || !state_in || !state_out || !nprot || !err_bits || carry < 0 || !c->pt_valid) return SHK_ERR_ARG;
  HIPCHK(hipSetDevice(c->dev));
  ShkWalkShard W;
  W.prev_fp = prev_fp; W.cap_local = c->g_nslots - c->q_lo; W.last = last; W.next_first_used = next_first_used;
  int rc = point_walk(c, carry, W, state_in, state_out, nprot, err_bits);
  prof_collect(c);
  if (rc) return rc;
  c->pt_nprot = *nprot;
  return SHK_OK;
}

extern "C" int shk_stage_point_finish(shk_ctx *c, shk_point *out, shk_summary *accept) {
  if (!c || !out || !accept || !c->pt_valid || (c->pt_words && !c->chist_n)) return SHK_ERR_ARG;
  HIPCHK(hipSetDevice(c->dev));
  PointOut po;
  po.newd_after = out->new_after; po.added_after = out->added_after; po.removed = out->removed; po.added_before = out->added_before;
  po.err = 0;
  const bool round_only = c->pt_words == nullptr;
  int rc = point_finish(c, c->pt_words, round_only ? 0 : c->pt_lo, c->pt_split, c->pt_hi, c->pt_nprot, &po);
  prof_collect(c);
  c->pt_valid = 0;
  if (rc) return rc;
  out->new_after = po.newd_after; out->added_after = po.added_after; out->removed = po.removed; out->added_before = po.added_before;
  out->err_bits = po.err;
  uint64_t newd_before = 0;
  if (!round_only) for (uint32_t ch = c->pt_lo; ch <= c->pt_split; ch++) newd_before += c->h_chist[ch];
  memset(accept, 0, sizeof(*accept));
  accept->new_distinct = newd_before + po.newd_after; accept->added = po.added_before + po.added_after; accept->removed = po.removed;
  accept->err_bits = po.err;
  return SHK_OK;
}

extern "C" int shk_denoise(shk_ctx *c, uint64_t *removed) {
  if (!c) return SHK_ERR_ARG;
  HIPCHK(hipSetDevice(c->dev));
  uint64_t r = 0;
  int rc = table_sync(c);
  if (!rc) rc = denoise_round(c, &r);
  if (!rc) c->rounds_done++;
  if (removed) *removed = r;
  return finish(c, rc);
}

extern "C" int shk_stats(shk_ctx *c, shk_totals *o) {
  if (!c || !o) return SHK_ERR_ARG;
  HIPCHK(hipSetDevice(c->dev));
  o->nelts = c->nelts; o->ndistinct = c->ndistinct; o->rounds_left = c->rounds_left; o->rounds_done = c->rounds_done;
  o->nslots = c->nslots; o->xnslots = c->xnslots; o->nblocks = c->nblocks; o->table_bytes = c->table_bytes;
  HIPCHK(hipMemcpyAsync(c->h_pinned + HP_FREE_PTR, c->fin[c->cur] + c->nregions, 8, hipMemcpyDeviceToHost, c->stream));
  HIPCHK(hipStreamSynchronize(c->stream));
  o->free_pointer = c->h_pinned[HP_FREE_PTR];
  return SHK_OK;
}

extern "C" int shk_header(shk_ctx *c, uint8_t out[128]) {
  if (!c || !out) return SHK_ERR_ARG;
  memset(out, 0, 128);
  uint64_t v;
#define PUT(off, val) do { v = (val); memcpy(out + (off), &v, 8); } while (0)
  PUT(0, c->table_bytes);
  memcpy(out + 8, &c->cfg.seed, 4);
  PUT(16, c->nslots); PUT(24, c->xnslots); PUT(32, (uint64_t)c->cfg.hb); PUT(40, 0);
  PUT(48, 8); PUT(56, 8);
  { unsigned __int128 range = (unsigned __int128)c->nslots << 8; memcpy(out + 64, &range, 16); }
  PUT(80, c->nblocks); PUT(88, c->nelts); PUT(96, c->ndistinct); PUT(104, 0);
  PUT(112, c->xnslots / (1ULL << 16) + 2);
#undef PUT
  return SHK_OK;
}

extern "C" int shk_export_blocks(shk_ctx *c, void *dst, uint64_t cap) {
  if (!c || !dst || cap < c->table_bytes) return SHK_ERR_ARG;
  HIPCHK(hipSetDevice(c->dev));
  { int rc = table_sync(c); if (rc) return rc; }
  HIPCHK(hipMemcpyAsync(dst, c->tab[c->cur], c->table_bytes, hipMemcpyDeviceToHost, c->stream));
  { uint32_t bits = 0; if (fetch_err(c, &bits)) return SHK_ERR_HIP; if (bits) return map_err_bits(bits); }
  HIPCHK(hipStreamSynchronize(c->stream));
  return SHK_OK;
}

extern "C" int shk_table_ptr(shk_ctx *c, void **d_table, uint64_t *nbytes) {
  if (!c || !d_table || !nbytes) return SHK_ERR_ARG;
  HIPCHK(hipSetDevice(c->dev));
  { int rc = table_sync(c); if (rc) return rc; }
  { uint32_t bits = 0; if (fetch_err(c, &bits)) return SHK_ERR_HIP; if (bits) return map_err_bits(bits); }
  *d_table = c->tab[c->cur]; *nbytes = c->table_bytes;
  return SHK_OK;
}
// ... 1007 lines not shown
```

sh-assembly_amd/csrc/shk_device.h:

```cpp
#pragma once
#include <hip/hip_runtime.h>
#include <stdint.h>

#define SHK_WAVE 64
#define SHK_MAX_WAVES 16
#define SHK_BLOCK_BYTES 89
#define SHK_OFF_OCC 1
#define SHK_OFF_RUN 9
#define SHK_OFF_TRAV 17
#define SHK_OFF_SLOTS 25

#define SHK_REGION_LOG2 8
#define SHK_REGION (1u << SHK_REGION_LOG2)
#define SHK_REGION_BLOCKS (SHK_REGION / 64)
#define SHK_IMG_BLOCKS 24
#define SHK_IMG_SLOTS (SHK_IMG_BLOCKS * 64)
#define SHK_IMG_BLOCKS_BIG 64
#define SHK_IMG_BYTES (SHK_IMG_BLOCKS * SHK_BLOCK_BYTES)
#define SHK_HCAP_LOG2 9
#define SHK_HCAP (1u << SHK_HCAP_LOG2)
#define SHK_MERGE_THREADS 64
#define SHK_MERGE_GROUP 128
#define SHK_CHUNK_BITS 12
#define SHK_MAX_CHUNKS (1u << SHK_CHUNK_BITS)

#define SHK_E_OLD_EXTENT   (1u << 0)
#define SHK_E_NEW_EXTENT   (1u << 1)
#define SHK_E_HASH_FULL    (1u << 2)
#define SHK_E_TABLE_FULL   (1u << 3)
#define SHK_E_CORRUPT      (1u << 4)
#define SHK_E_BAD_FASTQ    (1u << 5)
#define SHK_E_KEYS_FULL    (1u << 6)
#define SHK_E_RUN_TOO_LONG (1u << 7)
#define SHK_E_FUSED        (1u << 9)
#define SHK_E_SLOT_FULL    (1u << 10)

__device__ __forceinline__ unsigned shk_lane() { return threadIdx.x & (SHK_WAVE - 1); }
__device__ __forceinline__ unsigned shk_wave() { return threadIdx.x / SHK_WAVE; }

__device__ __forceinline__ uint64_t shk_rol64(uint64_t v, unsigned s) {
  s &= 63;
  return s ? (v << s) | (v >> (64 - s)) : v;
}
__device__ __forceinline__ uint64_t shk_ror64(uint64_t v, unsigned s) {
  s &= 63;
  return s ? (v >> s) | (v << (64 - s)) : v;
}

#define SHK_RP_TILE0_LOG2 14

__device__ __forceinline__ void shk_lds_barrier() {
#if defined(__HIP_DEVICE_COMPILE__)
  __builtin_amdgcn_fence(__ATOMIC_RELEASE, "workgroup", "local");
  __builtin_amdgcn_s_barrier();
  __builtin_amdgcn_fence(__ATOMIC_ACQUIRE, "workgroup", "local");
#else
  __syncthreads();
#endif
}

__device__ __forceinline__ void shk_wave_sync() {
  __builtin_amdgcn_fence(__ATOMIC_RELEASE, "wavefront");
  __builtin_amdgcn_wave_barrier();
  __builtin_amdgcn_fence(__ATOMIC_ACQUIRE, "wavefront");
}
#define SHK_DPP_STEPS(STEP) STEP(0x111, 0xf) STEP(0x112, 0xf) STEP(0x114, 0xf) STEP(0x118, 0xf) STEP(0x142, 0xa) STEP(0x143, 0xc)
__device__ __forceinline__ uint32_t shk_wave_incl_add(uint32_t x) {
#define SHK_STEP_(ctrl, rows) x += (uint32_t)__builtin_amdgcn_update_dpp(0, (int)x, ctrl, rows, 0xf, true);
  SHK_DPP_STEPS(SHK_STEP_)
#undef SHK_STEP_
  return x;
}
__device__ __forceinline__ uint64_t shk_wave_incl_add64(uint64_t x) {
#define SHK_STEP_(ctrl, rows) { const uint32_t lo_ = (uint32_t)__builtin_amdgcn_update_dpp(0, (int)(uint32_t)x, ctrl, rows, 0xf, true); \
                              const uint32_t hi_ = (uint32_t)__builtin_amdgcn_update_dpp(0, (int)(uint32_t)(x >> 32), ctrl, rows, 0xf, true); \
                              x += ((uint64_t)hi_ << 32) | lo_; }
  SHK_DPP_STEPS(SHK_STEP_)
#undef SHK_STEP_
  return x;
}
__device__ __forceinline__ uint32_t shk_dpp_xor_scan32(uint32_t x) {
  x ^= (uint32_t)__builtin_amdgcn_update_dpp(0, (int)x, 0x111, 0xf, 0xf, true);
  x ^= (uint32_t)__builtin_amdgcn_update_dpp(0, (int)x, 0x112, 0xf, 0xf, true);
  x ^= (uint32_t)__builtin_amdgcn_update_dpp(0, (int)x, 0x114, 0xf, 0xf, true);
  x ^= (uint32_t)__builtin_amdgcn_update_dpp(0, (int)x, 0x118, 0xf, 0xf, true);
  x ^= (uint32_t)__builtin_amdgcn_update_dpp(0, (int)x, 0x142, 0xa, 0xf, true);
  x ^= (uint32_t)__builtin_amdgcn_update_dpp(0, (int)x, 0x143, 0xc, 0xf, true);
  return x;
}
__device__ __forceinline__ uint64_t shk_wave_incl_xor64(uint64_t x) {
  const uint32_t lo = shk_dpp_xor_scan32((uint32_t)x), hi = shk_dpp_xor_scan32((uint32_t)(x >> 32));
  return ((uint64_t)hi << 32) | lo;
}
__device__ __forceinline__ uint64_t shk_last_lane64(uint64_t x) {
  const uint32_t lo = (uint32_t)__builtin_amdgcn_readlane((int)(uint32_t)x, 63);
  const uint32_t hi = (uint32_t)__builtin_amdgcn_readlane((int)(uint32_t)(x >> 32), 63);
  return ((uint64_t)hi << 32) | lo;
}

__device__ __forceinline__ uint32_t shk_block_exscan(uint32_t v, uint32_t *total, uint32_t *scratch) {
  unsigned lane = shk_lane(), wave = shk_wave(), nw = blockDim.x / SHK_WAVE;
  uint32_t incl = shk_wave_incl_add(v);
  if (lane == SHK_WAVE - 1) scratch[wave] = incl;
  __syncthreads();
  if (wave == 0) {
    uint32_t w = lane < nw ? scratch[lane] : 0;
    uint32_t wi = shk_wave_incl_add(w);
    if (lane < nw) scratch[lane] = wi - w;
    if (lane == nw - 1) scratch[SHK_MAX_WAVES] = wi;
  }
  __syncthreads();
  uint32_t res = scratch[wave] + incl - v;
  *total = scratch[SHK_MAX_WAVES];
  __syncthreads();
  return res;
}
__device__ __forceinline__ uint64_t shk_block_exscan64(uint64_t v, uint64_t *total, uint64_t *scratch) {
  unsigned lane = shk_lane(), wave = shk_wave(), nw = blockDim.x / SHK_WAVE;
  uint64_t incl = shk_wave_incl_add64(v);
  if (lane == SHK_WAVE - 1) scratch[wave] = incl;
  __syncthreads();
  if (wave == 0) {
    uint64_t w = lane < nw ? scratch[lane] : 0;
    uint64_t wi = shk_wave_incl_add64(w);
    if (lane < nw) scratch[lane] = wi - w;
    if (lane == nw - 1) scratch[SHK_MAX_WAVES] = wi;
  }
  __syncthreads();
  uint64_t res = scratch[wave] + incl - v;
  *total = scratch[SHK_MAX_WAVES];
  __syncthreads();
  return res;
}
__device__ __forceinline__ uint64_t shk_block_sum64(uint64_t v, uint64_t *scratch) {
  uint64_t t;
  shk_block_exscan64(v, &t, scratch);
  return t;
}

#define SHK_NEG_INF (-(1LL << 60))
struct ShkMP {
  long long a, b;
};
__device__ __forceinline__ ShkMP shk_mp_compose(ShkMP first, ShkMP second) {
  ShkMP r;
  r.a = first.a + second.a;
  long long t = first.b + second.a;
  r.b = t > second.b ? t : second.b;
  if (r.b < SHK_NEG_INF) r.b = SHK_NEG_INF;
  return r;
}
__device__ __forceinline__ long long shk_mp_apply(ShkMP m, long long f) {
  long long t = f + m.a;
  return t > m.b ? t : m.b;
}

#define SHK_NEG_INF_W (-(1 << 28))
struct ShkMPw {
  int a, b;
};
__device__ __forceinline__ ShkMPw shk_mpw_compose(ShkMPw first, ShkMPw second) {
  ShkMPw r;
  r.a = first.a + second.a;
  const int t = first.b + second.a;
  r.b = t > second.b ? t : second.b;
  if (r.b < SHK_NEG_INF_W) r.b = SHK_NEG_INF_W;
  return r;
}

__device__ __forceinline__ ShkMPw shk_mpw_wave_scan(ShkMPw x) {
#define SHK_STEP_(ctrl, rows) { ShkMPw y_; y_.a = __builtin_amdgcn_update_dpp(0, x.a, ctrl, rows, 0xf, true); \
                              y_.b = __builtin_amdgcn_update_dpp(SHK_NEG_INF_W, x.b, ctrl, rows, 0xf, false); \
                              x = shk_mpw_compose(y_, x); }
  SHK_DPP_STEPS(SHK_STEP_)
#undef SHK_STEP_
  return x;
}

__device__ __forceinline__ uint64_t shk_ld64(const uint8_t *p) {
  uint64_t v = 0;
#pragma unroll
  for (int i = 0; i < 8; i++) v |= (uint64_t)p[i] << (8 * i);
  return v;
}
__device__ __forceinline__ void shk_st64(uint8_t *p, uint64_t v) {
#pragma unroll
  for (int i = 0; i < 8; i++) p[i] = (uint8_t)(v >> (8 * i));
}

__device__ __forceinline__ unsigned shk_select64(uint64_t w, unsigned n) {
  if ((unsigned)__popcll(w) <= n) return 64;
  unsigned pos = 0;
#pragma unroll
  for (int width = 32; width >= 1; width >>= 1) {
    uint64_t low = w & ((1ULL << width) - 1);
    unsigned c = (unsigned)__popcll(low);
    if (n >= c) { n -= c; w >>= width; pos += width; } else { w = low; }
  }
  return pos;
}

__device__ __forceinline__ unsigned shk_enc_len(unsigned rem, uint64_t count) {
  if (count <= 1) return (unsigned)count;
  uint64_t c = count - 1;
  unsigned nd = 1;
  uint64_t t = c >> 7;
  while (t) { nd++; t >>= 7; }
  unsigned top = (unsigned)((c >> (7 * (nd - 1))) & 0x7f);
  if (nd > 1) top |= 0x80;
  return 1 + nd + (top > rem ? 1 : 0);
}
__device__ __forceinline__ unsigned shk_enc_write(uint8_t *dst, unsigned rem, uint64_t count) {
  dst[0] = (uint8_t)rem;
  if (count <= 1) return 1;
  uint64_t c = count - 1;
  unsigned nd = 1;
  uint64_t t = c >> 7;
  while (t) { nd++; t >>= 7; }
  unsigned top = (unsigned)((c >> (7 * (nd - 1))) & 0x7f);
  if (nd > 1) top |= 0x80;
  unsigned n = 1;
  if (top > rem) dst[n++] = 0;
  for (int i = (int)nd - 1; i >= 1; i--) dst[n++] = (uint8_t)(((c >> (7 * i)) & 0x7f) | 0x80);
  dst[n++] = (uint8_t)(c & 0x7f);
  return n;
}
__device__ __forceinline__ unsigned shk_dec(const uint8_t *s, bool first_is_runend, uint64_t *count) {
  unsigned rem = s[0];
  if (first_is_runend) { *count = 1; return 1; }
  unsigned digit = s[1];
  if (digit > rem) { *count = 1; return 1; }
  unsigned n = 1;
  uint64_t cnt = 0;
  if (digit == 0) { n++; digit = s[n]; }
  while (digit & 0x80) { cnt = cnt * 128 + (digit & 0x7f); n++; digit = s[n]; }
  cnt = cnt * 128 + digit;
  *count = cnt + 1;
  return n + 1;
}

#define SHK_KM_WMAX 6
template <int W> struct ShkKmer { uint64_t w[W]; };

template <int W> __device__ __forceinline__ ShkKmer<W> shk_km_zero() {
  ShkKmer<W> a;
#pragma unroll
  for (int j = 0; j < W; j++) a.w[j] = 0;
  return a;
}
template <int W> __device__ __forceinline__ ShkKmer<W> shk_km_mask(uint32_t k) {
  ShkKmer<W> m;
#pragma unroll
  for (int j = 0; j < W; j++) {
    const int bits = 2 * (int)k - 64 * j;
    m.w[j] = bits >= 64 ? ~0ULL : bits <= 0 ? 0ULL : ((1ULL << bits) - 1);
  }
  return m;
}
template <int W> __device__ __forceinline__ ShkKmer<W> shk_km_push(const ShkKmer<W> &a, unsigned c) {
  ShkKmer<W> r;
#pragma unroll
  for (int j = W - 1; j > 0; j--) r.w[j] = (a.w[j] << 2) | (a.w[j - 1] >> 62);
  r.w[0] = (a.w[0] << 2) | c;
  return r;
}
template <int W> __device__ __forceinline__ ShkKmer<W> shk_km_append(const ShkKmer<W> &a, unsigned c, const ShkKmer<W> &mask) {
  ShkKmer<W> r = shk_km_push(a, c);
#pragma unroll
  for (int j = 0; j < W; j++) r.w[j] &= mask.w[j];
  return r;
}
template <int W> __device__ __forceinline__ unsigned shk_km_base(const ShkKmer<W> &a, uint32_t p) {
  const uint32_t wi = p >> 5, sh = 2 * (p & 31);
  unsigned c = 0;
#pragma unroll
  for (int j = 0; j < W; j++) c = (uint32_t)j == wi ? (unsigned)(a.w[j] >> sh) & 3u : c;
  return c;
}
template <int W> __device__ __forceinline__ ShkKmer<W> shk_km_push_top(const ShkKmer<W> &a, unsigned c, uint32_t k) {
  const uint32_t wi = (k - 1) >> 5, sh = 2 * ((k - 1) & 31);
  ShkKmer<W> r;
#pragma unroll
  for (int j = 0; j < W - 1; j++) r.w[j] = (a.w[j] >> 2) | (a.w[j + 1] << 62);
  r.w[W - 1] = a.w[W - 1] >> 2;
#pragma unroll
  for (int j = 0; j < W; j++) r.w[j] |= (uint32_t)j == wi ? (uint64_t)c << sh : 0ULL;
  return r;
}
template <int W> __device__ __forceinline__ ShkKmer<W> shk_km_set_last(ShkKmer<W> a, unsigned c) {
  a.w[0] = (a.w[0] & ~3ULL) | c;
  return a;
}
template <int W> __device__ __forceinline__ bool shk_km_eq(const ShkKmer<W> &a, const ShkKmer<W> &b) {
  bool e = true;
#pragma unroll
  for (int j = 0; j < W; j++) e = e && a.w[j] == b.w[j];
  return e;
}
template <int W> __device__ __forceinline__ ShkKmer<W> shk_km_rc(const ShkKmer<W> &a, uint32_t k) {
  uint64_t t[W];
#pragma unroll
  for (int j = 0; j < W; j++) {
    uint64_t x = ~a.w[W - 1 - j];
    x = ((x >> 2) & 0x3333333333333333ULL) | ((x & 0x3333333333333333ULL) << 2);
    x = ((x >> 4) & 0x0F0F0F0F0F0F0F0FULL) | ((x & 0x0F0F0F0F0F0F0F0FULL) << 4);
    t[j] = __builtin_bswap64(x);
  }
  const uint32_t s = 64 * W - 2 * k, q = s >> 6, b = s & 63;
  ShkKmer<W> r;
#pragma unroll
  for (int j = 0; j < W; j++) {
    uint64_t lo = 0, hi = 0;
#pragma unroll
    for (int qq = 0; qq < W; qq++) {
      if ((uint32_t)qq == q) {
        lo = j + qq < W ? t[j + qq] : 0ULL;
        hi = j + qq + 1 < W ? t[j + qq + 1] : 0ULL;
      }
    }
    r.w[j] = b ? (lo >> b) | (hi << (64 - b)) : lo;
  }
  return r;
}
__device__ __forceinline__ uint64_t shk_ug_mix(uint64_t lo, uint64_t hi) {
  uint64_t h = lo * 0x9E3779B97F4A7C15ULL ^ (hi + 0x7F4A7C159E3779B9ULL) * 0xC2B2AE3D27D4EB4FULL;
  h ^= h >> 29; h *= 0xBF58476D1CE4E5B9ULL; h ^= h >> 32;
  return h;
}
template <int W> __device__ __forceinline__ uint64_t shk_km_mix(const ShkKmer<W> &a) {
  static_assert(W % 2 == 0, "pairs of words");
  uint64_t h = shk_ug_mix(a.w[0], a.w[1]);
#pragma unroll
  for (int j = 2; j < W; j += 2) h = shk_ug_mix(h ^ a.w[j], a.w[j + 1]);
  return h;
}
template <int W> __device__ __forceinline__ ShkKmer<W> shk_km_load(uint64_t *const (&p)[SHK_KM_WMAX], size_t i) {
// ... 10 lines not shown
```

Before: 34.65 billion.

## Scatter rolled k-mers into fixed-capacity slots to skip the histogram pass

When three partition levels are in use and the batch is large, the roll stage scatters keys straight into fixed-capacity per-digit slots. Slot bases come from a statistical bound instead of a histogram and prefix scan, which removes the roll histogram, fold, scan and copies. Later partition levels read per-bucket end arrays, and upper levels can also use slot capacities. If a slot overflows, a new error bit makes the host redo the batch through the old histogram path, and the feature turns itself off after repeated overflows. The cost is larger word buffers, gaps between slots that downstream kernels must skip, and extra host error checks that act as sync points.

```diff
diff --git a/sh-assembly_amd/csrc/partition_kernels.hip b/sh-assembly_amd/csrc/partition_kernels.hip
--- a/sh-assembly_amd/csrc/partition_kernels.hip
+++ b/sh-assembly_amd/csrc/partition_kernels.hip
@@ -96,7 +96,7 @@
 }
 
 template <bool NARROW>
-__global__ void k_rp_hist(const uint64_t *words_, const uint64_t *n_p, const uint64_t *bucket_base,
+__global__ void k_rp_hist(const uint64_t *words_, const uint64_t *n_p, const uint64_t *bucket_base, const uint64_t *bucket_end,
                           const uint32_t *tfb, ShkRpLevel lv, uint64_t *hist, uint32_t wtiles) {
   __shared__ uint32_t lh[SHK_RP_MAXP];
   using W = typename std::conditional<NARROW, uint32_t, uint64_t>::type;
@@ -108,7 +108,8 @@
   const uint32_t P = 1u << lv.bits;
   for (uint32_t b = tfb[(uint64_t)blockIdx.x * wtiles]; b < lv.nbuckets && bucket_base[b] < wend; b++) {
     const uint64_t lo = bucket_base[b] > wstart ? bucket_base[b] : wstart;
-    const uint64_t hi = bucket_base[b + 1] < wend ? bucket_base[b + 1] : wend;
+    const uint64_t be = bucket_end ? bucket_end[b] : bucket_base[b + 1];
+    const uint64_t hi = be < wend ? be : wend;
     if (hi <= lo) continue;
     for (uint32_t d = threadIdx.x; d < (P << lv.ng_log2); d += blockDim.x) lh[d] = 0;
     __syncthreads();
@@ -186,11 +187,18 @@
   const uint64_t stride = (uint64_t)gridDim.x * blockDim.x;
   for (uint64_t i = (uint64_t)blockIdx.x * blockDim.x + threadIdx.x; i < n; i += stride) cursor[i] = i * cap;
 }
+__global__ void k_rp_slot_bases(uint64_t *base, uint64_t *cursor, uint64_t n, uint64_t cap, uint64_t *extent) {
+  const uint64_t stride = (uint64_t)gridDim.x * blockDim.x;
+  for (uint64_t i = (uint64_t)blockIdx.x * blockDim.x + threadIdx.x; i <= n; i += stride) {
+    base[i] = i * cap;
+    if (i < n) cursor[i] = i * cap; else *extent = n * cap;
+  }
+}
 
 template <int TILE_LOG2, int THREADS, int PMAX = SHK_RP_MAXP, int FORM = RP_WORDS>
 __global__ void __launch_bounds__(THREADS) k_rp_scatter(const uint64_t *in_, uint64_t *out, const uint64_t *n_p,
-                                                        const uint64_t *bucket_base, const uint32_t *tfb, ShkRpLevel lv,
-                                                        uint64_t *cursor, uint32_t *err) {
+                                                        const uint64_t *bucket_base, const uint64_t *bucket_end, const uint32_t *tfb,
+                                                        ShkRpLevel lv, uint64_t *cursor, uint32_t *err) {
   constexpr uint32_t SHK_RP_TILE_ = 1u << TILE_LOG2;
   constexpr int KPT_ = (int)(SHK_RP_TILE_ / THREADS);
   static_assert(SHK_RP_TILE_ <= 65536, "a rank inside a digit takes 16 bits");
@@ -209,7 +217,8 @@
   const uint32_t P = 1u << lv.bits;
   for (uint32_t b = (lv.nbuckets > 1 ? tfb[(uint64_t)blockIdx.x << (TILE_LOG2 - 12)] : 0u); b < lv.nbuckets && bucket_base[b] < wend; b++) {
     const uint64_t lo = bucket_base[b] > wstart ? bucket_base[b] : wstart;
-    const uint64_t hi = bucket_base[b + 1] < wend ? bucket_base[b + 1] : wend;
+    const uint64_t be = bucket_end ? bucket_end[b] : bucket_base[b + 1];
+    const uint64_t hi = be < wend ? be : wend;
     if (hi <= lo) continue;
     const uint32_t cnt = (uint32_t)(hi - lo);
     for (uint32_t d = threadIdx.x; d < P; d += THREADS) lh[d] = 0;
@@ -250,7 +259,7 @@
         if (lv.ablate & 1) gbase[d] = cursor[((uint64_t)b * P + d) << lv.ng_log2] + (uint64_t)(blockIdx.x % 1024) * 24;
         else gbase[d] = v ? atomicAdd((unsigned long long *)&cursor[((((uint64_t)b * P) + d) << lv.ng_log2) | (blockIdx.x & ((1u << lv.ng_log2) - 1))], (unsigned long long)v) : 0;
         if (lv.slot_cap && v && gbase[d] + v > ((uint64_t)b * P + d + 1) * lv.slot_cap) {
-          atomicOr(err, SHK_E_SLOT_FULL);
+          atomicOr(err, lv.out32 ? SHK_E_SLOT_FULL : SHK_E_SLOT_FULL_UP);
           gbase[d] = ~0ULL;
         }
       }
@@ -268,6 +277,7 @@
       for (uint32_t d = threadIdx.x / SHK_WAVE; d < P; d += THREADS / SHK_WAVE) {
         const uint32_t l0 = lbase[d], len = lh[d];
         const uint64_t g0 = gbase[d];
+        if (g0 == ~0ULL) continue;
         for (uint32_t j = threadIdx.x % SHK_WAVE; j < len; j += SHK_WAVE) out32[g0 + j] = stage[l0 + j];
       }
     } else {
diff --git a/sh-assembly_amd/csrc/roll_kernels.hip b/sh-assembly_amd/csrc/roll_kernels.hip
--- a/sh-assembly_amd/csrc/roll_kernels.hip
+++ b/sh-assembly_amd/csrc/roll_kernels.hip
@@ -335,6 +335,7 @@
   for (;;) {
     while (!have && r < nreads) {
       const uint64_t st = A.rd_start[r], en = A.rd_end[r];
+      if (en - st > 65535) atomicOr(A.err, SHK_E_BAD_FASTQ);
       if (en - st <= 65535 && en - st >= A.k) {
         s.st = st; s.len = (uint32_t)(en - st); s.i = 0; s.fill = 0; s.fh = 0; s.rh = 0;
         tag = (uint64_t)(A.chunk_first + A.rd_chunk[r] * A.chunk_mul) << A.hb;
@@ -388,3 +389,17 @@
     if (!more) break;
   }
 }
+
+__global__ void k_roll_slot_ends(const uint64_t *cursor, uint32_t P, uint64_t cap, uint64_t *end, uint64_t *nwords, uint32_t *err) {
+  __shared__ uint64_t scratch[SHK_MAX_WAVES + 1];
+  uint64_t s = 0;
+  for (uint32_t d = threadIdx.x; d < P; d += blockDim.x) {
+    const uint64_t cu = cursor[d];
+    s += cu - (uint64_t)d * cap;
+    const bool over = cu > (uint64_t)(d + 1) * cap;
+    if (over) atomicOr(err, SHK_E_SLOT_FULL_UP);
+    end[d] = over ? (uint64_t)(d + 1) * cap : cu;
+  }
+  const uint64_t tot = shk_block_sum64(s, scratch);
+  if (threadIdx.x == 0) *nwords = tot;
+}
diff --git a/sh-assembly_amd/csrc/shk_api.hip b/sh-assembly_amd/csrc/shk_api.hip
--- a/sh-assembly_amd/csrc/shk_api.hip
+++ b/sh-assembly_amd/csrc/shk_api.hip
@@ -49,7 +49,8 @@
   DS_STAMPS = 16,
   DS_PAIR_LEN = 40,
   DS_PAIR_BASE = 42,
-  DS_END = 46
+  DS_EXTENT = 46,
+  DS_END = 48
 };
 enum ShkHostSlot {
   HP_COUNTERS = 0,
@@ -73,7 +74,7 @@
 static_assert(HP_COUNTERS + SHK_NCOUNTERS <= HP_ERR, "the counters mirror ends before the error word");
 static_assert(HP_COUNTERS + SHK_NCOUNTERS <= HP_SPECTRUM && DS_SPECTRUM + (int)SHK_SPEC_WORDS <= DS_STAMPS, "the spectrum's totals have four words of their own");
 static_assert(DS_END <= SHK_SCALAR_WORDS && HP_END <= SHK_SCALAR_WORDS, "both blocks fit their 64 words");
-static_assert(DS_PAIR_BASE + 4 == DS_END && HP_PAIR + (DS_END - DS_PAIR_LEN) == HP_END, "the pair block is uploaded in one copy");
+static_assert(DS_PAIR_BASE + 4 == DS_EXTENT && HP_PAIR + (DS_EXTENT - DS_PAIR_LEN) == HP_END, "the pair block is uploaded in one copy");
 
 enum { RP_SCATTER_GROUPED, RP_SCATTER_WIDE, RP_SCATTER_TILE };
 struct ShkPartLevel {
@@ -99,6 +100,7 @@
   uint64_t *d_base_sub = nullptr;
   uint64_t *d_base[5] = {};
   uint64_t *d_cursor = nullptr;
+  uint64_t *d_end[3] = {};
   uint32_t *d_tfb = nullptr;
   uint32_t *d_err = nullptr;
   uint64_t *h_pinned = nullptr;
@@ -106,6 +108,9 @@
   uint32_t region_cap = 0;
   uint32_t slot_overflows = 0;
   int slots_off = 0;
+  uint64_t roll_cap = 0;
+  uint32_t up_overflows = 0;
+  int up_off = 0;
   double prof_ms[KP_N] = {};
   uint64_t prof_n[KP_N] = {};
   std::vector<PendingEvent> pending;
@@ -122,6 +127,7 @@
   ShkRpLevel lv[4];
   ShkPartLevel part[4];
   bool roll_two;
+  bool roll_slots;
   uint32_t threads, hash_groups;
   uint64_t nelts, ndistinct;
   uint32_t rounds_left, rounds_done;
@@ -229,6 +235,8 @@
 static int point_alloc(shk_ctx *c);
 static uint64_t level_out(const shk_ctx *c, uint32_t l) { return (uint64_t)c->lv[l].nbuckets << c->lv[l].bits; }
 
+static uint64_t words_cap(const shk_ctx *c) { return c->cfg.max_batch_keys + (c->roll_slots ? c->cfg.max_batch_keys / 64 : 0); }
+
 static int bufs_alloc(const shk_ctx *c, ShkStageBufs *b, bool lent) {
   const uint64_t capk = c->cfg.max_batch_keys;
   const uint32_t maxch = SHK_MAX_CHUNKS;
@@ -240,7 +248,7 @@
       dmalloc(&b->d_reads_base, maxch + 1)) return SHK_ERR_HIP;
   if (dmalloc(&b->d_rd_start, c->max_reads + 1) || dmalloc(&b->d_rd_end, c->max_reads + 1) ||
       dmalloc(&b->d_nkeys, c->max_reads + 1) || dmalloc(&b->d_rd_chunk, c->max_reads + 1) || dmalloc(&b->d_key_base, c->max_reads + 2)) return SHK_ERR_HIP;
-  if (!lent && (dmalloc(&b->d_words[0], capk + 1) || dmalloc(&b->d_words[1], capk + 1))) return SHK_ERR_HIP;
+  if (!lent && (dmalloc(&b->d_words[0], words_cap(c) + 1) || dmalloc(&b->d_words[1], words_cap(c) + 1))) return SHK_ERR_HIP;
   if (dmalloc(&b->d_scalars, SHK_SCALAR_WORDS)) return SHK_ERR_HIP;
   HIPCHK(hipMemsetAsync(b->d_scalars, 0, SHK_SCALAR_WORDS * 8, b->stream));
   {
@@ -258,7 +266,8 @@
   }
   { const uint64_t nb = level_out(c, c->nlevels - 1), first = 1ULL << (c->lv[0].bits + c->lv[0].ng_log2);
     if (dmalloc(&b->d_cursor, (nb > first ? nb : first) + 2)) return SHK_ERR_HIP; }
-  if (dmalloc(&b->d_tfb, capk / SHK_RP_TILE + 2)) return SHK_ERR_HIP;
+  if (dmalloc(&b->d_tfb, (c->roll_slots ? 2 * words_cap(c) : capk) / SHK_RP_TILE + 2)) return SHK_ERR_HIP;
+  if (c->roll_slots && (dmalloc(&b->d_end[1], level_out(c, 0) + 2) || dmalloc(&b->d_end[2], level_out(c, 1) + 2))) return SHK_ERR_HIP;
   if (dmalloc(&b->d_err, 4)) return SHK_ERR_HIP;
   HIPCHK(hipMemsetAsync(b->d_err, 0, 16, b->stream));
   HIPCHK(hipHostMalloc((void **)&b->h_pinned, SHK_SCALAR_WORDS * sizeof(uint64_t), hipHostMallocDefault));
@@ -273,7 +282,7 @@
   b->evpool.clear();
   hipFree(b->d_text); hipFree(b->d_chunk_off); hipFree(b->d_chunk_len); hipFree(b->d_nlines); hipFree(b->d_reads_base);
   hipFree(b->d_rd_start); hipFree(b->d_rd_end); hipFree(b->d_rd_chunk); hipFree(b->d_nkeys); hipFree(b->d_key_base); hipFree(b->d_scalars);
-  hipFree(b->d_block_sums); hipFree(b->d_base_sub); hipFree(b->d_cursor); hipFree(b->d_tfb); hipFree(b->d_err);
+  hipFree(b->d_block_sums); hipFree(b->d_base_sub); hipFree(b->d_cursor); hipFree(b->d_end[1]); hipFree(b->d_end[2]); hipFree(b->d_tfb); hipFree(b->d_err);
   if (!b->lent) { hipFree(b->d_words[0]); hipFree(b->d_words[1]); }
   for (uint32_t l = 0; l < 4; l++) hipFree(b->d_hist[l]);
   for (uint32_t l = 0; l < 5; l++) if (!(b->lent && l == c->nlevels)) hipFree(b->d_base[l]);
@@ -327,6 +336,9 @@
     c->part[l].may_narrow = l >= 1 && l + 2 == c->nlevels && !words8;
     c->lv[l].cb = 32 - 16 - c->lv[c->nlevels - 1].bits;
   }
+  c->roll_slots = c->nlevels == 3 && c->part[1].may_narrow && c->part[2].may_slot &&
+                  !(getenv("SHK_ROLL_SLOTS") && atoi(getenv("SHK_ROLL_SLOTS")) == 0) &&
+                  cfg->max_batch_keys / (level_out(c, 1)) >= 28800;
   c->rounds_left = cfg->num_denoise;
   c->max_reads = cfg->max_batch_reads ? cfg->max_batch_reads : cfg->max_batch_bytes / 16 + 1024;
   { int rc = bufs_alloc(c, c, false); if (rc) return rc; }
@@ -545,34 +557,70 @@
 }
 
 static bool roll_path(const shk_ctx *c) { return c->nlevels >= 2; }
-static int roll_stage(const shk_ctx *c, ShkStageBufs *b, const void *text, int on_device, uint64_t text_bytes, const uint64_t *chunk_off,
-                      const uint64_t *chunk_len, uint32_t nchunks, uint32_t chunk_first, uint32_t chunk_mul) {
-  if (!chunk_labels_ok(nchunks, chunk_first, chunk_mul)) return SHK_ERR_BATCH;
-  const uint8_t *dtext;
-  uint64_t nreads;
-  { int rc = parse_stage(c, b, text, on_device, text_bytes, chunk_off, chunk_len, nchunks, &dtext, &nreads); if (rc) return rc; }
+
+static uint64_t up_slot_capacity(double m, uint64_t unit) {
+  const uint64_t cp = (uint64_t)ceil(m + 6.0 * sqrt(8.0 * m + 1.0) + 16.0);
+  return (cp + unit - 1) / unit * unit;
+}
+
+struct ShkRollBatch {
+  const uint8_t *dtext; uint64_t text_bytes, nreads;
+  uint32_t nchunks, chunk_first, chunk_mul;
+};
+
+static int roll_keys(const shk_ctx *c, ShkStageBufs *b, const ShkRollBatch &R, bool slots) {
   const uint64_t P = 1ULL << c->lv[0].bits;
   const uint32_t cb = c->lv[0].bits + c->lv[1].bits;
   const bool two = c->roll_two;
-  if (two) HIPCHK(hipMemsetAsync(b->d_hist[1], 0, (1ULL << cb) * 8, b->stream));
+  b->roll_cap = 0;
+  if (slots) {
+    const uint64_t U = c->cfg.max_batch_keys < R.text_bytes / 2 ? c->cfg.max_batch_keys : R.text_bytes / 2;
+    const uint64_t cap0 = up_slot_capacity((double)U / (double)P, 16);
+    if (P * cap0 <= words_cap(c)) b->roll_cap = cap0;
+  }
+  const uint64_t cap0 = b->roll_cap;
+  if (cap0) {
+    ProfScope ps(c, b, KP_RP_PREP);
+    hipLaunchKernelGGL(k_rp_slot_bases, dim3((uint32_t)(P / 256 + 1)), dim3(256), 0, b->stream, b->d_base[1], b->d_cursor, P, cap0, b->d_scalars + DS_EXTENT);
+  } else if (two) HIPCHK(hipMemsetAsync(b->d_hist[1], 0, (1ULL << cb) * 8, b->stream));
   else HIPCHK(hipMemsetAsync(b->d_hist[0], 0, P * 8, b->stream));
   ShkRollArgs A;
-  roll_args(c, b, A, dtext, text_bytes, chunk_first, chunk_mul);
+  roll_args(c, b, A, R.dtext, R.text_bytes, R.chunk_first, R.chunk_mul);
   A.q_lo = c->q_lo;
   A.dig_shift = c->lv[0].shift; A.dig_bits = c->lv[0].bits;
   A.hist = two ? b->d_hist[1] : b->d_hist[0]; A.hist_shift = two ? c->lv[1].shift : c->lv[0].shift; A.hist_bits = two ? cb : c->lv[0].bits;
   A.cursor = b->d_cursor; A.out = b->d_words[0];
-  { int rc = pack_stage(c, b, A, nreads, text_bytes, b->d_words[1]); if (rc) return rc; }
+  if (cap0) A.cap = P * cap0;
+  { int rc = pack_stage(c, b, A, R.nreads, R.text_bytes, b->d_words[1]); if (rc) return rc; }
+  if (cap0) {
+    launch_roll_scatter(c, b, A, R.nreads);
+    ProfScope ps(c, b, KP_RP_PREP);
+    hipLaunchKernelGGL(k_roll_slot_ends, dim3(1), dim3(c->threads < 256 ? c->threads : 256), 0, b->stream, (const uint64_t *)b->d_cursor, (uint32_t)P, cap0,
+                       b->d_end[1], b->d_scalars + DS_NWORDS, b->d_err);
+    HIPCHK(hipGetLastError());
+    return SHK_OK;
+  }
   { ProfScope ps(c, b, KP_ROLL_HIST);
-    launch_roll_hist(c, b, A, nreads, two);
+    launch_roll_hist(c, b, A, R.nreads, two);
     if (two) hipLaunchKernelGGL(k_roll_fold, dim3((uint32_t)(P / 256 + 1)), dim3(256), 0, b->stream, (const uint64_t *)b->d_hist[1], (uint32_t)P,
                                 1u << c->lv[1].bits, b->d_hist[0]); }
   if (run_scan<uint64_t>(c, b, b->d_hist[0], P, nullptr, b->d_base[1])) return SHK_ERR_HIP;
   HIPCHK(hipMemcpyAsync(b->d_scalars + DS_NWORDS, b->d_base[1] + P, 8, hipMemcpyDeviceToDevice, b->stream));
   HIPCHK(hipMemcpyAsync(b->d_cursor, b->d_base[1], P * 8, hipMemcpyDeviceToDevice, b->stream));
-  launch_roll_scatter(c, b, A, nreads);
+  launch_roll_scatter(c, b, A, R.nreads);
   HIPCHK(hipGetLastError());
   return SHK_OK;
+}
+
+static bool roll_slots_batch(const shk_ctx *c, const ShkStageBufs *b, uint32_t nchunks) {
+  return c->roll_slots && !b->up_off && nchunks <= (1u << c->lv[1].cb);
+}
+static int roll_stage(const shk_ctx *c, ShkStageBufs *b, const void *text, int on_device, uint64_t text_bytes, const uint64_t *chunk_off,
+                      const uint64_t *chunk_len, uint32_t nchunks, uint32_t chunk_first, uint32_t chunk_mul, ShkRollBatch *R) {
+  if (!chunk_labels_ok(nchunks, chunk_first, chunk_mul)) return SHK_ERR_BATCH;
+  R->text_bytes = text_bytes; R->nchunks = nchunks; R->chunk_first = chunk_first; R->chunk_mul = chunk_mul;
+  { int rc = parse_stage(c, b, text, on_device, text_bytes, chunk_off, chunk_len, nchunks, &R->dtext, &R->nreads); if (rc) return rc; }
+  return roll_keys(c, b, *R, roll_slots_batch(c, b, nchunks));
 }
 
 struct ShkPartInput {
@@ -581,11 +629,15 @@
   uint32_t first_level;
   bool counted[2];
   uint32_t nchunks;
+  uint64_t slot_cap0;
+  bool redo;
 };
-static ShkPartInput part_from_roll(const shk_ctx *c, const ShkStageBufs *b, uint64_t n, uint32_t nchunks) { return {{b->d_words[0], nullptr}, {n, 0}, 1, 0, 1, {false, c->roll_two}, nchunks}; }
-static ShkPartInput part_from_hash(const ShkStageBufs *b, uint64_t n, uint32_t nchunks) { return {{b->d_words[0], nullptr}, {n, 0}, 1, 0, 0, {true, false}, nchunks}; }
+static ShkPartInput part_from_roll(const shk_ctx *c, const ShkStageBufs *b, uint64_t n, uint32_t nchunks) {
+  return {{b->d_words[0], nullptr}, {n, 0}, 1, 0, 1, {false, c->roll_two && !b->roll_cap}, nchunks, b->roll_cap, false};
+}
+static ShkPartInput part_from_hash(const ShkStageBufs *b, uint64_t n, uint32_t nchunks) { return {{b->d_words[0], nullptr}, {n, 0}, 1, 0, 0, {true, false}, nchunks, 0, false}; }
 static ShkPartInput part_from_words(const ShkStageBufs *b, const uint64_t *w, uint64_t n, const uint64_t *w2 = nullptr, uint64_t n2 = 0) {
-  return {{w, w2}, {n, n2}, w2 ? 2 : 1, w == b->d_words[0] ? 0 : w == b->d_words[1] ? 1 : -1, 0, {false, false}, 0};
+  return {{w, w2}, {n, n2}, w2 ? 2 : 1, w == b->d_words[0] ? 0 : w == b->d_words[1] ? 1 : -1, 0, {false, false}, 0, 0, false};
 }
 
 static uint32_t slot_capacity(const shk_ctx *c, uint64_t nregions, uint64_t nwords) {
@@ -595,39 +647,57 @@
   return cp >= 64 && (double)cp >= mean + 6.0 * sqrt(8.0 * mean + 1.0) + 16.0 ? (uint32_t)cp : 0;
 }
 
+#define SHK_RC_REDO_UP 0x5348
+
 static int partition_stage(const shk_ctx *c, ShkStageBufs *b, const ShkPartInput &in, int *dst) {
   const uint64_t *n_p = b->d_scalars + DS_NWORDS;
   const uint64_t nmax = in.n[0] + in.n[1];
   { ProfScope ps(c, b, KP_RP_PREP);
     hipLaunchKernelGGL(k_rp_base1, dim3(1), dim3(64), 0, b->stream, n_p, b->d_base[0]); }
-  const uint32_t nwin = (uint32_t)(nmax / SHK_RP_TILE + 1);
   int cur = in.in_buf < 0 ? 1 : in.in_buf;
   bool counted[4] = {in.counted[0], in.counted[1], false, false};
   bool narrow = false;
+  bool up_checked = false;
+  uint64_t ext = in.slot_cap0 ? in.slot_cap0 << c->lv[0].bits : nmax;
+  const uint64_t *ext_p = in.slot_cap0 ? b->d_scalars + DS_EXTENT : n_p, *ends = in.slot_cap0 ? b->d_end[1] : nullptr;
   b->region_cap = 0;
   for (uint32_t l = in.first_level; l < c->nlevels; l++) {
     const ShkPartLevel &pl = c->part[l];
     const uint64_t nb = c->lv[l].nbuckets, P = 1ULL << c->lv[l].bits;
+    const bool last = l + 1 == c->nlevels;
     const bool narrow_in = narrow;
     narrow = pl.may_narrow && in.nchunks && in.nchunks <= (1u << c->lv[l].cb);
-    struct Src { const uint64_t *w, *n_p, *base; uint64_t n; } srcs[2] = {{l == in.first_level ? in.src[0] : b->d_words[cur], n_p, b->d_base[l], nmax}, {}};
+    struct Src { const uint64_t *w, *n_p, *base, *end; uint64_t n; } srcs[2] = {{l == in.first_level ? in.src[0] : b->d_words[cur], ext_p, b->d_base[l], ends, ext}, {}};
     int nsrc = 1;
     if (l == 0 && in.nsrc == 2) {
-      srcs[0] = {in.src[0], b->d_scalars + DS_PAIR_LEN, b->d_scalars + DS_PAIR_BASE, in.n[0]};
-      srcs[1] = {in.src[1], b->d_scalars + DS_PAIR_LEN + 1, b->d_scalars + DS_PAIR_BASE + 2, in.n[1]};
+      srcs[0] = {in.src[0], b->d_scalars + DS_PAIR_LEN, b->d_scalars + DS_PAIR_BASE, nullptr, in.n[0]};
+      srcs[1] = {in.src[1], b->d_scalars + DS_PAIR_LEN + 1, b->d_scalars + DS_PAIR_BASE + 2, nullptr, in.n[1]};
       nsrc = 2;
     }
+    const uint32_t nwin = (uint32_t)(ext / SHK_RP_TILE + 1);
     uint32_t cap = pl.may_slot && !b->slots_off && !counted[l] ? slot_capacity(c, nb * P, nmax) : 0;
+    uint64_t cap_up = 0;
+    if (in.slot_cap0 && !last) {
+      cap_up = up_slot_capacity((double)nmax / (double)(nb * P), 32);
+      const uint64_t room = 2 * words_cap(c) / (nb * P) / 32 * 32;
+      if (cap_up > room) cap_up = room;
+    }
     { ProfScope ps(c, b, KP_RP_PREP);
-      hipLaunchKernelGGL(k_rp_tile_first, dim3(nwin / 256 + 1), dim3(256), 0, b->stream, b->d_base[l], (uint32_t)nb, n_p, b->d_tfb); }
+      hipLaunchKernelGGL(k_rp_tile_first, dim3(nwin / 256 + 1), dim3(256), 0, b->stream, b->d_base[l], (uint32_t)nb, ext_p, b->d_tfb); }
     for (;;) {
       ShkRpLevel lvl = c->lv[l];
 #ifdef SHK_DIAGNOSTICS
       if (const char *e = getenv("SHK_RP_ABLATE")) lvl.ablate = (uint32_t)atoi(e);
 #endif
       uint64_t *cursor = b->d_cursor;
-      if (cap) {
-        ProfScope ps(c, b, KP_RP_SLOTS);
+      if (cap_up) {
+        ProfScope ps(c, b, KP_RP_PREP);
+        cursor = b->d_end[l + 1];
+        lvl.slot_cap = (uint32_t)cap_up;
+        hipLaunchKernelGGL(k_rp_slot_bases, dim3((uint32_t)((nb * P) / 256 + 1 < 4096 ? (nb * P) / 256 + 1 : 4096)), dim3(256), 0, b->stream, b->d_base[l + 1],
+                           cursor, nb * P, cap_up, b->d_scalars + DS_EXTENT + 1);
+      } else if (cap) {
+        ProfScope ps(c, b, in.redo ? KP_RP_PREP : KP_RP_SLOTS);
         cursor = b->d_base[l + 1];
         lvl.slot_cap = cap;
         hipLaunchKernelGGL(k_rp_slot_cursors, dim3((uint32_t)((nb * P) / 256 + 1 < 4096 ? (nb * P) / 256 + 1 : 4096)), dim3(256), 0, b->stream, cursor, nb * P, cap);
@@ -647,11 +717,11 @@
           const uint32_t wt = nwin / 4096 + 1;
           for (int si = 0; si < nsrc; si++)
             if (narrow_in)
-              hipLaunchKernelGGL(k_rp_hist<true>, dim3(nwin / wt + 1), dim3(c->threads), 0, b->stream, srcs[si].w, srcs[si].n_p, srcs[si].base, b->d_tfb,
-                                 c->lv[l], b->d_hist[l], wt);
+              hipLaunchKernelGGL(k_rp_hist<true>, dim3(nwin / wt + 1), dim3(c->threads), 0, b->stream, srcs[si].w, srcs[si].n_p, srcs[si].base, srcs[si].end,
+                                 b->d_tfb, c->lv[l], b->d_hist[l], wt);
             else
-              hipLaunchKernelGGL(k_rp_hist<false>, dim3(nwin / wt + 1), dim3(c->threads), 0, b->stream, srcs[si].w, srcs[si].n_p, srcs[si].base, b->d_tfb,
-                                 c->lv[l], b->d_hist[l], wt);
+              hipLaunchKernelGGL(k_rp_hist<false>, dim3(nwin / wt + 1), dim3(c->threads), 0, b->stream, srcs[si].w, srcs[si].n_p, srcs[si].base, srcs[si].end,
+                                 b->d_tfb, c->lv[l], b->d_hist[l], wt);
         }
         if (c->lv[l].ng_log2) {
           const uint32_t ng = c->lv[l].ng_log2;
@@ -670,31 +740,36 @@
           const dim3 wide((uint32_t)(S.n >> SHK_RP_TILE0_LOG2) + 1);
           if (narrow && pl.scatter == RP_SCATTER_WIDE)
             hipLaunchKernelGGL((k_rp_scatter<SHK_RP_TILE0_LOG2, 1024, 256, RP_NARROW_OUT>), wide, dim3(1024), 0, b->stream, S.w, b->d_words[cur ^ 1], S.n_p,
-                               S.base, b->d_tfb, lvl, cursor, b->d_err);
+                               S.base, S.end, b->d_tfb, lvl, cursor, b->d_err);
           else if (narrow)
             hipLaunchKernelGGL((k_rp_scatter<12, SHK_RP_THREADS, SHK_RP_MAXP, RP_NARROW_OUT>), dim3((uint32_t)(S.n / SHK_RP_TILE + 1)), dim3(SHK_RP_THREADS), 0,
-                               b->stream, S.w, b->d_words[cur ^ 1], S.n_p, S.base, b->d_tfb, lvl, cursor, b->d_err);
+                               b->stream, S.w, b->d_words[cur ^ 1], S.n_p, S.base, S.end, b->d_tfb, lvl, cursor, b->d_err);
           else if (narrow_in)
             hipLaunchKernelGGL((k_rp_scatter<12, SHK_RP_THREADS, SHK_RP_MAXP, RP_NARROW_IN>), dim3((uint32_t)(S.n / SHK_RP_TILE + 1)), dim3(SHK_RP_THREADS), 0,
-                               b->stream, S.w, b->d_words[cur ^ 1], S.n_p, S.base, b->d_tfb, lvl, cursor, b->d_err);
+                               b->stream, S.w, b->d_words[cur ^ 1], S.n_p, S.base, S.end, b->d_tfb, lvl, cursor, b->d_err);
           else if (pl.scatter == RP_SCATTER_GROUPED)
-            hipLaunchKernelGGL((k_rp_scatter<SHK_RP_TILE0_LOG2, 1024>), wide, dim3(1024), 0, b->stream, S.w, b->d_words[cur ^ 1], S.n_p, S.base,
+            hipLaunchKernelGGL((k_rp_scatter<SHK_RP_TILE0_LOG2, 1024>), wide, dim3(1024), 0, b->stream, S.w, b->d_words[cur ^ 1], S.n_p, S.base, S.end,
                                b->d_tfb, lvl, cursor, b->d_err);
           else if (pl.scatter == RP_SCATTER_WIDE)
-            hipLaunchKernelGGL((k_rp_scatter<SHK_RP_TILE0_LOG2, 1024, 256>), wide, dim3(1024), 0, b->stream, S.w, b->d_words[cur ^ 1], S.n_p, S.base,
+            hipLaunchKernelGGL((k_rp_scatter<SHK_RP_TILE0_LOG2, 1024, 256>), wide, dim3(1024), 0, b->stream, S.w, b->d_words[cur ^ 1], S.n_p, S.base, S.end,
                                b->d_tfb, lvl, cursor, b->d_err);
           else
             hipLaunchKernelGGL((k_rp_scatter<12, SHK_RP_THREADS>), dim3((uint32_t)(S.n / SHK_RP_TILE + 1)), dim3(SHK_RP_THREADS), 0, b->stream, S.w,
-                               b->d_words[cur ^ 1], S.n_p, S.base, b->d_tfb, lvl, cursor, b->d_err);
+                               b->d_words[cur ^ 1], S.n_p, S.base, S.end, b->d_tfb, lvl, cursor, b->d_err);
         } }
-      if (!cap) break;
+      if (!cap && !(in.slot_cap0 && last && !up_checked)) break;
       uint32_t bits = 0;
       if (fetch_err(b, &bits)) return SHK_ERR_HIP;
+      if (bits & SHK_E_SLOT_FULL_UP) return SHK_RC_REDO_UP;
       if (bits & ~SHK_E_SLOT_FULL) return map_err_bits(bits & ~SHK_E_SLOT_FULL);
+      if (in.slot_cap0 && !up_checked) { b->up_overflows = 0; up_checked = true; }
+      if (!cap) break;
       if (!bits) { b->region_cap = cap; b->slot_overflows = 0; break; }
       if (++b->slot_overflows >= 2) b->slots_off = 1;
       cap = 0;
     }
+    if (cap_up) { ext = (nb * P) * cap_up; ext_p = b->d_scalars + DS_EXTENT + 1; ends = b->d_end[l + 1]; }
+    else { ext = nmax; ext_p = n_p; ends = nullptr; }
     cur ^= 1;
   }
   HIPCHK(hipGetLastError());
@@ -1285,16 +1360,28 @@
 static int front_end(const shk_ctx *c, ShkStageBufs *b, const void *text, int on_device, uint64_t text_bytes, const uint64_t *chunk_off,
                      const uint64_t *chunk_len, uint32_t nchunks, uint64_t *nwords, int *dst, uint32_t *region_cap) {
   const bool roll = roll_path(c);
-  int rc = roll ? roll_stage(c, b, text, on_device, text_bytes, chunk_off, chunk_len, nchunks, 0, 1)
+  ShkRollBatch R = {};
+  bool part_redo = false;
+  int rc = roll ? roll_stage(c, b, text, on_device, text_bytes, chunk_off, chunk_len, nchunks, 0, 1, &R)
                 : hash_stage(c, b, text, on_device, text_bytes, chunk_off, chunk_len, nchunks, 0, 1, true);
-  if (rc) return rc;
-  uint32_t bits = 0;
-  HIPCHK(hipMemcpyAsync(b->h_pinned + HP_NWORDS, b->d_scalars + DS_NWORDS, 8, hipMemcpyDeviceToHost, b->stream));
-  if (fetch_err(b, &bits)) return SHK_ERR_HIP;
-  if (bits) return map_err_bits(bits);
-  *nwords = b->h_pinned[HP_NWORDS];
-  if (*nwords > c->cfg.max_batch_keys) return SHK_ERR_BATCH;
-  rc = partition_stage(c, b, roll ? part_from_roll(c, b, *nwords, nchunks) : part_from_hash(b, *nwords, nchunks), dst);
+  for (;;) {
+    if (rc) return rc;
+    uint32_t bits = 0;
+    HIPCHK(hipMemcpyAsync(b->h_pinned + HP_NWORDS, b->d_scalars + DS_NWORDS, 8, hipMemcpyDeviceToHost, b->stream));
+    if (fetch_err(b, &bits)) return SHK_ERR_HIP;
+    if (!(bits & SHK_E_SLOT_FULL_UP)) {
+      if (bits) return map_err_bits(bits);
+      *nwords = b->h_pinned[HP_NWORDS];
+      if (*nwords > c->cfg.max_batch_keys) return SHK_ERR_BATCH;
+      ShkPartInput in = roll ? part_from_roll(c, b, *nwords, nchunks) : part_from_hash(b, *nwords, nchunks);
+      in.redo = part_redo;
+      rc = partition_stage(c, b, in, dst);
+      if (rc != SHK_RC_REDO_UP) break;
+      part_redo = true;
+    }
+    if (++b->up_overflows >= 2) b->up_off = 1;
+    rc = roll_keys(c, b, R, false);
+  }
   *region_cap = b->region_cap;
   return rc;
 }
@@ -1341,9 +1428,9 @@
   { int rc = bufs_alloc(c, &F->b, true); if (rc) return rc; }
   F->par = roll_path(c) ? (int)((c->nlevels - 1) & 1) : (int)(c->nlevels & 1);
   const uint64_t capk = c->cfg.max_batch_keys;
-  if (dmalloc(&F->scratch, capk + 1)) return SHK_ERR_HIP;
+  if (dmalloc(&F->scratch, words_cap(c) + 1)) return SHK_ERR_HIP;
   for (int k2 = 0; k2 < 2; k2++)
-    if (dmalloc(&F->slot[k2].words, capk + 1) || dmalloc(&F->slot[k2].base, level_out(c, c->nlevels - 1) + 2)) return SHK_ERR_HIP;
+    if (dmalloc(&F->slot[k2].words, words_cap(c) + 1) || dmalloc(&F->slot[k2].base, level_out(c, c->nlevels - 1) + 2)) return SHK_ERR_HIP;
   return SHK_OK;
 }
 static void front_destroy(shk_ctx *c) {
@@ -1554,12 +1641,12 @@
   int rc = owner_bins(c, nshards, 1, [&] {
     ProfScope ps(c, KP_RP_HIST);
     const uint32_t wt = nwin / 4096 + 1;
-    hipLaunchKernelGGL(k_rp_hist<false>, dim3(nwin / wt + 1), dim3(c->threads), 0, c->stream, c->d_words[0], n_p, c->d_base[0], c->d_tfb, lv, c->d_block_sums + ROUTE_HIST, wt);
+    hipLaunchKernelGGL(k_rp_hist<false>, dim3(nwin / wt + 1), dim3(c->threads), 0, c->stream, c->d_words[0], n_p, c->d_base[0], (const uint64_t *)nullptr, c->d_tfb, lv, c->d_block_sums + ROUTE_HIST, wt);
   }, counts, base);
   if (rc) return finish(c, rc);
   { ProfScope ps(c, KP_RP_SCATTER);
     hipLaunchKernelGGL((k_rp_scatter<12, SHK_RP_THREADS>), dim3(nwin), dim3(SHK_RP_THREADS), 0, c->stream, c->d_words[0], send, n_p,
-                       c->d_base[0], c->d_tfb, lv, c->d_block_sums + ROUTE_CURSOR, c->d_err); }
+                       c->d_base[0], (const uint64_t *)nullptr, c->d_tfb, lv, c->d_block_sums + ROUTE_CURSOR, c->d_err); }
   HIPCHK(hipGetLastError());
   *d_out = send;
   return finish(c, 0);
diff --git a/sh-assembly_amd/csrc/shk_device.h b/sh-assembly_amd/csrc/shk_device.h
--- a/sh-assembly_amd/csrc/shk_device.h
+++ b/sh-assembly_amd/csrc/shk_device.h
@@ -32,6 +32,7 @@
 #define SHK_E_BAD_FASTQ    (1u << 5)
 #define SHK_E_KEYS_FULL    (1u << 6)
 #define SHK_E_RUN_TOO_LONG (1u << 7)
+#define SHK_E_SLOT_FULL_UP (1u << 8)
 #define SHK_E_FUSED        (1u << 9)
 #define SHK_E_SLOT_FULL    (1u << 10)
 
```

Result: faster. 35.54 billion, median of 6 (+2.6%).
